# Xharlie/BtcDet

Measured on AMD Instinct MI355X. Metric: scenes/s fwd+bwd KITTI-Car bs=2/GPU (BtcDet hot path), higher is better.
Workload: dtype f32

## Files before the change

### btcdet_amd/_lib.py

```python
import ctypes
import os

import numpy as np
import torch

_HERE = os.path.dirname(os.path.abspath(__file__))
LIB_PATH = os.path.join(_HERE, "libbtcdet_hip.so")
_lib = None

c_i32p = ctypes.POINTER(ctypes.c_int32)
c_f32p = ctypes.POINTER(ctypes.c_float)
vp = ctypes.c_void_p
ci = ctypes.c_int
sz = ctypes.c_size_t

MODE_SUBM, MODE_CONV, MODE_TRANSPOSE = 0, 1, 2


class BtcHipError(RuntimeError):
    pass


class BtcOccConfig(ctypes.Structure):
    _fields_ = [("batch", ctypes.c_int32), ("grid", ctypes.c_int32 * 3), ("sphere_grid", ctypes.c_int32 * 3),
                ("dist_kern", ctypes.c_int32 * 3), ("concede_x", ctypes.c_int32), ("empt_sur_thresh", ctypes.c_int32),
                ("max_boxes", ctypes.c_int32), ("use_box_weight", ctypes.c_int32),
                ("occ_range", ctypes.c_float * 6), ("occ_voxel", ctypes.c_float * 3),
                ("sphere_range", ctypes.c_float * 6), ("sphere_voxel", ctypes.c_float * 3),
                ("det_zmin", ctypes.c_float), ("det_zmax", ctypes.c_float),
                ("w_fore_cls", ctypes.c_float), ("w_mirr_cls", ctypes.c_float), ("w_bm_cls", ctypes.c_float),
                ("w_neg_cls", ctypes.c_float), ("w_fore_res", ctypes.c_float), ("w_mirr_res", ctypes.c_float),
                ("w_bm_res", ctypes.c_float), ("box_weight", ctypes.c_float), ("backproject_lut", ctypes.c_void_p),
                ("reverse_vis", ctypes.c_int32), ("vis_half", ctypes.c_int32)]


OCC_BUFFER_FIELDS = ["vcc_mask", "voxelwise_mask", "bm_voxelwise_mask", "occ_voxelwise_mask", "fore_voxelwise_mask",
                     "pos_mask", "general_cls_loss_mask", "occ_fore_cls_mask", "occ_mirr_cls_mask", "occ_bm_cls_mask",
                     "general_reg_loss_mask", "forebox_label", "general_cls_loss_mask_float",
                     "general_reg_loss_mask_float", "res_mtrx", "pos_all_num"]


class BtcOccBuffers(ctypes.Structure):
    _fields_ = [(k, ctypes.c_void_p) for k in OCC_BUFFER_FIELDS]


class BtcChainLayer(ctypes.Structure):
    _fields_ = [("kind", ctypes.c_int32), ("ref", ctypes.c_int32), ("mode", ctypes.c_int32), ("in_shape", ctypes.c_int32 * 3),
                ("out_shape", ctypes.c_int32 * 3), ("k", ctypes.c_int32 * 3), ("s", ctypes.c_int32 * 3), ("p", ctypes.c_int32 * 3),
                ("d", ctypes.c_int32 * 3)]


class BtcPovConfig(ctypes.Structure):
    _fields_ = [("batch", ctypes.c_int32), ("max_k", ctypes.c_int32), ("occ_grid", ctypes.c_int32 * 3), ("det_grid", ctypes.c_int32 * 3),
                ("occ_origin", ctypes.c_float * 3), ("occ_voxel", ctypes.c_float * 3), ("det_origin", ctypes.c_float * 3),
                ("det_voxel", ctypes.c_float * 3), ("occ_thresh", ctypes.c_float), ("inten", ctypes.c_float), ("code_dim", ctypes.c_int32)]


_SIGS = {
    "btc_last_error": (ctypes.c_char_p, []),
    "btc_version": (ci, []),
    "btc_tune_set": (ci, [ci, ci]),
    "btc_tune_value": (ci, [ci]),
    "btc_mean_vfe": (ci, [vp, vp, ci, ci, ci, ci, vp, vp]),
    "btc_occ_vfe": (ci, [vp, vp, ci, ci, ci, ci, ci, vp, vp, vp]),
    "btc_boxes_pairwise_bev": (ci, [vp, ci, vp, ci, ci, vp, vp]),
    "btc_nms_ws_bytes": (sz, [ci]),
    "btc_nms": (ci, [vp, ci, ctypes.c_float, ci, vp, vp, vp, sz, vp]),
    "btc_nms_topk_ws_bytes": (sz, [ci, ci, ci]),
    "btc_trilinear_corners": (ci, [vp, ctypes.c_longlong, ctypes.c_longlong, c_f32p, c_f32p, c_f32p, c_i32p, ci, vp, vp, vp, vp, vp, vp]),
    "btc_trilinear_gather": (ci, [vp, ci, ctypes.c_longlong, vp, vp, vp, vp]),
    "btc_trilinear_scatter": (ci, [vp, ci, vp, vp, vp, ci, vp, vp]),
    "btc_nms_topk": (ci, [vp, ci, ci, ctypes.c_float, ci, ci, vp, vp, vp, sz, vp]),
    "btc_voxelize_ws_bytes": (sz, [ci, ci, ci]),
    "btc_voxelize": (ci, [vp, ci, ci, ci, ci, ci, vp, ci, c_f32p, c_f32p, c_i32p, ci, ci, vp, vp, vp, vp, vp, sz, vp]),
    "btc_cart_to_occ_coords": (ci, [vp, vp, ci, ci, ci, vp]),
    "btc_voxel_shift_col": (ci, [vp, vp, ci, ci, ci, ci, vp, ctypes.c_float, vp]),
    "btc_range_mask_ws_bytes": (sz, [ci]),
    "btc_range_mask_compact": (ci, [vp, vp, ci, ci, ci, vp, ci, c_f32p, vp, vp, vp, vp, vp, sz, vp]),
    "btc_gather_rows": (ci, [vp, vp, ci, ci, ci, vp, vp, vp]),
    "btc_out_shape": (ci, [c_i32p, c_i32p, c_i32p, c_i32p, c_i32p, c_i32p, ci, c_i32p]),
    "btc_rulebook_subm_ws_bytes": (sz, [ci]),
    "btc_rulebook_subm": (ci, [vp, ci, ci, c_i32p, c_i32p, c_i32p, vp, vp, vp, sz, vp]),
    "btc_rulebook_conv_ws_bytes": (sz, [ci, c_i32p]),
    "btc_rulebook_conv_count": (ci, [vp, ci, ci, c_i32p, c_i32p, c_i32p, c_i32p, c_i32p, c_i32p, ci, vp, vp, sz, vp]),
    "btc_rulebook_conv_fill": (ci, [vp, ci, ci, c_i32p, c_i32p, c_i32p, c_i32p, c_i32p, c_i32p, ci, ci, vp, vp, vp, vp, sz, vp]),
    "btc_pairs_from_nbr_ws_bytes": (sz, [ci, ci]),
    "btc_pairs_from_nbr": (ci, [vp, ci, ci, ci, vp, vp, vp, sz, vp]),
    "btc_chain_ws_bytes": (sz, [vp, ci, ci, ci]),
    "btc_chain_caps": (ci, [vp, ci, ci, ci, vp]),
    "btc_chain_levels": (ci, [vp, ci, ci, vp, ci, vp, vp, vp, vp, sz, vp]),
    "btc_chain_maps": (ci, [vp, ci, ci, vp, ci, vp, vp, vp, vp, vp, vp, vp, sz, vp]),
    "btc_conv_fwd": (ci, [vp, vp, vp, vp, ci, ci, ci, ci, vp, vp]),
    "btc_conv_dgrad": (ci, [vp, vp, vp, ci, ci, ci, ci, vp, vp]),
    "btc_conv_wgrad_ws_bytes": (sz, [ci, ci, ci, ci, ci]),
    "btc_conv_wgrad": (ci, [vp, vp, vp, ci, vp, ci, ci, ci, ci, vp, vp, sz, vp]),
    "btc_conv_fwd_bf16": (ci, [vp, vp, vp, vp, ci, ci, ci, ci, vp, vp]),
    "btc_conv_dgrad_bf16": (ci, [vp, vp, vp, ci, ci, ci, ci, vp, vp]),
    "btc_conv_wgrad_bf16": (ci, [vp, vp, vp, ci, vp, ci, ci, ci, ci, vp, vp, sz, vp]),
    "btc_conv_bf16w_supported": (ci, [ci, ci, ci]),
    "btc_weights_to_bf16": (ci, [vp, ci, ci, ci, vp, vp, vp]),
    "btc_conv_split_supported": (ci, [ci, ci, ci]),
    "btc_set_scratch": (ci, [vp, vp, sz]),
    "btc_conv_split_wanted": (ci, [ci, ci, ci, ci]),
    "btc_weights_split3": (ci, [vp, ci, ci, ci, vp, vp, vp]),
    "btc_weights_split3_multi": (ci, [vp, vp, vp, c_i32p, c_i32p, c_i32p, ci, vp]),
    "btc_weights_to_bf16_multi": (ci, [vp, vp, vp, c_i32p, c_i32p, c_i32p, ci, vp]),
    "btc_conv_fwd_bf16w": (ci, [vp, vp, vp, vp, ci, ci, ci, ci, vp, vp]),
    "btc_conv_dgrad_bf16w": (ci, [vp, vp, vp, ci, ci, ci, ci, vp, vp]),
    "btc_row_orders": (ci, [vp, c_i32p, c_i32p, ci, vp, vp]),
    "btc_row_orders_keyed": (ci, [vp, vp, c_i32p, c_i32p, ci, vp, vp]),
    "btc_conv_apply_ordered": (ci, [ci, ci, vp, vp, vp, vp, vp, ci, ci, ci, ci, vp, vp]),
    "btc_conv_apply_src": (ci, [ci, ci, vp, ctypes.c_longlong, vp, vp, vp, vp, ci, ci, ci, ci, vp, vp]),
    "btc_conv_wgrad_ordered": (ci, [ci, vp, vp, vp, ci, vp, ci, vp, vp, ci, ci, ci, vp, vp, sz, vp]),
    "btc_conv_wgrad_slabs": (ci, [ci, vp, vp, vp, ci, vp, ci, vp, vp, ci, ci, ci, vp, vp, sz, vp, vp]),
    "btc_wgrad_reduce_multi": (ci, [vp, vp, vp, vp, ci, vp]),
    "btc_adam_group_ws_bytes": (sz, [ci]),
    "btc_adam_max_segments": (ci, []),
    "btc_grads_pack": (ci, [vp, ci, vp, vp, vp, vp, c_i32p, vp, vp]),
    "btc_adam_group_step": (ci, [vp, ci, vp, vp, vp, vp, c_i32p, ci, vp, vp, vp, ctypes.c_longlong, ctypes.c_float, ctypes.c_float, ctypes.c_float,
                                 ctypes.c_float, ctypes.c_float, ctypes.c_float, vp, sz, vp]),
    "btc_maxpool_fwd": (ci, [vp, vp, ci, ci, ci, vp, vp]),
    "btc_maxpool_bwd": (ci, [vp, vp, vp, vp, ci, ci, ci, vp, vp]),
    "btc_dense_fwd": (ci, [vp, vp, ci, ci, c_i32p, vp, vp]),
    "btc_dense_bwd": (ci, [vp, vp, ci, ci, c_i32p, vp, vp]),
    "btc_revoxelize_ws_bytes": (sz, [ci, ci, c_i32p]),
    "btc_revoxelize_count": (ci, [vp, ci, ci, c_i32p, vp, vp, vp, sz, vp]),
    "btc_revoxelize_fill": (ci, [vp, vp, ci, ci, ci, c_i32p, ci, ci, vp, vp, vp, vp, sz, vp]),
    "btc_pass_occ_vox_ws_bytes": (sz, [ctypes.POINTER(BtcPovConfig), ci, ci]),
    "btc_pass_occ_vox_count": (ci, [ctypes.POINTER(BtcPovConfig), vp, vp, vp, vp, vp, vp, ci, ci, ci, vp, vp, sz, vp]),
    "btc_pass_occ_vox_fill": (ci, [ctypes.POINTER(BtcPovConfig), vp, ci, ci, ci, ci, ci, ci, vp, vp, vp, vp, vp, vp, sz, vp]),
    "btc_pass_occ_vox_fill_i32": (ci, [ctypes.POINTER(BtcPovConfig), vp, ci, ci, ci, ci, ci, ci, vp, vp, vp, vp, vp, vp, vp, vp, sz, vp]),
    "btc_occ_loss_ws_bytes": (sz, []),
    "btc_occ_loss_fwd": (ci, [vp, vp, vp, vp, vp, vp, vp, vp, ci, ctypes.c_longlong, ctypes.c_float, ctypes.c_float, ctypes.c_float, vp, vp, vp,
                              sz, vp]),
    "btc_occ_loss_bwd": (ci, [vp, vp, vp, vp, vp, vp, vp, vp, ci, ctypes.c_longlong, ctypes.c_float, vp, vp, vp, vp, vp]),
    "btc_occ_loss_fwd_total": (ci, [vp, vp, vp, vp, vp, vp, vp, vp, ci, ctypes.c_longlong, ctypes.c_float, ctypes.c_float, ctypes.c_float, vp, vp,
                                    vp, sz, vp]),
    "btc_occ_loss_bwd_total": (ci, [vp, vp, vp, vp, vp, vp, vp, vp, ci, ctypes.c_longlong, ctypes.c_float, vp, vp, vp, vp, vp]),
    "btc_dense_split_fwd": (ci, [vp, vp, ci, ci, ci, vp, vp, vp, vp]),
    "btc_occ_prob": (ci, [vp, vp, ci, ctypes.c_longlong, vp, vp]),
    "btc_dense_split_bwd": (ci, [vp, vp, vp, ci, ci, ci, vp, vp, vp]),
    "btc_cat_pad_fwd": (ci, [vp, ci, vp, ci, ctypes.c_longlong, ci, ci, vp, vp]),
    "btc_cat_pad_bwd": (ci, [vp, ci, ctypes.c_longlong, ci, vp, ci, vp, ci, vp]),
    "btc_sumsq2_ws_bytes": (sz, []),
    "btc_sumsq2_fwd": (ci, [vp, ctypes.c_longlong, ci, ctypes.c_double, vp, ctypes.c_longlong, ci, ctypes.c_double, vp, vp, sz, vp]),
    "btc_sumsq2_bwd": (ci, [vp, ctypes.c_longlong, ci, ctypes.c_float, vp, vp, ctypes.c_longlong, ci, ctypes.c_float, vp, vp, vp]),
    "btc_bn_ws_bytes": (sz, [ci]),
    "btc_bn_relu_fwd": (ci, [vp, ci, ci, vp, vp, vp, vp, vp, ctypes.c_float, ctypes.c_float, ci, ci, vp, vp, vp, vp, sz, vp]),
    "btc_spin": (ci, [ci, vp]),
    "btc_bn_relu_bwd": (ci, [vp, vp, vp, ci, ci, vp, vp, vp, ci, ci, vp, vp, vp, vp, sz, vp]),
    "btc_bn_relu_fwd_bf16": (ci, [vp, ci, ci, vp, vp, vp, vp, vp, ctypes.c_float, ctypes.c_float, ci, ci, vp, vp, vp, vp, sz, vp]),
    "btc_bn_relu_bwd_bf16": (ci, [vp, vp, vp, ci, ci, vp, vp, vp, ci, ci, vp, vp, vp, vp, sz, vp]),
    "btc_ball_query": (ci, [vp, vp, vp, vp, ci, ci, ctypes.c_float, ctypes.c_float, ci, vp, vp]),
    "btc_group_points": (ci, [vp, vp, vp, vp, ci, ci, ci, ci, vp, vp]),
    "btc_group_points_grad": (ci, [vp, vp, vp, vp, ci, ci, ci, ci, ci, vp, vp]),
    "btc_furthest_point_sampling": (ci, [vp, ci, ci, ci, vp, vp, vp]),
    "btc_three_nn": (ci, [vp, vp, vp, vp, ci, ci, vp, vp, vp]),
    "btc_three_interpolate": (ci, [vp, vp, vp, ci, ci, vp, vp]),
    "btc_three_interpolate_grad": (ci, [vp, vp, vp, ci, ci, ci, vp, vp]),
    "btc_bn_fuse_ws_bytes": (sz, []),
    "btc_conv_bn_relu_fwd": (ci, [ci, vp, vp, vp, vp, vp, ci, ci, ci, ci, vp, vp, vp, vp, vp, vp, ctypes.c_float, ctypes.c_float, ci, vp, vp, vp, vp, sz, vp, vp]),
    "btc_conv_bn_relu_fwd_src": (ci, [ci, vp, ctypes.c_longlong, vp, vp, vp, vp, ci, ci, ci, ci, vp, vp, vp, vp, vp, vp, ctypes.c_float, ctypes.c_float, ci, vp, vp, vp, vp, sz, vp, vp]),
    "btc_col_sum": (ci, [vp, ci, ci, vp, vp, sz, vp]),
    "btc_col_sum_bf16": (ci, [vp, ci, ci, vp, vp, sz, vp]),
    "btc_occ_targets_ws_bytes": (sz, [ctypes.POINTER(BtcOccConfig)]),
    "btc_occ_backproject_lut": (ci, [ctypes.POINTER(BtcOccConfig), vp, vp]),
    "btc_occ_targets": (ci, [ctypes.POINTER(BtcOccConfig), vp, vp, vp, ci, ci, ci, vp, vp, vp, vp, ci, vp, vp,
                             ctypes.POINTER(BtcOccBuffers), vp, sz, vp]),
}

EXPORTED_SYMBOLS = tuple(_SIGS.keys())

_INFER_SIGS = {
    "btc_conv_bn_eval_fwd": (ci, [ci, vp, ctypes.c_longlong, vp, vp, vp, vp, ci, ci, ci, ci, vp, vp, vp, vp, ctypes.c_float, ci, vp, vp]),
    "btc_det_select_nms_ws_bytes": (sz, [ci, ci]),
    "btc_det_select_nms": (ci, [vp, vp, ci, ci, ci, ci, ci, ctypes.c_float, ctypes.c_float, ci, ci, ci, vp, vp, vp, vp, sz, vp]),
    "btc_det_finish": (ci, [vp, vp, ci, ci, ci, ci, ci, ci, vp, vp, vp, vp, ci, vp, ci, ci, vp, ci, ci, c_f32p, ci, vp, vp, vp, vp, vp, vp]),
    "btc_occ_metrics_ws_bytes": (sz, [ci, ci]),
    "btc_occ_metrics": (ci, [vp, vp, vp, vp, ctypes.c_longlong, vp, vp, vp, ctypes.c_longlong, vp, vp, ci, ci, ci, vp, vp, sz, vp]),
    "btc_kitti_overlaps": (ci, [vp, vp, vp, vp, vp, c_i32p, ci, vp, vp, vp]),
    "btc_kitti_match_tp": (ci, [vp, vp, vp, vp, vp, vp, vp, c_i32p, ci, ci, ci, ci, ci, ci, vp, vp, vp]),
    "btc_kitti_match_stats_ws_bytes": (sz, [ci, ci, ci, ci, ci]),
    "btc_kitti_match_stats": (ci, [vp, vp, vp, vp, vp, vp, vp, vp, vp, vp, vp, c_i32p, ci, ci, ci, ci, ci, ci, ci, vp, vp, vp, sz, vp]),
}

INFER_EXPORTED_SYMBOLS = tuple(_INFER_SIGS.keys())

_AUGMENT_SIGS = {
    "btc_augment_ws_bytes": (sz, [ci, ci, ci]),
    "btc_augment_batch": (ci, [vp, ci, ci, vp, ci, vp, vp, vp, ctypes.c_longlong, vp, vp, vp, vp, ci, ctypes.c_longlong, vp, vp,
                               ctypes.c_longlong, vp, vp, vp, vp, sz, vp]),
    "btc_world_transform": (ci, [vp, ci, ci, vp, ci, vp, vp, vp, vp]),
}

AUGMENT_EXPORTED_SYMBOLS = tuple(_AUGMENT_SIGS.keys())

_BESTMATCH_SIGS = {
    "btc_place_templates": (ci, [vp, ctypes.c_longlong, vp, vp, vp, vp, vp, ci, ci, vp, vp, ctypes.c_longlong, ci, vp, vp]),
}

BESTMATCH_EXPORTED_SYMBOLS = tuple(_BESTMATCH_SIGS.keys())

_FRAMES_SIGS = {
    "btc_fov_crop_ws_bytes": (sz, [ci, ci]),
    "btc_fov_crop": (ci, [vp, ci, ci, vp, ci, vp, ci, vp, vp, vp, vp, sz, vp]),
}

FRAMES_EXPORTED_SYMBOLS = tuple(_FRAMES_SIGS.keys())

_GTDB_SIGS = {
    "btc_cut_objects_ws_bytes": (sz, [ci, ci, ci, ci]),
    "btc_cut_objects": (ci, [vp, ci, ci, vp, ci, vp, vp, vp, ci, ci, ci, vp, vp, vp, vp, sz, vp]),
}

GTDB_EXPORTED_SYMBOLS = tuple(_GTDB_SIGS.keys())

cf = ctypes.c_float
_TEMPLATES_SIGS = {
    "btc_nn_sqdist": (ci, [vp, ci, vp, ci, vp, vp, ci, ci, vp, vp]),
    "btc_match_candidates": (ci, [vp, ci, vp, vp, ci, vp, vp, ci, ci, cf, cf, cf, ci, ci, vp, vp, vp]),
    "btc_select_templates_ws_bytes": (sz, [ci, ci, ci]),
    "btc_select_templates": (ci, [vp, ci, vp, ci, vp, vp, vp, vp, vp, vp, ci, ci, ci, ci, ci, cf, cf, cf, ci, ci, vp, vp, vp, vp, vp, sz, vp]),
}

TEMPLATES_EXPORTED_SYMBOLS = tuple(_TEMPLATES_SIGS.keys())

_INFOS_SIGS = {
    "btc_count_in_boxes_ws_bytes": (sz, [ci, ci]),
    "btc_count_in_boxes": (ci, [vp, ci, ci, vp, ci, vp, vp, vp, ci, vp, vp, vp, sz, vp]),
    "btc_coverage_cells_ws_bytes": (sz, [ci, ci]),
    "btc_coverage_cells": (ci, [vp, ci, vp, ci, ci, vp, vp, ci, ci, vp, vp, vp, sz, vp]),
}

INFOS_EXPORTED_SYMBOLS = tuple(_INFOS_SIGS.keys())

_HEADS_SIGS = {
    "btc_anchor_targets_ws_bytes": (sz, [ci, ci]),
    "btc_anchor_targets": (ci, [vp, ci, ci, vp, ci, vp, vp, vp, ci, vp, ci, ci, vp, vp, vp, vp, sz, vp]),
    "btc_decode_anchor_boxes": (ci, [vp, vp, vp, ci, ci, ci, cf, cf, vp, vp]),
}

HEADS_EXPORTED_SYMBOLS = tuple(_HEADS_SIGS.keys())

_ANCHOR_LOSS_SIGS = {
    "btc_anchor_loss_ws_bytes": (sz, [ci, ci]),
    "btc_anchor_loss_fwd": (ci, [vp, vp, vp, vp, vp, vp, ci, ci, ci, ci, cf, cf, cf, cf, vp, vp, vp, sz, vp]),
    "btc_anchor_loss_bwd": (ci, [vp, vp, vp, vp, vp, vp, ci, ci, ci, ci, cf, cf, cf, cf, vp, vp, vp, vp, vp, vp]),
}

ANCHOR_LOSS_EXPORTED_SYMBOLS = tuple(_ANCHOR_LOSS_SIGS.keys())


class BtcRoiTargetsConfig(ctypes.Structure):
    _fields_ = [("R", ctypes.c_int32), ("fg_quota", ctypes.c_int32), ("by_class", ctypes.c_int32), ("score_type", ctypes.c_int32),
                ("reg_fg", ctypes.c_float), ("cls_fg", ctypes.c_float), ("cls_bg", ctypes.c_float), ("cls_bg_lo", ctypes.c_float),
                ("fg_thresh", ctypes.c_float), ("cls_span", ctypes.c_float), ("hard_bg_ratio", ctypes.c_double)]


_ROI_TARGETS_SIGS = {
    "btc_roi_targets_ws_bytes": (sz, [ci, ci]),
    "btc_roi_targets": (ci, [vp, vp, vp, vp, vp, vp, ci, ci, ci, ctypes.POINTER(BtcRoiTargetsConfig), vp, vp, vp, vp, vp, vp, vp, vp, vp, vp, vp, vp, sz, vp]),
}

ROI_TARGETS_EXPORTED_SYMBOLS = tuple(_ROI_TARGETS_SIGS.keys())


def lib():
    global _lib
    if _lib is None:
        if not os.path.exists(LIB_PATH):
            raise BtcHipError(
                f"{LIB_PATH} not found: build it with `python -c 'import __graft_entry__ as g; g.build()'` "
                f"or `make -C btcdet_amd/csrc` (there is no CPU fallback for the hot path)")
        L = ctypes.CDLL(LIB_PATH)
        for name, (res, args) in (list(_SIGS.items()) + list(_INFER_SIGS.items()) + list(_AUGMENT_SIGS.items()) + list(_BESTMATCH_SIGS.items()) +
                                  list(_FRAMES_SIGS.items()) + list(_GTDB_SIGS.items()) + list(_TEMPLATES_SIGS.items()) + list(_INFOS_SIGS.items()) + list(_HEADS_SIGS.items()) +
                                  list(_ANCHOR_LOSS_SIGS.items()) + list(_ROI_TARGETS_SIGS.items())):
            fn = getattr(L, name)
            fn.restype = res
            fn.argtypes = args
        for kv in filter(None, os.environ.get("BTC_TUNE", "").split(",")):
            k, v = kv.split("=")
            if L.btc_tune_set(int(k), int(v)) != 0:
                raise BtcHipError("BTC_TUNE: bad entry %r" % kv)
        _lib = L
    return _lib


_fast = False


def fast():
    global _fast
    if _fast is False:
        _fast = None
        if os.environ.get("BTC_FASTPATH", "1") != "0":
            try:
                lib()
                from . import _btcfast
                if _btcfast.abi_version() == lib().btc_version():
                    _fast = _btcfast
            except ImportError:
                _fast = None
    return _fast


def check(rc, what):
    if rc != 0:
        msg = lib().btc_last_error().decode("utf-8", "replace")
        raise BtcHipError(f"{what} failed (code {rc}): {msg}")


_raw_stream = torch._C._cuda_getCurrentRawStream
_cur_device = torch._C._cuda_getDevice


def stream_ptr():
    return _raw_stream(_cur_device())


def ptr(t):
    if t is None:
        return None
    if not (t.is_cuda and t.is_contiguous()):
        raise BtcHipError("expected a contiguous tensor on the GPU (HIP) device")
    return t.data_ptr()


_I3_CACHE = {}


def i3(v):
    if isinstance(v, (int, np.integer)):
        key = (int(v),) * 3
    else:
        key = tuple(int(x) for x in np.asarray(v).reshape(-1))
        if len(key) != 3:
            raise BtcHipError(f"expected 3 values, got {v!r}")
    a = _I3_CACHE.get(key)
    if a is None:
        a = np.ascontiguousarray(np.array(key, dtype=np.int32))
        a.setflags(write=False)
        a_ptr = a.ctypes.data_as(c_i32p)
        _I3_CACHE[key] = a
        _I3P_CACHE[id(a)] = (a, a_ptr)
    return a


_I3P_CACHE = {}


def i3p(a):
    hit = _I3P_CACHE.get(id(a))
    if hit is not None and hit[0] is a:
        return hit[1]
    return a.ctypes.data_as(c_i32p)


def f32p(a):
    return a.ctypes.data_as(c_f32p)


def workspace(nbytes, device):
    return torch.empty(max(int(nbytes), 256), dtype=torch.uint8, device=device)
```

### btcdet_amd/backbones_3d.py

```python
import os
from functools import partial

import torch
import torch.nn as nn

from . import spconv


def post_act_block(in_channels, out_channels, kernel_size, indice_key=None, stride=1, padding=0, conv_type='subm',
                   norm_fn=None, defaultvalue=1.0, activation=nn.ReLU):
    if conv_type == 'subm':
        conv = spconv.SubMConv3d(in_channels, out_channels, kernel_size, bias=False, indice_key=indice_key)
    elif conv_type == 'subm2d':
        conv = spconv.SubMConv2d(in_channels, out_channels, kernel_size, bias=False, indice_key=indice_key)
    elif conv_type == 'spconv':
        conv = spconv.SparseConv3d(in_channels, out_channels, kernel_size, stride=stride, padding=padding, bias=False,
                                   indice_key=indice_key)
    elif conv_type == 'fixspconv':
        conv = fixSparseConv3d(in_channels, out_channels, kernel_size, stride=stride, padding=padding, bias=False,
                               indice_key=indice_key, defaultvalue=defaultvalue)
        conv.requires_grad_(False)
    elif conv_type == 'spdeconv':
        conv = spconv.SparseConvTranspose3d(in_channels, out_channels, kernel_size, stride=stride, padding=padding,
                                            bias=False, indice_key=indice_key)
    elif conv_type == 'inverseconv':
        conv = spconv.SparseInverseConv3d(in_channels, out_channels, kernel_size, indice_key=indice_key, bias=False)
    elif conv_type == 'submbias':
        conv = spconv.SubMConv3d(in_channels, out_channels, kernel_size, bias=True, indice_key=indice_key)
    elif conv_type == 'maxpool':
        conv = spconv.SparseMaxPool3d(kernel_size, stride=stride, padding=padding)
    else:
        raise NotImplementedError(conv_type)
    if norm_fn is not None:
        return spconv.SparseSequential(conv, norm_fn(out_channels), activation())
    return spconv.SparseSequential(conv)


def _feature_dtype(model_cfg):
    v = str(model_cfg.get("FEATURE_DTYPE", "fp32")).lower()
    if v in ("bf16", "bfloat16"):
        return torch.bfloat16
    if v in ("fp32", "float32"):
        return None
    raise ValueError("FEATURE_DTYPE must be fp32 or bf16, got %r" % v)


class fixSparseConv3d(spconv.SparseConv3d):

    def __init__(self, in_channels, out_channels, kernel_size, stride=1, padding=0, bias=False, indice_key=None,
                 defaultvalue=1.0):
        super(fixSparseConv3d, self).__init__(in_channels, out_channels, kernel_size, stride=stride, padding=padding,
                                              bias=bias, indice_key=indice_key)
        self.weight.data.fill_(defaultvalue)


def _to_feature_dtype(x, dtype):
    if dtype is not None and x.features is not None and x.features.dtype != dtype and x.features.shape[1] % 16 == 0:
        x.features = x.features.to(dtype)
    return x


def _seq(specs, norm_fn):
    return spconv.SparseSequential(*[post_act_block(ci, co, k, norm_fn=norm_fn, **kw) for ci, co, k, kw in specs])


class VoxelBackBoneDeconv(nn.Module):

    def __init__(self, model_cfg, input_channels, grid_size, **kwargs):
        super().__init__()
        self.model_cfg = model_cfg
        self.y_shift = model_cfg.get("SHIFT", 0)
        self.feature_dtype = _feature_dtype(model_cfg)
        norm_fn = partial(nn.BatchNorm1d, eps=1e-3, momentum=0.01)
        self.sparse_shape = grid_size[::-1]
        self.sparse_shape[1] += self.y_shift * 2
        c = [16, 32, 64]
        sp = dict(padding=1, conv_type='spconv')
        self.conv1 = spconv.SparseSequential(post_act_block(input_channels, c[0], 3, norm_fn=norm_fn, indice_key='spconv1', **sp))
        self.conv2 = _seq([(c[0], c[1], 3, dict(stride=2, indice_key='spconv2', **sp)),
                           (c[1], c[1], 3, dict(padding=1, indice_key='subm2'))], norm_fn)
        self.conv3 = _seq([(c[1], c[2], 3, dict(stride=2, indice_key='spconv3', **sp)),
                           (c[2], c[2], 3, dict(padding=1, indice_key='subm3'))], norm_fn)
        self.deconv4 = _seq([(c[2], c[1], 3, dict(stride=2, padding=1, indice_key='spconv4', conv_type='spdeconv')),
                             (c[1], c[1], 3, dict(padding=1, indice_key='subm4'))], norm_fn)
        self.deconv5 = _seq([(c[1], c[1], 3, dict(stride=2, padding=1, indice_key='spconv5', conv_type='spdeconv')),
                             (c[1], c[1], 3, dict(padding=1, indice_key='subm5'))], norm_fn)
        self.num_point_features = c[1]

    def forward(self, batch_dict):
        voxel_features, voxel_coords = batch_dict['voxel_features'], batch_dict['voxel_coords'].int()
        if self.feature_dtype is not None and voxel_features.shape[1] % 16 == 0:
            voxel_features = voxel_features.to(self.feature_dtype)
        if self.y_shift > 0:
            voxel_features, voxel_coords = self.add_shift(voxel_features, voxel_coords)
        x = spconv.SparseConvTensor(features=voxel_features, indices=voxel_coords, spatial_shape=self.sparse_shape,
                                    batch_size=batch_dict['batch_size'])
        ready = batch_dict.pop('occ_geometry', None)
        if ready is not None and ready[0] is voxel_coords:
            x.indice_dict = ready[1]
        x = self._forward_stages(x)
        if self.y_shift > 0:
            x = self.remove_shift(x)
        batch_dict.update({'encoded_spconv_tensor': x, 'encoded_spconv_tensor_stride': 1})
        return batch_dict

    def _forward_stages(self, x):
        for stage in (self.conv1, self.conv2, self.conv3, self.deconv4, self.deconv5):
            x = stage(x)
            x = _to_feature_dtype(x, self.feature_dtype)
        return x

    def prefetch_geometry(self, batch_dict, head=None):
        if self.y_shift > 0:
            return batch_dict
        voxel_coords = batch_dict['voxel_coords'].int()
        if not voxel_coords.is_cuda:
            return batch_dict
        from .spconv import ops as sp_ops
        stages = (self.conv1, self.conv2, self.conv3, self.deconv4, self.deconv5)
        bs = batch_dict['batch_size']
        merged_head = head is not None and hasattr(head, "_merge_ok") and head._merge_ok()
        if sp_ops.fast() is not None and (head is None or merged_head or hasattr(head, "conv_cls")):
            from .spconv.geometry import cached_plan
            def plan_stages():
                out = list(stages)
                if head is not None:
                    out.append(head.conv_cls)
                    if getattr(head, "reg", False):
                        out.append(head.conv_res)
                return out
            plan = cached_plan(self, (int(bs), id(head)), plan_stages, self.sparse_shape, bs)
            indice_dict = {}
            plan.run(voxel_coords, indice_dict)
            batch_dict['occ_geometry'] = (voxel_coords, indice_dict)
            return batch_dict
        x = spconv.SparseConvTensor(features=None, indices=voxel_coords, spatial_shape=self.sparse_shape, batch_size=bs)
        for stage in stages:
            x = stage.forward_geometry(x)
        if head is not None and hasattr(head, "forward_geometry"):
            head.forward_geometry(x)
        batch_dict['occ_geometry'] = (voxel_coords, x.indice_dict)
        return batch_dict

    def add_shift(self, voxel_features, voxel_coords):
        y_max = self.sparse_shape[1] - 2 * self.y_shift
        left = voxel_coords[..., 2] < self.y_shift
        right = voxel_coords[..., 2] >= (y_max - self.y_shift)
        lc, rc = voxel_coords[left, :].clone(), voxel_coords[right, :].clone()
        rc[..., 2] -= y_max
        lc[..., 2] += y_max
        feats = torch.cat([voxel_features[right, :], voxel_features, voxel_features[left, :]], dim=0)
        coords = torch.cat([rc, voxel_coords, lc], dim=0)
        coords[..., 2] += self.y_shift
        return feats, coords

    def remove_shift(self, x):
        y_max = self.sparse_shape[1] - 2 * self.y_shift
        x.indices[..., 2] -= self.y_shift
        keep = (x.indices[..., 2] >= 0) & (x.indices[..., 2] < y_max)
        x.features, x.indices = x.features[keep, :], x.indices[keep, :]
        x.spatial_shape[1] -= self.y_shift * 2
        return x


DET_GEOMETRY_WALK = True
FAST_STAGES = True


class VoxelBackBone8xOcc(nn.Module):

    def __init__(self, model_cfg, input_channels, grid_size, **kwargs):
        super().__init__()
        self.model_cfg = model_cfg
        norm_fn = partial(nn.BatchNorm1d, eps=1e-3, momentum=0.01)
        self.sparse_shape = grid_size[::-1] + [1, 0, 0]
        self.occ_conv_type = self.model_cfg.OCC_CONV_TYPE
        self.occ_conv_exec = self.model_cfg.OCC_CONV_EXECUTE
        self.out_feat_type = getattr(self.model_cfg, "OUT_FEAT_TYPE", ["None", "None", "None", "None", "combine"])
        self.out_att = getattr(self.model_cfg, "OCC_ATT", [False, False, False, False])
        c = [16, 32, 64, 64, 128]
        self.occ_code_num = input_channels - kwargs["original_num_rawpoint_features"]
        add = [self.occ_code_num if t else 0 for t in self.occ_conv_exec] + [0] * (4 - len(self.occ_conv_exec))

        for i in range(1, len(self.occ_conv_exec)):
            self._build_occ_net(self.occ_conv_type[i], i)
        for i in range(len(self.occ_conv_exec)):
            if self.out_att[i]:
                ch = c[i] + add[i]
                setattr(self, 'att_conv%d' % (i + 1), spconv.SparseSequential(post_act_block(
                    ch, ch, 3, norm_fn=norm_fn, stride=1, padding=1, indice_key='subm%d' % (i + 1), activation=nn.LeakyReLU)))

        self.conv1 = spconv.SparseSequential(
            spconv.SubMConv3d(input_channels, c[0], 3, padding=1, bias=False, indice_key='subm1'), norm_fn(c[0]), nn.ReLU())
        self.conv1_combine = _seq([(c[0] + add[0], c[0], 3, dict(padding=1, indice_key='subm1'))], norm_fn)
        down = [None, dict(stride=2, padding=1, indice_key='spconv2', conv_type='spconv'),
                dict(stride=2, padding=1, indice_key='spconv3', conv_type='spconv'),
                dict(stride=2, padding=(0, 1, 1), indice_key='spconv4', conv_type='spconv')]
        for lvl in (1, 2, 3):
            setattr(self, 'conv%d' % (lvl + 1), _seq([(c[lvl - 1], c[lvl], 3, down[lvl])], norm_fn))
            key = 'subm%d' % (lvl + 1)
            setattr(self, 'conv%d_combine' % (lvl + 1),
                    _seq([(c[lvl] + add[lvl], c[lvl], 3, dict(padding=1, indice_key=key)),
                          (c[lvl], c[lvl], 3, dict(padding=1, indice_key=key))], norm_fn))
        last_pad = self.model_cfg.get('last_pad', 0)
        self.feature_dtype = _feature_dtype(model_cfg)
        self.conv_out = spconv.SparseSequential(
            spconv.SparseConv3d(c[3], c[4], (3, 1, 1), stride=(2, 1, 1), padding=last_pad, bias=False,
                                indice_key='spconv_down2'), norm_fn(c[4]), nn.ReLU())
        self.num_point_features = 128

        for i in range(4):
            if self.out_feat_type[i] == "2D":
                ch = c[i] * [41, 21, 11, 5][i]
                setattr(self, 'squeeze_z_conv%d' % (i + 1), spconv.SparseSequential(post_act_block(
                    ch, ch // 2, 3, norm_fn=norm_fn, padding=1, indice_key='submsqueez%d' % (i + 1), conv_type='subm2d')))
        self._build_combine_net(norm_fn, c, self.out_feat_type[4])
        self.walk_async = True

    def _walk_geometry(self, coords, bs, indice_dict, allow_async=True):
        from .spconv import ops as sp_ops
        if not (DET_GEOMETRY_WALK and coords.is_cuda and sp_ops.fast() is not None and sp_ops.CAPTURE is None):
            return False
        from .spconv.geometry import cached_plan
        plan = cached_plan(self, int(bs), self._plan_stages, self.sparse_shape, bs)
        if allow_async and self.walk_async and sp_ops.PROFILE is None and plan.entries[0][0] == 0:
            conv0 = plan.convs[0]
            rb0 = sp_ops.build_rulebook_g(coords, bs, conv0._geometry(self.sparse_shape))
            if conv0.indice_key is not None:
                indice_dict[conv0.indice_key] = rb0
            indice_dict.setdefault("__geometry_cache__", {})[conv0._gkey(coords, self.sparse_shape)] = (rb0, coords)
            return (plan, plan.start(coords, side_stream=True), {0: rb0}, coords)
        return ("done", plan, plan.run(coords, indice_dict))

    def _plan_stages(self):
        stages = [self.conv1, self.conv1_combine, self.conv2, self.conv2_combine, self.conv3, self.conv3_combine, self.conv4, self.conv4_combine,
                  self.conv_out]
        if getattr(self, "squeezeBev", None) is not None:
            stages.append(self.squeezeBev)
        if getattr(self, "down3", None) is not None:
            stages += [self.down2, self.down3, self.down_combine]
        return stages

    @staticmethod
    def _finish_walk(walk, indice_dict):
        if isinstance(walk, tuple) and walk[0] == "done":
            return walk[1], walk[2]
        if isinstance(walk, tuple):
            plan, handle, have, coords = walk
            return plan, plan.finish(handle, coords, indice_dict, have)
        return None

    def _stage(self, stage, x, ready):
        sl = ready[0].stage_slices.get(id(stage)) if ready is not None else None
        if sl is not None:
            chain = stage._chain_plan(x, ready[1][sl[0]:sl[1]])
            if chain is not None:
                return stage._run_chain(x, *chain)
        return stage(x)

    def _stages(self, stages, x, ready):
        for stage in stages:
            x = self._stage(stage, x, ready)
        return x

    def _build_occ_net(self, kind, i):
        n = self.occ_code_num
        key = 'spconv%d' % (i + 1)
        pad = 1 if i < 3 else (1, 1, 1)
        kw = {'maxpool': dict(k=3, conv_type='maxpool'), 'weight': dict(k=3, conv_type='spconv'),
              'fix': dict(k=3, conv_type='fixspconv', defaultvalue=1.0 / 27),
              'avgpool': dict(k=2, conv_type='fixspconv', defaultvalue=1)}[kind]
        k = kw.pop('k')
        setattr(self, 'occ_conv%d' % (i + 1), spconv.SparseSequential(
            post_act_block(n, n, k, norm_fn=None, stride=2, padding=pad, indice_key=key, **kw)))

    def _build_combine_net(self, norm_fn, c, comb_type):
        sp = dict(stride=2, conv_type='spconv')
        self.down2 = _seq([(c[1], c[1], 3, dict(padding=1, indice_key='spconv3', **sp)),
                           (c[1], c[2], 3, dict(padding=(0, 1, 1), indice_key='spconv4', **sp))], norm_fn)
        self.down3 = _seq([(c[2], c[2], 3, dict(padding=(0, 1, 1), indice_key='spconv4', **sp))], norm_fn)
        cat = c[2] * 2 + c[3]
        if comb_type == "big_combine":
            self.down_combine = _seq([(cat, c[3] * 2, 3, dict(padding=1, indice_key='subm4')),
                                      (c[3] * 2, c[3] * 2, 3, dict(padding=1, indice_key='subm4'))], norm_fn)
        elif comb_type == "combine":
            self.down_combine = _seq([(cat, c[3] * 2, 3, dict(padding=1, indice_key='subm4')),
                                      (c[3] * 2, c[3] * 2, 3, dict(stride=[1, 2, 2], padding=(1, 1, 1), indice_key='spconv5',
                                                                   conv_type='spconv')),
                                      (c[3] * 2, c[3] * 2, 3, dict(padding=1, indice_key='subm5'))], norm_fn)
        elif comb_type == "big_bev_combine":
            self.squeezeBev = _seq([(c[4], c[3], (2, 1, 1), dict(stride=(2, 1, 1), padding=0, indice_key='subm_down2',
                                                                  conv_type='spconv'))], norm_fn)
            self.down_combine = _seq([(cat + c[3], c[3] * 2, 3, dict(padding=1, indice_key='subm4')),
                                      (c[3] * 2, c[3] * 2, 3, dict(padding=1, indice_key='subm4'))], norm_fn)

    @staticmethod
    def sparse_cat(input_lst, pad=False):
        xrep, xocc = input_lst
        if pad:
            from .spconv import ops as sp_ops
            xrep.features = sp_ops.cat_features(xrep.features, xocc.features)
        else:
            xrep.features = torch.cat((xrep.features, xocc.features.to(xrep.features.dtype)), dim=1)
        return xrep

    @staticmethod
    def apply_att(x, att_conv):
        a = att_conv(x)
        x.features = x.features * a.features + x.features
        return x

    def suqeeze(self, feat, i, kind):
        if kind == "None":
            return None
        if kind == "3D":
            return feat
        conv = getattr(self, "squeeze_z_conv{}".format(i), None)
        dense = feat.dense()
        B, C, Z, Y, X = list(dense.shape)
        inds = torch.unique(torch.cat([feat.indices[..., 0:1], feat.indices[..., 2:]], dim=-1), dim=0).long()
        pix = dense.reshape(B, C * Z, Y, X)[inds[..., 0], :, inds[..., 1], inds[..., 2]]
        return conv(spconv.SparseConvTensor(features=pix, indices=inds.int(), spatial_shape=[Y, X], batch_size=B)).dense()

    @staticmethod
    def compress_height(t):
        d = t.dense()
        N, C, D, H, W = d.shape
        return d.view(N, C * D, H, W)

    def res_combine(self, x2, x3, x4, bev, out_feat_type="combine", ready=None):
        if getattr(self, "down3", None) is None:
            return None
        x2, x3 = self._stage(self.down2, x2, ready), self._stage(self.down3, x3, ready)
        if out_feat_type == "big_bev_combine":
            bev2d = self.compress_height(self._stage(self.squeezeBev, bev, ready))
            x4.features = torch.cat((x2.features, x3.features, x4.features,
                                     _BevGather.apply(bev2d, x4.indices, tuple(x4.spatial_shape), x4.batch_size).to(x4.features.dtype)), dim=1)
        else:
            x4.features = torch.cat((x2.features, x3.features, x4.features), dim=1)
        return self._stage(self.down_combine, x4, ready)

    @staticmethod
    def _coords_i32(batch_dict):
        from .vfe import i32_twin
        coords = batch_dict['voxel_coords']
        tw = i32_twin(batch_dict, coords)
        return tw if tw is not None else coords.int()

    def prefetch_geometry(self, batch_dict):
        coords = self._coords_i32(batch_dict)
        if not coords.is_cuda or coords.shape[0] == 0:
            return batch_dict
        indice_dict = {}
        walk = self._walk_geometry(coords, batch_dict['batch_size'], indice_dict, allow_async=False)
        if isinstance(walk, tuple) and walk[0] == "done":
            batch_dict['det_geometry'] = (coords, indice_dict, walk)
        return batch_dict

    def forward(self, batch_dict):
        coords = self._coords_i32(batch_dict)
        feats = batch_dict['voxel_features']
        if self.feature_dtype is not None and feats.shape[1] % 16 == 0:
            feats = feats.to(self.feature_dtype)
        bs = batch_dict['batch_size']
        x = spconv.SparseConvTensor(features=feats, indices=coords, spatial_shape=self.sparse_shape, batch_size=bs)
        pre = batch_dict.pop('det_geometry', None)
        if pre is not None and pre[0] is coords:
            x.indice_dict = pre[1]
            walk = pre[2]
        else:
            walk = self._walk_geometry(coords, bs, x.indice_dict)
        n_occ = len(self.occ_conv_exec)
        ready = None
        if FAST_STAGES and isinstance(walk, tuple) and walk[0] == "done":
            ready = self._finish_walk(walk, x.indice_dict)
        merge_first = ready is not None and not (n_occ > 0 and self.occ_conv_exec[0])
        x1 = _to_feature_dtype(self._stage(self.conv1, x, ready), self.feature_dtype)
        if merge_first:
            x1 = self._stage(self.conv1_combine, x1, ready)
        occ = None
        if n_occ > 0:
            occ = spconv.SparseConvTensor(features=batch_dict["occ_voxel_features"], indices=coords,
                                          spatial_shape=self.sparse_shape, batch_size=bs)
            occ.indice_dict["__geometry_cache__"] = x.indice_dict.setdefault("__geometry_cache__", {})
            if self.occ_conv_exec[0]:
                x1 = self.sparse_cat([x1, occ], pad=not self.out_att[0])
                if self.out_att[0]:
                    x1 = self.apply_att(x1, self.att_conv1)
        if not merge_first:
            x1 = self._stage(self.conv1_combine, x1, ready)
        if ready is None:
            ready = self._finish_walk(walk, x.indice_dict)
            if not FAST_STAGES:
                ready = None
        levels = [x1]
        cur = x1
        for lvl in (1, 2, 3):
            if not (n_occ > lvl):
                cur = self._stages([getattr(self, 'conv%d' % (lvl + 1)), getattr(self, 'conv%d_combine' % (lvl + 1))], cur, ready)
                levels.append(cur)
                continue
            cur = self._stage(getattr(self, 'conv%d' % (lvl + 1)), cur, ready)
            if n_occ > lvl:
                occ = getattr(self, 'occ_conv%d' % (lvl + 1))(occ)
                if self.occ_conv_exec[lvl]:
                    cur = self.sparse_cat([cur, occ], pad=not self.out_att[lvl])
                    if self.out_att[lvl]:
                        cur = self.apply_att(cur, getattr(self, 'att_conv%d' % (lvl + 1)))
            cur = self._stage(getattr(self, 'conv%d_combine' % (lvl + 1)), cur, ready)
            levels.append(cur)
        x1, x2, x3, x4 = levels
        out = self._stage(self.conv_out, x4, ready)
        batch_dict.update({'encoded_spconv_tensor': out, 'encoded_spconv_tensor_stride': 8})
        batch_dict['__level_rows__'] = {'det_L0': int(x1.features.shape[0]), 'det_L1': int(x2.features.shape[0]),
                                        'det_L2': int(x3.features.shape[0]), 'det_L3': int(x4.features.shape[0]),
                                        'det_out': int(out.features.shape[0])}
        batch_dict.update({'multi_scale_3d_features': {
            'x_conv1': self.suqeeze(x1, 1, self.out_feat_type[0]),
            'x_conv2': self.suqeeze(x2, 2, self.out_feat_type[1]),
            'x_conv3': self.suqeeze(x3, 3, self.out_feat_type[2]),
            'x_conv4': self.suqeeze(x4, 4, self.out_feat_type[3]),
            'x_combine': self.res_combine(x2, x3, x4, out, out_feat_type=self.out_feat_type[4], ready=ready),
        }})
        return batch_dict


class _BevGather(torch.autograd.Function):

    @staticmethod
    def forward(ctx, bev2d, indices, spatial_shape, batch_size):
        inds = indices.long()
        ctx.save_for_backward(indices)
        ctx.meta = (spatial_shape, batch_size, bev2d.dtype)
        return bev2d[inds[:, 0], :, inds[:, 2], inds[:, 3]]

    @staticmethod
    def backward(ctx, grad):
        (indices,) = ctx.saved_tensors
        spatial_shape, batch_size, dtype = ctx.meta
        vol = spconv.SparseConvTensor(grad.contiguous(), indices, list(spatial_shape), batch_size).dense()
        return vol.sum(2).to(dtype), None, None, None


class SparseBasicBlock(spconv.SparseModule):
    expansion = 1

    def __init__(self, inplanes, planes, stride=1, norm_fn=None, downsample=None, indice_key=None):
        super().__init__()
        assert norm_fn is not None
        self.conv1 = spconv.SubMConv3d(inplanes, planes, kernel_size=3, stride=stride, padding=1, bias=True, indice_key=indice_key)
        self.bn1 = norm_fn(planes)
        self.relu = nn.ReLU()
        self.conv2 = spconv.SubMConv3d(planes, planes, kernel_size=3, stride=stride, padding=1, bias=True, indice_key=indice_key)
        self.bn2 = norm_fn(planes)
        self.downsample = downsample
        self.stride = stride

    def forward(self, x):
        identity = x.features if self.downsample is None else self.downsample(x).features
        out = self.conv1(x)
        out.features = _bn_act(self.bn1, out.features, True)
        out = self.conv2(out)
        out.features = torch.relu(_bn_act(self.bn2, out.features, False) + identity)
        return out


def _bn_act(bn, feats, relu):
    from .spconv import fused_bn
    if feats.is_cuda and feats.dim() == 2 and fused_bn.is_sync(bn):
        return fused_bn.sync_batch_norm_relu(bn, feats, relu)
    if feats.is_cuda and feats.dim() == 2 and feats.shape[0] > 0 and fused_bn.fusable(bn):
        return fused_bn.batch_norm_relu(bn, feats, relu)
    y = bn(feats)
    return torch.relu(y) if relu else y


def _lateral_combine(x_lateral, x_bottom, conv_expnd, comb_conv):
    x_expnd = conv_expnd(x_lateral)
    M = x_bottom.features.shape[0]
    ind_all = torch.cat([x_bottom.indices, x_expnd.indices], dim=0)
    _, rinds = torch.unique(ind_all, dim=0, return_inverse=True)
    pad = torch.zeros((M, x_expnd.features.shape[1]), dtype=x_bottom.features.dtype, device=x_bottom.features.device)
    pad[rinds[M:], :] = x_expnd.features.to(pad.dtype)
    x_bottom.features = torch.cat([x_bottom.features, pad], dim=-1)
    return comb_conv(x_bottom)


class _ResDecoderBase(nn.Module):

    def forward(self, batch_dict):
        feats, coords = batch_dict['voxel_features'], batch_dict['voxel_coords'].int()
        x = spconv.SparseConvTensor(features=feats, indices=coords, spatial_shape=self.sparse_shape, batch_size=batch_dict['batch_size'])
        x1 = self.conv1(x)
        x2 = self.conv2(x1)
        x3 = self.conv3(x2)
        x2d = _lateral_combine(x2, self.deconv2(x3), self.conv22, self.comb_conv2)
        x1d = _lateral_combine(x1, self.deconv1(x2d), self.conv11, self.comb_conv1)
        batch_dict.update({'encoded_spconv_tensor': x1d, 'encoded_spconv_tensor_stride': 1})
        return batch_dict


class VoxelBackBoneDeconvRes(_ResDecoderBase):

    def __init__(self, model_cfg, input_channels, grid_size, **kwargs):
        super().__init__()
        self.model_cfg = model_cfg
        norm_fn = partial(nn.BatchNorm1d, eps=1e-3, momentum=0.01)
        self.sparse_shape = grid_size[::-1]
        c = [16, 32, 64]
        sp, dc = dict(conv_type='spconv'), dict(conv_type='spdeconv')
        self.conv1 = _seq([(input_channels, c[0], 3, dict(padding=1, indice_key='spconv1', **sp))], norm_fn)
        self.conv2 = _seq([(c[0], c[1], 3, dict(stride=2, padding=1, indice_key='spconv2', **sp)),
                           (c[1], c[1], 3, dict(padding=1, indice_key='subm2'))], norm_fn)
        self.conv3 = _seq([(c[1], c[2], 3, dict(stride=2, padding=1, indice_key='spconv3', **sp)),
                           (c[2], c[2], 3, dict(padding=1, indice_key='subm3'))], norm_fn)
        self.conv22 = _seq([(c[1], c[1], 3, dict(stride=1, padding=1, indice_key='spconv22', **sp))], norm_fn)
        self.deconv2 = _seq([(c[2], c[1], 3, dict(stride=2, padding=1, indice_key='spconvd2', **dc))], norm_fn)
        self.comb_conv2 = _seq([(c[1] + c[1], c[1], 3, dict(padding=1, indice_key='submd2'))], norm_fn)
        self.conv11 = _seq([(c[0], c[0], 3, dict(stride=1, padding=1, indice_key='spconv11', **sp))], norm_fn)
        self.deconv1 = _seq([(c[1], c[1], 3, dict(stride=2, padding=1, indice_key='spconvd1', **dc))], norm_fn)
        self.comb_conv1 = _seq([(c[1] + c[0], c[1], 3, dict(padding=1, indice_key='submd1'))], norm_fn)
        self.num_point_features = c[1]


class VoxelBackBoneInverseRes(_ResDecoderBase):

    def __init__(self, model_cfg, input_channels, grid_size, **kwargs):
        super().__init__()
        self.model_cfg = model_cfg
        norm_fn = partial(nn.BatchNorm1d, eps=1e-3, momentum=0.01)
        self.sparse_shape = grid_size[::-1]
        c = [16, 32, 64]
        sp, inv = dict(conv_type='spconv'), dict(conv_type='inverseconv')
        self.conv1 = _seq([(input_channels, c[0], 3, dict(padding=1, indice_key='subm1'))], norm_fn)
        self.conv2 = _seq([(c[0], c[1], 3, dict(stride=2, padding=1, indice_key='spconv2', **sp)),
                           (c[1], c[1], 3, dict(padding=1, indice_key='subm2'))], norm_fn)
        self.conv3 = _seq([(c[1], c[2], 3, dict(stride=2, padding=1, indice_key='spconv3', **sp)),
                           (c[2], c[2], 3, dict(padding=1, indice_key='subm3'))], norm_fn)
        self.conv22 = _seq([(c[1], c[1], 3, dict(stride=1, padding=1, indice_key='subm2'))], norm_fn)
        self.deconv2 = _seq([(c[2], c[1], 3, dict(stride=2, padding=1, indice_key='spconv3', **inv))], norm_fn)
        self.comb_conv2 = _seq([(c[1] + c[1], c[1], 3, dict(padding=1, indice_key='subm2'))], norm_fn)
        self.conv11 = _seq([(c[0], c[0], 3, dict(stride=1, padding=1, indice_key='subm1'))], norm_fn)
        self.deconv1 = _seq([(c[1], c[1], 3, dict(stride=2, padding=1, indice_key='spconv2', **inv))], norm_fn)
        self.comb_conv1 = _seq([(c[1] + c[0], c[1], 3, dict(padding=1, indice_key='subm1'))], norm_fn)
        self.num_point_features = c[1]


class VoxelResBackBone8x(nn.Module):

    def __init__(self, model_cfg, input_channels, grid_size, **kwargs):
        super().__init__()
        self.model_cfg = model_cfg
        norm_fn = partial(nn.BatchNorm1d, eps=1e-3, momentum=0.01)
        self.sparse_shape = grid_size[::-1] + [1, 0, 0]
        self.conv_input = spconv.SparseSequential(spconv.SubMConv3d(input_channels, 16, 3, padding=1, bias=False, indice_key='subm1'),
                                                  norm_fn(16), nn.ReLU())
        res = lambda ch, key: SparseBasicBlock(ch, ch, norm_fn=norm_fn, indice_key=key)
        down = lambda ci, co, pad, key: post_act_block(ci, co, 3, norm_fn=norm_fn, stride=2, padding=pad, indice_key=key, conv_type='spconv')
        self.conv1 = spconv.SparseSequential(res(16, 'res1'), res(16, 'res1'))
        self.conv2 = spconv.SparseSequential(down(16, 32, 1, 'spconv2'), res(32, 'res2'), res(32, 'res2'))
        self.conv3 = spconv.SparseSequential(down(32, 64, 1, 'spconv3'), res(64, 'res3'), res(64, 'res3'))
        self.conv4 = spconv.SparseSequential(down(64, 128, (0, 1, 1), 'spconv4'), res(128, 'res4'), res(128, 'res4'))
        last_pad = self.model_cfg.get('last_pad', 0)
        self.conv_out = spconv.SparseSequential(spconv.SparseConv3d(128, 128, (3, 1, 1), stride=(2, 1, 1), padding=last_pad, bias=False,
                                                                    indice_key='spconv_down2'), norm_fn(128), nn.ReLU())
        self.num_point_features = 128

    def forward(self, batch_dict):
        feats, coords = batch_dict['voxel_features'], batch_dict['voxel_coords'].int()
        x = spconv.SparseConvTensor(features=feats, indices=coords, spatial_shape=self.sparse_shape, batch_size=batch_dict['batch_size'])
        x = self.conv_input(x)
        x1 = self.conv1(x)
        x2 = self.conv2(x1)
        x3 = self.conv3(x2)
        x4 = self.conv4(x3)
        out = self.conv_out(x4)
        batch_dict.update({'encoded_spconv_tensor': out, 'encoded_spconv_tensor_stride': 8,
                           'multi_scale_3d_features': {'x_conv1': x1, 'x_conv2': x2, 'x_conv3': x3, 'x_conv4': x4}})
        return batch_dict


__all__ = {'VoxelBackBoneDeconv': VoxelBackBoneDeconv, 'VoxelBackBone8xOcc': VoxelBackBone8xOcc,
           'VoxelBackBoneDeconvRes': VoxelBackBoneDeconvRes, 'VoxelBackBoneInverseRes': VoxelBackBoneInverseRes,
           'VoxelResBackBone8x': VoxelResBackBone8x}
```

### btcdet_amd/csrc/binding.cpp

```cpp
#include <torch/extension.h>
#include <c10/hip/HIPCachingAllocator.h>
#include <c10/hip/HIPStream.h>
#include <c10/hip/HIPGuard.h>
#include <hip/hip_runtime_api.h>
#include <torch/csrc/autograd/engine.h>

#include <atomic>
#include <mutex>
#include <stdexcept>
#include <string>
#include <unordered_map>
#include <cstdio>
#include <cstdlib>
#include <memory>
#include <tuple>
#include <vector>

#include "../../include/btcdet_hip.h"
#include "../../include/btcdet_hip_infer.h"

namespace {

using at::Tensor;
using OptTensor = c10::optional<at::Tensor>;

inline void chk(int rc, const char* what) {
  if (rc != 0) throw std::runtime_error(std::string(what) + " failed (code " + std::to_string(rc) + "): " + btc_last_error());
}

inline const float* fptr(const OptTensor& t) { return (t.has_value() && t->defined()) ? (const float*)t->data_ptr() : nullptr; }
inline void* vptr(const OptTensor& t) { return (t.has_value() && t->defined()) ? t->data_ptr() : nullptr; }
inline void* st(int64_t stream) { return reinterpret_cast<void*>(stream); }
inline const int32_t* ip(int64_t p) { return reinterpret_cast<const int32_t*>(p); }


inline void need(bool ok, const char* msg) {
  if (!ok) throw std::runtime_error(msg);
}
inline void need(bool ok, const char* who, const char* msg) {
  if (!ok) throw std::runtime_error(std::string(who) + msg);
}

struct WqEntry {
  c10::weak_intrusive_ptr<c10::TensorImpl> weak;
  uint32_t version;
  Tensor q;
  WqEntry(c10::weak_intrusive_ptr<c10::TensorImpl> w, uint32_t v, Tensor t) : weak(std::move(w)), version(v), q(std::move(t)) {}
};
std::mutex g_wq_mu;
std::unordered_map<const void*, WqEntry> g_wq;
std::unordered_map<const void*, WqEntry> g_ws;

void convert_weights(const Tensor& w, int64_t K, int64_t cin, int64_t cout, int planes, Tensor& q, int64_t stream) {
  char* row1 = (char*)q.data_ptr() + 2 * planes * w.numel();
  if (planes == 1)
    chk(btc_weights_to_bf16((const float*)w.data_ptr(), (int)K, (int)cin, (int)cout, q.data_ptr(), row1, st(stream)), "btc_weights_to_bf16");
  else
    chk(btc_weights_split3((const float*)w.data_ptr(), (int)K, (int)cin, (int)cout, q.data_ptr(), row1, st(stream)), "btc_weights_split3");
}

Tensor weights_q(const Tensor& w, int64_t K, int64_t cin, int64_t cout, int64_t stream, int planes) {
  const void* key = w.unsafeGetTensorImpl();
  const uint32_t version = (uint32_t)w._version();
  if (!w.is_leaf()) {
    Tensor q = at::empty({2, planes * w.numel()}, w.options().dtype(at::kBFloat16));
    convert_weights(w, K, cin, cout, planes, q, stream);
    return q;
  }
  std::lock_guard<std::mutex> lock(g_wq_mu);
  auto& tab = planes == 1 ? g_wq : g_ws;
  auto it = tab.find(key);
  if (it != tab.end() && !it->second.weak.expired() && it->second.version == version && it->second.q.get_device() == w.get_device())
    return it->second.q;
  Tensor q = (it != tab.end() && !it->second.weak.expired() && it->second.q.numel() == 2 * planes * w.numel() && it->second.q.get_device() == w.get_device())
                 ? it->second.q : at::empty({2, planes * w.numel()}, w.options().dtype(at::kBFloat16));
  convert_weights(w, K, cin, cout, planes, q, stream);
  if (it != tab.end()) tab.erase(it);
  tab.emplace(key, WqEntry(c10::weak_intrusive_ptr<c10::TensorImpl>(w.getIntrusivePtr()), version, q));
  for (auto e = tab.begin(); e != tab.end();) e = e->second.weak.expired() ? tab.erase(e) : std::next(e);
  return q;
}

void refresh_weights(const std::vector<Tensor>& weights, int64_t stream, int planes) {
  const size_t n = weights.size();
  if (n == 0) return;
  std::vector<const float*> W(n);
  std::vector<void*> ws(n), wts(n);
  std::vector<int32_t> K(n), Cin(n), Cout(n);
  std::lock_guard<std::mutex> lock(g_wq_mu);
  auto& tab = planes == 1 ? g_wq : g_ws;
  for (size_t i = 0; i < n; ++i) {
    const Tensor& w = weights[i];
    need(w.is_leaf() && w.is_contiguous() && w.scalar_type() == at::kFloat && w.dim() >= 3, "refresh_weights: contiguous fp32 leaf weights [.., Cin, Cout] expected");
    const int64_t cin = w.size(-2), cout = w.size(-1);
    const void* key = w.unsafeGetTensorImpl();
    auto it = tab.find(key);
    Tensor q = (it != tab.end() && !it->second.weak.expired() && it->second.q.numel() == 2 * planes * w.numel() && it->second.q.get_device() == w.get_device())
                   ? it->second.q : at::empty({2, planes * w.numel()}, w.options().dtype(at::kBFloat16));
    if (it != tab.end()) tab.erase(it);
    tab.emplace(key, WqEntry(c10::weak_intrusive_ptr<c10::TensorImpl>(w.getIntrusivePtr()), (uint32_t)w._version(), q));
    W[i] = (const float*)w.data_ptr();
    ws[i] = q.data_ptr();
    wts[i] = (char*)q.data_ptr() + 2 * planes * w.numel();
    K[i] = (int32_t)(w.numel() / (cin * cout)); Cin[i] = (int32_t)cin; Cout[i] = (int32_t)cout;
  }
  if (planes == 1)
    chk(btc_weights_to_bf16_multi(W.data(), ws.data(), wts.data(), K.data(), Cin.data(), Cout.data(), (int)n, st(stream)), "btc_weights_to_bf16_multi");
  else
    chk(btc_weights_split3_multi(W.data(), ws.data(), wts.data(), K.data(), Cin.data(), Cout.data(), (int)n, st(stream)), "btc_weights_split3_multi");
}

void split_weights(const std::vector<Tensor>& weights, int64_t stream) { refresh_weights(weights, stream, 3); }
void bf16_weights(const std::vector<Tensor>& weights, int64_t stream) { refresh_weights(weights, stream, 1); }

void ensure_scratch(const Tensor& like, int64_t stream) {
  static std::mutex mu;
  static std::unordered_map<uint64_t, Tensor> tab;
  const uint64_t key = ((uint64_t)(uint8_t)like.get_device() << 56) ^ (uint64_t)stream;
  std::lock_guard<std::mutex> lock(mu);
  if (tab.find(key) != tab.end()) return;
  Tensor t = at::empty({(int64_t)48 << 20}, like.options().dtype(at::kByte));
  chk(btc_set_scratch(st(stream), t.data_ptr(), (size_t)t.numel()), "btc_set_scratch");
  tab.emplace(key, t);
}

struct Operands {
  int operands;
  const void* w;
  Tensor hold;
};

Operands operands_of(const Tensor& src, const Tensor& w, int64_t K, int64_t cred, int64_t cres, int64_t n_rows, int pass, int64_t stream) {
  const bool fwd = pass == BTC_PASS_FWD, bf = src.scalar_type() == at::kBFloat16;
  int planes = 0;
  if (bf) {
    if (btc_conv_bf16w_supported((int)K, (int)cred, (int)cres) && btc_tune_value(BTC_TUNE_BF16_OPERANDS) != 1) planes = 1;
  } else if (src.scalar_type() == at::kFloat && btc_conv_split_wanted((int)K, (int)cred, (int)cres, (int)n_rows) &&
             src.numel() * 4 < (int64_t)0xFFFFFF00LL) {
    ensure_scratch(src, stream);
    planes = 3;
  }
  if (!planes) return {bf ? BTC_OPERANDS_BF16_ACT : BTC_OPERANDS_F32, w.data_ptr(), Tensor()};
  Tensor q = weights_q(w, K, fwd ? cred : cres, fwd ? cres : cred, stream, planes);
  return {planes == 1 ? BTC_OPERANDS_BF16 : BTC_OPERANDS_F32_SPLIT, (const char*)q.data_ptr() + (fwd ? 2 * planes * w.numel() : 0), q};
}

const int32_t* order_ptr(const OptTensor& o, int64_t n_rows, const char* who) {
  if (!o.has_value() || !o->defined()) return nullptr;
  need(o->scalar_type() == at::kInt && o->is_contiguous() && o->numel() == n_rows, who, ": the row order does not match the map");
  return (const int32_t*)o->data_ptr();
}

struct FwdSite {
  int64_t cin, cout, K, n_res;
  const int32_t* order;
  Tensor out;
};

FwdSite fwd_site(const char* who, const Tensor& features, const Tensor& w, const Tensor& map_fwd, const OptTensor& order_fwd, bool stats_ok = true) {
  FwdSite f;
  f.cin = w.size(-2), f.cout = w.size(-1), f.K = map_fwd.size(1), f.n_res = map_fwd.size(0);
  need(features.is_contiguous() && w.is_contiguous() && map_fwd.is_contiguous(), who, ": contiguous tensors expected");
  need(w.numel() == f.K * f.cin * f.cout && features.size(1) == f.cin, who, ": weight does not match the rulebook / features");
  need(stats_ok, who, ": running statistics of the result channels expected");
  f.order = order_ptr(order_fwd, f.n_res, who);
  f.out = at::empty({f.n_res, f.cout}, features.options());
  return f;
}

Tensor conv_fwd(const Tensor& features, const Tensor& w, const OptTensor& bias, const Tensor& map_fwd, const OptTensor& order_fwd, int64_t stream) {
  FwdSite f = fwd_site("conv_fwd", features, w, map_fwd, order_fwd);
  const Operands op = operands_of(features, w, f.K, f.cin, f.cout, f.n_res, BTC_PASS_FWD, stream);
  chk(btc_conv_apply_src(BTC_PASS_FWD, op.operands, features.data_ptr(), (long long)features.size(0), op.w, fptr(bias), (const int32_t*)map_fwd.data_ptr(),
                         f.order, (int)f.n_res, (int)f.K, (int)f.cin, (int)f.cout, f.out.data_ptr(), st(stream)), "btc_conv_apply_src (fwd)");
  return f.out;
}

std::tuple<Tensor, Tensor> bn_fwd(const Tensor& x, const OptTensor& gamma, const OptTensor& beta, const OptTensor& rm, const OptTensor& rv,
                                  const OptTensor& nbt, bool use_batch, double momentum, double eps, bool relu, const Tensor& ws, int64_t ws_bytes,
                                  int64_t stream) {
  const int64_t N = x.size(0), C = x.size(1);
  Tensor y = at::empty_like(x);
  Tensor stats = at::empty({2, C}, x.options().dtype(at::kFloat));
  float* mean = (float*)stats.data_ptr();
  float* rstd = mean + C;
  long long* nb = (nbt.has_value() && nbt->defined()) ? (long long*)nbt->data_ptr() : nullptr;
  if (x.scalar_type() == at::kBFloat16)
    chk(btc_bn_relu_fwd_bf16(x.data_ptr(), (int)N, (int)C, fptr(gamma), fptr(beta), (float*)vptr(rm), (float*)vptr(rv), nb, (float)momentum,
                             (float)eps, (int)use_batch, (int)relu, y.data_ptr(), mean, rstd, ws.data_ptr(), (size_t)ws_bytes, st(stream)),
        "btc_bn_relu_fwd_bf16");
  else
    chk(btc_bn_relu_fwd((const float*)x.data_ptr(), (int)N, (int)C, fptr(gamma), fptr(beta), (float*)vptr(rm), (float*)vptr(rv), nb,
                        (float)momentum, (float)eps, (int)use_batch, (int)relu, (float*)y.data_ptr(), mean, rstd, ws.data_ptr(), (size_t)ws_bytes,
                        st(stream)), "btc_bn_relu_fwd");
  return std::make_tuple(y, stats);
}

Tensor fuse_ws_of(const Tensor& like, int64_t stream) {
  static std::mutex mu;
  static std::unordered_map<uint64_t, Tensor> tab;
  const uint64_t key = ((uint64_t)(uint8_t)like.get_device() << 56) ^ (uint64_t)stream;
  std::lock_guard<std::mutex> lock(mu);
  auto it = tab.find(key);
  if (it != tab.end()) return it->second;
  Tensor t = at::zeros({(int64_t)btc_bn_fuse_ws_bytes()}, like.options().dtype(at::kByte));
  tab.emplace(key, t);
  return t;
}

std::tuple<Tensor, Tensor, Tensor> conv_bn_fwd(const Tensor& features, const Tensor& w, const OptTensor& bias, const Tensor& map_fwd,
                                               const OptTensor& order_fwd, const OptTensor& gamma, const OptTensor& beta, const OptTensor& rm, const OptTensor& rv,
                                               const OptTensor& nbt, bool use_batch, double momentum, double eps, bool relu, const Tensor& ws,
                                               int64_t ws_bytes, int64_t stream) {
  if (use_batch && map_fwd.size(0) >= 1) {
    FwdSite f = fwd_site("conv_bn_fwd", features, w, map_fwd, order_fwd);
    Tensor y = at::empty_like(f.out);
    Tensor stats = at::empty({2, f.cout}, features.options().dtype(at::kFloat));
    Tensor fw = fuse_ws_of(features, stream);
    float* mean = (float*)stats.data_ptr();
    long long* nb = (nbt.has_value() && nbt->defined()) ? (long long*)nbt->data_ptr() : nullptr;
    const Operands op = operands_of(features, w, f.K, f.cin, f.cout, f.n_res, BTC_PASS_FWD, stream);
    chk(btc_conv_bn_relu_fwd_src(op.operands, features.data_ptr(), (long long)features.size(0), op.w, fptr(bias), (const int32_t*)map_fwd.data_ptr(), f.order,
                                 (int)f.n_res, (int)f.K, (int)f.cin, (int)f.cout, f.out.data_ptr(), fptr(gamma), fptr(beta), (float*)vptr(rm), (float*)vptr(rv), nb,
                                 (float)momentum, (float)eps, (int)relu, y.data_ptr(), mean, mean + f.cout, ws.data_ptr(), (size_t)ws_bytes, fw.data_ptr(), st(stream)),
        "btc_conv_bn_relu_fwd_src");
    return std::make_tuple(f.out, y, stats);
  }
  Tensor x = conv_fwd(features, w, bias, map_fwd, order_fwd, stream);
  auto ys = bn_fwd(x, gamma, beta, rm, rv, nbt, use_batch, momentum, eps, relu, ws, ws_bytes, stream);
  return std::make_tuple(x, std::get<0>(ys), std::get<1>(ys));
}

std::atomic<int64_t> g_eval_fold_calls{0};

Tensor conv_bn_eval_fold(const Tensor& features, const Tensor& w, const OptTensor& bias, const Tensor& map_fwd, const OptTensor& order_fwd,
                         const OptTensor& gamma, const OptTensor& beta, const Tensor& rm, const Tensor& rv, double eps, bool relu, int64_t stream) {
  FwdSite f = fwd_site("conv_bn_eval_fold", features, w, map_fwd, order_fwd,
                       rm.defined() && rv.defined() && rm.numel() == w.size(-1) && rv.numel() == w.size(-1));
  const Operands op = operands_of(features, w, f.K, f.cin, f.cout, f.n_res, BTC_PASS_FWD, stream);
  chk(btc_conv_bn_eval_fwd(op.operands, features.data_ptr(), (long long)features.size(0), op.w, fptr(bias), (const int32_t*)map_fwd.data_ptr(), f.order,
                           (int)f.n_res, (int)f.K, (int)f.cin, (int)f.cout, fptr(gamma), fptr(beta), (const float*)rm.data_ptr(), (const float*)rv.data_ptr(),
                           (float)eps, (int)relu, f.out.data_ptr(), st(stream)), "btc_conv_bn_eval_fwd");
  ++g_eval_fold_calls;
  return f.out;
}

int64_t eval_fold_calls() { return g_eval_fold_calls.load(); }

bool eval_fold_wanted(const Tensor& features, const Tensor& weight, const OptTensor& bias, const Tensor& map_fwd, const OptTensor& gamma,
                      const OptTensor& beta, const OptTensor& rm, const OptTensor& rv, bool use_batch) {
  if (use_batch || map_fwd.size(0) < 1 || !(rm.has_value() && rm->defined() && rv.has_value() && rv->defined())) return false;
  if (btc_tune_value(BTC_TUNE_EVAL_FOLD) == 1) return false;
  if (!at::GradMode::is_enabled()) return true;
  auto rg = [](const OptTensor& t) { return t.has_value() && t->defined() && t->requires_grad(); };
  return !(features.requires_grad() || weight.requires_grad() || rg(bias) || rg(gamma) || rg(beta));
}

std::tuple<Tensor, Tensor> bn_bwd(const Tensor& x, const Tensor& y, const Tensor& dy, const OptTensor& gamma, const Tensor& stats, bool use_batch,
                                  bool relu, const Tensor& ws, int64_t ws_bytes, int64_t stream) {
  const int64_t N = x.size(0), C = x.size(1);
  need(dy.is_contiguous() && dy.scalar_type() == x.scalar_type(), "bn_bwd: dy must be contiguous and of the activation type");
  Tensor dx = at::empty_like(x);
  Tensor dparam = at::empty({2, C}, x.options().dtype(at::kFloat));
  const float* mean = (const float*)stats.data_ptr();
  float* dgamma = (float*)dparam.data_ptr();
  if (x.scalar_type() == at::kBFloat16)
    chk(btc_bn_relu_bwd_bf16(x.data_ptr(), y.data_ptr(), dy.data_ptr(), (int)N, (int)C, fptr(gamma), mean, mean + C, (int)use_batch, (int)relu,
                             dx.data_ptr(), dgamma, dgamma + C, ws.data_ptr(), (size_t)ws_bytes, st(stream)), "btc_bn_relu_bwd_bf16");
  else
    chk(btc_bn_relu_bwd((const float*)x.data_ptr(), (const float*)y.data_ptr(), (const float*)dy.data_ptr(), (int)N, (int)C, fptr(gamma), mean,
                        mean + C, (int)use_batch, (int)relu, (float*)dx.data_ptr(), dgamma, dgamma + C, ws.data_ptr(), (size_t)ws_bytes, st(stream)),
        "btc_bn_relu_bwd");
  return std::make_tuple(dx, dparam);
}

struct SlabJob {
  Tensor ws;
  c10::weak_intrusive_ptr<c10::StorageImpl> dw_storage;
  float* dw;
  long long count;
  int S;
};

struct SideStream {
  hipStream_t side = nullptr;
  hipEvent_t fork = nullptr, join = nullptr;
  c10::hip::HIPStream* c10side = nullptr;
  std::mutex slab_mu;
  std::vector<SlabJob> slabs;
  std::atomic<bool> pending{false};
  std::atomic<int> queued_task{-1};
};

std::atomic<bool> g_defer_join{false};
const bool g_batch_reduce = true;

unsigned sync_event_flags() {
  return hipEventDisableTiming | hipEventDisableSystemFence;
}

SideStream& side_of(int device) {
  static SideStream tab[64];
  static std::mutex mu;
  SideStream& s = tab[device & 63];
  std::lock_guard<std::mutex> lock(mu);
  if (!s.side) {
    static std::vector<c10::hip::HIPStream> keep;
    keep.reserve(64);
    keep.push_back(c10::hip::getStreamFromPool(false, (c10::DeviceIndex)device));
    s.c10side = &keep.back();
    s.side = keep.back().stream();
    const unsigned flags = sync_event_flags();
    if (hipEventCreateWithFlags(&s.fork, flags) != hipSuccess || hipEventCreateWithFlags(&s.join, flags) != hipSuccess)
      throw std::runtime_error("hipEventCreateWithFlags failed");
  }
  return s;
}

void reduce_slabs(SideStream& s) {
  std::vector<SlabJob> jobs;
  {
    std::lock_guard<std::mutex> lock(s.slab_mu);
    jobs.swap(s.slabs);
  }
  if (jobs.empty()) return;
  std::vector<const float*> parts;
  std::vector<float*> dws;
  std::vector<int> S;
  std::vector<long long> counts;
  std::vector<c10::intrusive_ptr<c10::StorageImpl>> alive;
  for (size_t i = 0; i < jobs.size(); ++i) {
    auto st = jobs[i].dw_storage.lock();
    if (!st) continue;
    alive.push_back(std::move(st));
    parts.push_back((const float*)jobs[i].ws.data_ptr());
    dws.push_back(jobs[i].dw);
    S.push_back(jobs[i].S);
    counts.push_back(jobs[i].count);
  }
  if (parts.empty()) return;
  chk(btc_wgrad_reduce_multi(parts.data(), dws.data(), S.data(), counts.data(), (int)parts.size(), (void*)s.side), "btc_wgrad_reduce_multi");
}

void join_side(SideStream& s, hipStream_t main) {
  if (!s.pending.load()) return;
  reduce_slabs(s);
  if (hipEventRecord(s.join, s.side) != hipSuccess || hipStreamWaitEvent(main, s.join, 0) != hipSuccess)
    throw std::runtime_error("side-stream join failed");
  s.pending = false;
}

void join_wgrad() {
  const int dev = (int)c10::hip::current_device();
  join_side(side_of(dev), c10::hip::getCurrentHIPStream().stream());
}

void set_defer_wgrad_join(bool on) { g_defer_join = on; }

void set_side_stream(int64_t raw_stream, int64_t device_index) {
  SideStream& s = side_of((int)device_index);
  if (s.pending.load()) throw std::runtime_error("set_side_stream: weight gradients are in flight on the current side stream");
  static std::mutex mu;
  std::lock_guard<std::mutex> lock(mu);
  static std::vector<c10::hip::HIPStream> keep;
  keep.reserve(256);
  keep.push_back(c10::hip::getStreamFromExternal(reinterpret_cast<hipStream_t>(raw_stream), (c10::DeviceIndex)device_index));
  s.c10side = &keep.back();
  s.side = keep.back().stream();
}

std::tuple<OptTensor, OptTensor> conv_bwd(const Tensor& features, const Tensor& w, const Tensor& map_fwd, const Tensor& map_bwd,
                                          const OptTensor& order_bwd, const Tensor& grad_out, bool need_din, bool need_dw, bool overlap,
                                          bool allow_defer, int64_t stream) {
  const int64_t cin = w.size(-2), cout = w.size(-1), K = map_fwd.size(1), n_res = map_fwd.size(0), n_src = map_bwd.size(0);
  need(grad_out.is_contiguous() && grad_out.scalar_type() == features.scalar_type(), "conv_bwd: grad must be contiguous and of the activation type");
  const bool bf = features.scalar_type() == at::kBFloat16;
  const int32_t* order = order_ptr(order_bwd, n_src, "conv_bwd");
  const bool mirror = map_fwd.numel() > 0 && map_bwd.data_ptr() == map_fwd.data_ptr();
  const int pass_dgrad = mirror ? BTC_PASS_DGRAD_MIRROR : BTC_PASS_DGRAD;
  const int32_t* wg_map_bwd = (const int32_t*)map_bwd.data_ptr();
  OptTensor din, dw;
  Tensor ws;
  hipStream_t main = (hipStream_t)st(stream);
  const bool defer = g_defer_join && need_dw && allow_defer && (!w.is_leaf() || !w.grad().defined());
  SideStream* ss = ((overlap && need_din && need_dw) || defer) ? &side_of(features.get_device()) : nullptr;
  void* wstream = st(stream);
  if (ss) {
    if (hipEventRecord(ss->fork, main) != hipSuccess || hipStreamWaitEvent(ss->side, ss->fork, 0) != hipSuccess)
      throw std::runtime_error("side-stream fork failed");
    wstream = (void*)ss->side;
  }
  const bool wgrad_first = bf;
  Tensor q_hold;
  auto run_dgrad = [&]() {
  if (need_din) {
    Tensor d = at::empty({n_src, cin}, features.options());
    const Operands op = operands_of(grad_out, w, K, cout, cin, n_src, pass_dgrad, stream);
    q_hold = op.hold;
    chk(btc_conv_apply_src(pass_dgrad, op.operands, grad_out.data_ptr(), (long long)grad_out.size(0), op.w, nullptr, (const int32_t*)map_bwd.data_ptr(), order,
                           (int)n_src, (int)K, (int)cin, (int)cout, d.data_ptr(), st(stream)), "btc_conv_apply_src (dgrad)");
    din = d;
  }
  };
  auto run_wgrad = [&]() {
  if (need_dw) {
    Tensor g = at::empty(w.sizes(), w.options());
    const size_t ws_bytes = btc_conv_wgrad_ws_bytes((int)n_res, (int)K, (int)cin, (int)cout, (int)n_src);
    ws = at::empty({(int64_t)(ws_bytes > 256 ? ws_bytes : 256)}, features.options().dtype(at::kByte));
    if (defer && g_batch_reduce) {
      int n_slabs = 0;
      chk(btc_conv_wgrad_slabs((int)bf, features.data_ptr(), grad_out.data_ptr(), (const int32_t*)map_fwd.data_ptr(), (int)n_res, wg_map_bwd, (int)n_src,
                               nullptr, nullptr, (int)K, (int)cin, (int)cout, (float*)g.data_ptr(), ws.data_ptr(), ws_bytes, &n_slabs, wstream),
          "btc_conv_wgrad_slabs");
      if (n_slabs > 0) {
        std::lock_guard<std::mutex> lock(ss->slab_mu);
        ss->slabs.push_back(SlabJob{ws, g.storage().getWeakStorageImpl(), (float*)g.data_ptr(), (long long)g.numel(), n_slabs});
      }
    } else if (bf)
      chk(btc_conv_wgrad_bf16(features.data_ptr(), grad_out.data_ptr(), (const int32_t*)map_fwd.data_ptr(), (int)n_res,
                              wg_map_bwd, (int)n_src, (int)K, (int)cin, (int)cout, (float*)g.data_ptr(), ws.data_ptr(),
                              ws_bytes, wstream), "btc_conv_wgrad_bf16");
    else
      chk(btc_conv_wgrad((const float*)features.data_ptr(), (const float*)grad_out.data_ptr(), (const int32_t*)map_fwd.data_ptr(), (int)n_res,
                         wg_map_bwd, (int)n_src, (int)K, (int)cin, (int)cout, (float*)g.data_ptr(), ws.data_ptr(),
                         ws_bytes, wstream), "btc_conv_wgrad");
    dw = g;
  }
  };
  if (wgrad_first) { run_wgrad(); run_dgrad(); } else { run_dgrad(); run_wgrad(); }
  if (ss && !defer) {
    ss->pending = true;
    join_side(*ss, main);
  } else if (ss) {
    ss->pending = true;
    c10::hip::HIPCachingAllocator::recordStream(grad_out.storage().data_ptr(), *ss->c10side);
    c10::hip::HIPCachingAllocator::recordStream(ws.storage().data_ptr(), *ss->c10side);
    c10::hip::HIPCachingAllocator::recordStream(features.storage().data_ptr(), *ss->c10side);
    c10::hip::HIPCachingAllocator::recordStream(dw->storage().data_ptr(), *ss->c10side);
    c10::hip::HIPCachingAllocator::recordStream(map_fwd.storage().data_ptr(), *ss->c10side);
    c10::hip::HIPCachingAllocator::recordStream(map_bwd.storage().data_ptr(), *ss->c10side);
    const int task = torch::autograd::get_current_graph_task_id();
    if (task < 0) {
      join_side(*ss, main);
    } else if (ss->queued_task.load() != task) {
      SideStream* sp = ss;
      try {
        torch::autograd::Engine::get_default_engine().queue_callback([sp]() {
          sp->queued_task = -1;
          join_side(*sp, c10::hip::getCurrentHIPStream().stream());
        });
        ss->queued_task = task;
      } catch (const std::exception&) {
        join_side(*ss, main);
      }
    }
  }
  return std::make_tuple(din, dw);
}

std::vector<Tensor> row_orders_keyed(const std::vector<Tensor>& maps, const std::vector<Tensor>& keys, int64_t stream);
std::vector<Tensor> row_orders(const std::vector<Tensor>& maps, int64_t stream) { return row_orders_keyed(maps, {}, stream); }

std::vector<Tensor> row_orders_keyed(const std::vector<Tensor>& maps, const std::vector<Tensor>& keys, int64_t stream) {
  std::vector<Tensor> out(maps.size());
  need(keys.empty() || keys.size() == maps.size(), "row_orders: one key tensor (or an undefined one) per map");
  for (size_t base = 0; base < maps.size(); base += BTC_ROW_ORDER_MAX_MAPS) {
    const size_t m = std::min(maps.size() - base, (size_t)BTC_ROW_ORDER_MAX_MAPS);
    std::vector<const int32_t*> ptrs(m), kptrs(m, nullptr);
    std::vector<int32_t> ns(m), ks(m);
    int64_t total = 0;
    for (size_t j = 0; j < m; ++j) {
      const Tensor& t = maps[base + j];
      need(t.dim() == 2 && t.scalar_type() == at::kInt && t.is_contiguous(), "row_orders: (n, K) int32 contiguous maps expected");
      ptrs[j] = (const int32_t*)t.data_ptr();
      ns[j] = (int32_t)t.size(0);
      ks[j] = (int32_t)t.size(1);
      total += t.size(0);
      if (!keys.empty() && keys[base + j].defined()) {
        const Tensor& k = keys[base + j];
        need(k.scalar_type() == at::kInt && k.is_contiguous() && k.numel() == t.size(0), "row_orders: keys must be (n) int32 contiguous");
        kptrs[j] = (const int32_t*)k.data_ptr();
      }
    }
    Tensor order = at::empty({total > 0 ? total : 1}, maps[base].options());
    chk(btc_row_orders_keyed(ptrs.data(), kptrs.data(), ns.data(), ks.data(), (int)m, (int32_t*)order.data_ptr(), st(stream)), "btc_row_orders_keyed");
    int64_t off = 0;
    for (size_t j = 0; j < m; ++j) {
      out[base + j] = order.narrow(0, off, ns[j]);
      off += ns[j];
    }
  }
  return out;
}

Tensor rulebook_subm(const Tensor& indices, int64_t batch, int64_t p_in, int64_t p_k, int64_t p_d, int64_t K, int64_t stream) {
  const int64_t n = indices.size(0);
  Tensor nbr = at::empty({n, K}, indices.options());
  const size_t ws_bytes = btc_rulebook_subm_ws_bytes((int)n);
  Tensor ws = at::empty({(int64_t)(ws_bytes > 256 ? ws_bytes : 256)}, indices.options().dtype(at::kByte));
  chk(btc_rulebook_subm((const int32_t*)indices.data_ptr(), (int)n, (int)batch, ip(p_in), ip(p_k), ip(p_d), (int32_t*)nbr.data_ptr(), nullptr,
                        ws.data_ptr(), ws_bytes, st(stream)), "btc_rulebook_subm");
  return nbr;
}

std::tuple<Tensor, Tensor, Tensor, Tensor, Tensor> rulebook_conv(const Tensor& indices, int64_t batch, int64_t p_in, int64_t p_out, int64_t p_k, int64_t p_s,
                                                 int64_t p_p, int64_t p_d, int64_t mode, int64_t K, int64_t ws_bytes, int64_t stream) {
  const int64_t n = indices.size(0);
  Tensor ws = at::empty({ws_bytes > 256 ? ws_bytes : 256}, indices.options().dtype(at::kByte));
  Tensor d_n = at::empty({1}, indices.options());
  chk(btc_rulebook_conv_count((const int32_t*)indices.data_ptr(), (int)n, (int)batch, ip(p_in), ip(p_out), ip(p_k), ip(p_s), ip(p_p), ip(p_d),
                              (int)mode, (int32_t*)d_n.data_ptr(), ws.data_ptr(), (size_t)ws_bytes, st(stream)), "btc_rulebook_conv_count");
  const int64_t n_out = d_n.item<int32_t>();
  Tensor out_indices = at::empty({n_out, 4}, indices.options());
  Tensor nbr_out = at::empty({n_out, K}, indices.options());
  Tensor nbr_in = at::empty({n, K}, indices.options());
  chk(btc_rulebook_conv_fill((const int32_t*)indices.data_ptr(), (int)n, (int)batch, ip(p_in), ip(p_out), ip(p_k), ip(p_s), ip(p_p), ip(p_d),
                             (int)mode, (int)n_out, (int32_t*)out_indices.data_ptr(), (int32_t*)nbr_out.data_ptr(), (int32_t*)nbr_in.data_ptr(),
                             ws.data_ptr(), (size_t)ws_bytes, st(stream)), "btc_rulebook_conv_fill");
  auto ord = row_orders({nbr_out, nbr_in}, stream);
  return std::make_tuple(out_indices, nbr_out, nbr_in, ord[0], ord[1]);
}

inline int64_t current_stream() { return reinterpret_cast<int64_t>(c10::hip::getCurrentHIPStream().stream()); }

struct ConvBNReLUNode : public torch::autograd::Function<ConvBNReLUNode> {
  static Tensor forward(torch::autograd::AutogradContext* ctx, const Tensor& features, const Tensor& weight, const OptTensor& bias,
                        const Tensor& map_fwd, const Tensor& map_bwd, const OptTensor& order_fwd, const OptTensor& order_bwd,
                        const OptTensor& gamma, const OptTensor& beta, const OptTensor& rm, const OptTensor& rv, const OptTensor& nbt,
                        bool use_batch, double momentum, double eps, bool relu, const Tensor& ws, int64_t ws_bytes, bool overlap,
                        bool allow_defer) {
    const int64_t stream = current_stream();
    auto r = conv_bn_fwd(features, weight, bias, map_fwd, order_fwd, gamma, beta, rm, rv, nbt, use_batch, momentum, eps, relu, ws, ws_bytes, stream);
    const Tensor g = (gamma.has_value() && gamma->defined()) ? *gamma : Tensor();
    const Tensor ob = (order_bwd.has_value() && order_bwd->defined()) ? *order_bwd : Tensor();
    ctx->save_for_backward({features, weight, map_fwd, map_bwd, std::get<0>(r), std::get<1>(r), g, std::get<2>(r), ws, ob});
    ctx->saved_data["use_batch"] = use_batch;
    ctx->saved_data["relu"] = relu;
    ctx->saved_data["ws_bytes"] = ws_bytes;
    ctx->saved_data["overlap"] = overlap;
    ctx->saved_data["allow_defer"] = allow_defer;
    ctx->saved_data["has_bias"] = bias.has_value() && bias->defined();
    return std::get<1>(r);
  }

  static torch::autograd::variable_list backward(torch::autograd::AutogradContext* ctx, torch::autograd::variable_list grads) {
    const auto saved = ctx->get_saved_variables();
    const Tensor &features = saved[0], &w = saved[1], &map_fwd = saved[2], &map_bwd = saved[3], &x = saved[4], &y = saved[5], &gamma = saved[6],
                 &stats = saved[7], &ws = saved[8];
    const bool use_batch = ctx->saved_data["use_batch"].toBool(), relu = ctx->saved_data["relu"].toBool();
    const int64_t ws_bytes = ctx->saved_data["ws_bytes"].toInt(), stream = current_stream();
    Tensor dy = grads[0];
    if (dy.scalar_type() != x.scalar_type()) dy = dy.to(x.scalar_type());
    dy = dy.contiguous();
    OptTensor og;
    if (gamma.defined()) og = gamma;
    auto b = bn_bwd(x, y, dy, og, stats, use_batch, relu, ws, ws_bytes, stream);
    const Tensor& dx = std::get<0>(b);
    const Tensor& dparam = std::get<1>(b);
    OptTensor order_bwd;
    if (saved[9].defined()) order_bwd = saved[9];
    auto cb = conv_bwd(features, w, map_fwd, map_bwd, order_bwd, dx, ctx->needs_input_grad(0), ctx->needs_input_grad(1),
                       ctx->saved_data["overlap"].toBool(), ctx->saved_data["allow_defer"].toBool(), stream);
    Tensor din = std::get<0>(cb).has_value() ? *std::get<0>(cb) : Tensor();
    Tensor dw = std::get<1>(cb).has_value() ? *std::get<1>(cb) : Tensor();
    Tensor db;
    if (ctx->saved_data["has_bias"].toBool() && ctx->needs_input_grad(2)) {
      db = at::empty({dx.size(1)}, dx.options().dtype(at::kFloat));
      if (dx.scalar_type() == at::kBFloat16)
        chk(btc_col_sum_bf16(dx.data_ptr(), (int)dx.size(0), (int)dx.size(1), (float*)db.data_ptr(), ws.data_ptr(), (size_t)ws_bytes, st(stream)),
            "btc_col_sum_bf16");
      else
        chk(btc_col_sum((const float*)dx.data_ptr(), (int)dx.size(0), (int)dx.size(1), (float*)db.data_ptr(), ws.data_ptr(), (size_t)ws_bytes,
                        st(stream)), "btc_col_sum");
    }
    Tensor dgamma, dbeta;
    if (gamma.defined()) {
      dgamma = dparam[0];
      dbeta = dparam[1];
    }
    return {din, dw, db, Tensor(), Tensor(), Tensor(), Tensor(), dgamma, dbeta, Tensor(), Tensor(), Tensor(), Tensor(), Tensor(), Tensor(), Tensor(), Tensor(), Tensor(),
            Tensor(), Tensor()};
  }
};

Tensor conv_bn_relu(const Tensor& features, const Tensor& weight, const OptTensor& bias, const Tensor& map_fwd, const Tensor& map_bwd,
                    const OptTensor& order_fwd, const OptTensor& order_bwd, const OptTensor& gamma, const OptTensor& beta, const OptTensor& rm, const OptTensor& rv, const OptTensor& nbt, bool use_batch,
                    double momentum, double eps, bool relu, const Tensor& ws, int64_t ws_bytes, bool overlap, bool allow_defer) {
  if (eval_fold_wanted(features, weight, bias, map_fwd, gamma, beta, rm, rv, use_batch))
    return conv_bn_eval_fold(features, weight, bias, map_fwd, order_fwd, gamma, beta, *rm, *rv, eps, relu, current_stream());
  return ConvBNReLUNode::apply(features, weight, bias, map_fwd, map_bwd, order_fwd, order_bwd, gamma, beta, rm, rv, nbt, use_batch, momentum, eps, relu, ws, ws_bytes,
                               overlap, allow_defer);
}

struct WalkSide {
  hipStream_t side = nullptr;
  c10::hip::HIPStream* c10side = nullptr;
  hipEvent_t fork[8] = {}, done[8] = {};
  int32_t* host_counts = nullptr;
  std::atomic<unsigned> next{0};
};

WalkSide& walk_of(int device) {
  static WalkSide tab[64];
  static std::mutex mu;
  WalkSide& w = tab[device & 63];
  std::lock_guard<std::mutex> lock(mu);
  if (!w.side) {
    static std::vector<c10::hip::HIPStream> keep;
    keep.reserve(64);
    keep.push_back(c10::hip::getStreamFromPool(false, (c10::DeviceIndex)device));
    bool ok = hipHostMalloc((void**)&w.host_counts, 8 * BTC_CHAIN_MAX_LAYERS * sizeof(int32_t), hipHostMallocDefault) == hipSuccess;
    for (int i = 0; ok && i < 8; ++i)
      ok = hipEventCreateWithFlags(&w.fork[i], sync_event_flags()) == hipSuccess &&
           hipEventCreateWithFlags(&w.done[i], hipEventDisableTiming) == hipSuccess;
    if (!ok) throw std::runtime_error("geometry walk: event / pinned-memory setup failed");
    w.c10side = &keep.back();
    w.side = keep.back().stream();
  }
  return w;
}

struct PendingWalk {
  Tensor indices, ws, d_counts, h_counts;
  std::vector<Tensor> out_idx;
  std::vector<BtcChainLayer> layers;
  std::vector<int64_t> kind, K, ref;
  size_t wsb = 0;
  int n0 = 0;
  int64_t batch = 0;
  bool side = false;
  hipEvent_t done = nullptr;
  const int32_t* counts = nullptr;
};

std::shared_ptr<PendingWalk> geometry_walk_start(const Tensor& indices, int64_t batch, const std::vector<int64_t>& kind,
                                                 const std::vector<int64_t>& a_in, const std::vector<int64_t>& a_out,
                                                 const std::vector<int64_t>& a_k, const std::vector<int64_t>& a_s,
                                                 const std::vector<int64_t>& a_p, const std::vector<int64_t>& a_d,
                                                 const std::vector<int64_t>& mode, const std::vector<int64_t>& K,
                                                 const std::vector<int64_t>& ws_bytes, const std::vector<int64_t>& ref, int64_t side_mode) {
  need(side_mode == 0 || side_mode == 1, "geometry_walk_start: side_mode must be 0 or 1");
  const bool side = side_mode == 1;
  const size_t n = kind.size();
  need(a_in.size() == n && a_out.size() == n && a_k.size() == n && a_s.size() == n && a_p.size() == n && a_d.size() == n && mode.size() == n &&
           K.size() == n && ws_bytes.size() == n && ref.size() == n, "geometry_walk: per-layer argument lists differ in length");
  need(n >= 1 && n <= BTC_CHAIN_MAX_LAYERS, "geometry_walk: too many layers for one chain");
  auto p = std::make_shared<PendingWalk>();
  p->indices = indices; p->batch = batch; p->kind = kind; p->K = K; p->ref = ref; p->side = side;
  p->n0 = (int)indices.size(0);
  p->layers.resize(n);
  for (size_t i = 0; i < n; ++i) {
    BtcChainLayer& l = p->layers[i];
    l.kind = (int32_t)kind[i];
    l.ref = (int32_t)ref[i];
    l.mode = (int32_t)mode[i];
    for (int j = 0; j < 3; ++j) {
      const bool built = kind[i] < 2;
      l.in_shape[j] = built ? ip(a_in[i])[j] : 1;
      l.out_shape[j] = built ? (kind[i] == 1 ? ip(a_out[i])[j] : ip(a_in[i])[j]) : 1;
      l.k[j] = built ? ip(a_k[i])[j] : 1;
      l.s[j] = (built && kind[i] == 1) ? ip(a_s[i])[j] : 1;
      l.p[j] = (built && kind[i] == 1) ? ip(a_p[i])[j] : 0;
      l.d[j] = built ? ip(a_d[i])[j] : 1;
    }
  }
  std::vector<int64_t> cap(n, 0);
  chk(btc_chain_caps(p->layers.data(), (int)n, (int)batch, p->n0, cap.data()), "btc_chain_caps");
  p->wsb = btc_chain_ws_bytes(p->layers.data(), (int)n, (int)batch, p->n0);
  need(p->wsb > 0, "geometry_walk: btc_chain_ws_bytes failed");
  p->ws = at::empty({(int64_t)p->wsb}, indices.options().dtype(at::kByte));
  p->d_counts = at::empty({(int64_t)n}, indices.options());
  p->out_idx.resize(n);
  std::vector<int32_t*> p_out_idx(n, nullptr);
  for (size_t i = 0; i < n; ++i)
    if (kind[i] == 1) {
      p->out_idx[i] = at::empty({cap[i], 4}, indices.options());
      p_out_idx[i] = (int32_t*)p->out_idx[i].data_ptr();
    }
  hipStream_t main = (hipStream_t)st(current_stream());
  hipStream_t run = main;
  WalkSide* w = nullptr;
  int slot = 0;
  if (side) {
    w = &walk_of(indices.get_device());
    slot = (int)(w->next.fetch_add(1) & 7u);
  }
  if (side) {
    run = w->side;
    if (hipEventRecord(w->fork[slot], main) != hipSuccess || hipStreamWaitEvent(run, w->fork[slot], 0) != hipSuccess)
      throw std::runtime_error("geometry walk: fork failed");
    for (const Tensor* t : {&p->ws, &p->d_counts, &p->indices}) c10::hip::HIPCachingAllocator::recordStream(t->storage().data_ptr(), *w->c10side);
    for (const Tensor& t : p->out_idx)
      if (t.defined()) c10::hip::HIPCachingAllocator::recordStream(t.storage().data_ptr(), *w->c10side);
  }
  chk(btc_chain_levels((const int32_t*)indices.data_ptr(), p->n0, (int)batch, p->layers.data(), (int)n, p_out_idx.data(), cap.data(),
                       (int32_t*)p->d_counts.data_ptr(), p->ws.data_ptr(), p->wsb, (void*)run), "btc_chain_levels");
  if (side) {
    int32_t* host = w->host_counts + slot * BTC_CHAIN_MAX_LAYERS;
    if (hipMemcpyAsync(host, p->d_counts.data_ptr(), n * sizeof(int32_t), hipMemcpyDeviceToHost, run) != hipSuccess ||
        hipEventRecord(w->done[slot], run) != hipSuccess)
      throw std::runtime_error("geometry walk: read-back enqueue failed");
    p->done = w->done[slot];
    p->counts = host;
  } else {
    p->h_counts = p->d_counts.to(at::kCPU);
    p->counts = (const int32_t*)p->h_counts.data_ptr();
  }
  return p;
}

std::vector<std::vector<Tensor>> geometry_walk_finish(const std::shared_ptr<PendingWalk>& p, const std::vector<int64_t>& skip_maps) {
  const size_t n = p->kind.size();
  const std::vector<int64_t>&kind = p->kind, &K = p->K, &ref = p->ref;
  const Tensor& indices = p->indices;
  const int64_t stream = current_stream();
  if (p->side) {
    if (hipEventSynchronize(p->done) != hipSuccess || hipStreamWaitEvent((hipStream_t)st(stream), p->done, 0) != hipSuccess)
      throw std::runtime_error("geometry walk: join failed");
    const c10::hip::HIPStream cur = c10::hip::getCurrentHIPStream();
    for (const Tensor* t : {&p->ws, &p->d_counts, &p->indices}) c10::hip::HIPCachingAllocator::recordStream(t->storage().data_ptr(), cur);
    for (const Tensor& t : p->out_idx)
      if (t.defined()) c10::hip::HIPCachingAllocator::recordStream(t.storage().data_ptr(), cur);
  }
  int32_t hc_copy[BTC_CHAIN_MAX_LAYERS];
  for (size_t i = 0; i < n; ++i) hc_copy[i] = p->counts[i];
  const int32_t* hc = hc_copy;
  std::vector<char> skip(n, 0);
  for (int64_t i : skip_maps) {
    need(i >= 0 && (size_t)i < n && kind[i] == 0, "geometry_walk: only built submanifold layers can skip their maps");
    skip[i] = 1;
  }
  std::vector<Tensor> level_in(n), level_out(n);
  std::vector<int32_t*> p_out_idx(n, nullptr), p_nbr_out(n, nullptr), p_nbr_in(n, nullptr);
  Tensor cur = indices;
  int64_t strided_elems = 0, other_elems = 0;
  for (size_t i = 0; i < n; ++i) {
    if (kind[i] == 0) {
      level_in[i] = level_out[i] = cur;
      if (!skip[i]) other_elems += cur.size(0) * K[i];
    } else if (kind[i] == 1) {
      level_in[i] = cur;
      p_out_idx[i] = (int32_t*)p->out_idx[i].data_ptr();
      cur = p->out_idx[i].narrow(0, 0, hc[i]);
      level_out[i] = cur;
      strided_elems += (int64_t)hc[i] * K[i];
      other_elems += level_in[i].size(0) * K[i];
    } else {
      need(ref[i] >= 0 && (size_t)ref[i] < i, "geometry_walk: bad layer reference");
      cur = kind[i] == 2 ? level_in[ref[i]] : level_out[ref[i]];
      level_in[i] = kind[i] == 2 ? level_out[ref[i]] : level_in[ref[i]];
      level_out[i] = cur;
    }
  }
  Tensor buf_s = at::empty({strided_elems > 0 ? strided_elems : 1}, indices.options());
  Tensor buf_o = at::empty({other_elems > 0 ? other_elems : 1}, indices.options());
  int64_t off_s = 0, off_o = 0;
  std::vector<std::vector<Tensor>> out(n);
  constexpr int order_mode = 1;
  auto wants_order = [&](size_t i) {
    return !skip[i] && K[i] <= 64 && ((kind[i] == 1 && order_mode >= 1) || (kind[i] == 0 && order_mode >= 2));
  };
  int64_t key_elems = 0;
  for (size_t i = 0; i < n; ++i)
    if (kind[i] == 1 && wants_order(i)) key_elems += level_in[i].size(0) + level_out[i].size(0);
  Tensor buf_k = at::empty({key_elems > 0 ? key_elems : 1}, indices.options());
  int64_t off_k = 0;
  std::vector<int32_t*> p_first_out(n, nullptr), p_first_in(n, nullptr);
  std::vector<Tensor> key_out(n), key_in(n);
  for (size_t i = 0; i < n; ++i) {
    if (kind[i] > 1 || skip[i]) continue;
    const int64_t rows_in = level_in[i].size(0), rows_out = level_out[i].size(0);
    Tensor nbr_out, nbr_in;
    if (kind[i] == 1) {
      nbr_out = buf_s.narrow(0, off_s, rows_out * K[i]).view({rows_out, K[i]});
      off_s += rows_out * K[i];
    } else {
      nbr_out = buf_o.narrow(0, off_o, rows_out * K[i]).view({rows_out, K[i]});
      off_o += rows_out * K[i];
    }
    p_nbr_out[i] = (int32_t*)nbr_out.data_ptr();
    if (kind[i] == 1) {
      nbr_in = buf_o.narrow(0, off_o, rows_in * K[i]).view({rows_in, K[i]});
      off_o += rows_in * K[i];
      p_nbr_in[i] = (int32_t*)nbr_in.data_ptr();
      if (wants_order(i)) {
        key_in[i] = buf_k.narrow(0, off_k, rows_in);
        off_k += rows_in;
        p_first_in[i] = (int32_t*)key_in[i].data_ptr();
        key_out[i] = buf_k.narrow(0, off_k, rows_out);
        off_k += rows_out;
        p_first_out[i] = (int32_t*)key_out[i].data_ptr();
      }
    } else {
      nbr_in = nbr_out;
    }
    out[i] = {level_in[i], level_out[i], nbr_out, nbr_in};
  }
  chk(btc_chain_maps((const int32_t*)indices.data_ptr(), p->n0, (int)p->batch, p->layers.data(), (int)n, hc, p_out_idx.data(), p_nbr_out.data(),
                     p_nbr_in.data(), p_first_out.data(), p_first_in.data(), p->ws.data_ptr(), p->wsb, st(stream)), "btc_chain_maps");
  std::vector<Tensor> to_order, to_order_keys;
  for (size_t i = 0; i < n; ++i)
    if (wants_order(i)) {
      to_order.push_back(out[i][2]);
      to_order_keys.push_back(key_out[i]);
      to_order.push_back(out[i][3]);
      to_order_keys.push_back(key_in[i]);
    }
  if (!to_order.empty()) {
    auto ord = row_orders_keyed(to_order, to_order_keys, stream);
    size_t q = 0;
    for (size_t i = 0; i < n; ++i)
      if (wants_order(i)) {
        out[i].push_back(ord[q++]);
        out[i].push_back(ord[q++]);
      }
  }
  return out;
}

std::vector<std::vector<Tensor>> geometry_walk(const Tensor& indices, int64_t batch, const std::vector<int64_t>& kind,
                                               const std::vector<int64_t>& a_in, const std::vector<int64_t>& a_out,
                                               const std::vector<int64_t>& a_k, const std::vector<int64_t>& a_s,
                                               const std::vector<int64_t>& a_p, const std::vector<int64_t>& a_d,
                                               const std::vector<int64_t>& mode, const std::vector<int64_t>& K,
                                               const std::vector<int64_t>& ws_bytes, const std::vector<int64_t>& ref) {
  return geometry_walk_finish(geometry_walk_start(indices, batch, kind, a_in, a_out, a_k, a_s, a_p, a_d, mode, K, ws_bytes, ref, 0), {});
}

Tensor conv_bn_relu_chain(const Tensor& features, const std::vector<Tensor>& weights, const std::vector<OptTensor>& biases,
                          const std::vector<Tensor>& map_fwd, const std::vector<Tensor>& map_bwd, const std::vector<OptTensor>& order_fwd,
                          const std::vector<OptTensor>& order_bwd, const std::vector<OptTensor>& gammas,
                          const std::vector<OptTensor>& betas, const std::vector<OptTensor>& rms, const std::vector<OptTensor>& rvs,
                          const std::vector<OptTensor>& nbts, const std::vector<bool>& use_batch, const std::vector<double>& momenta,
                          const std::vector<double>& epss, const std::vector<bool>& relus, const Tensor& ws, const std::vector<int64_t>& ws_bytes,
                          const std::vector<bool>& overlaps, const std::vector<bool>& allow_defers) {
  const size_t L = weights.size();
  need(L >= 1 && biases.size() == L && map_fwd.size() == L && map_bwd.size() == L && order_fwd.size() == L && order_bwd.size() == L && gammas.size() == L && betas.size() == L && rms.size() == L &&
           rvs.size() == L && nbts.size() == L && use_batch.size() == L && momenta.size() == L && epss.size() == L && relus.size() == L &&
           ws_bytes.size() == L && overlaps.size() == L && allow_defers.size() == L,
       "conv_bn_relu_chain: per-layer argument lists differ in length");
  Tensor x = features;
  for (size_t i = 0; i < L; ++i) {
    if (eval_fold_wanted(x, weights[i], biases[i], map_fwd[i], gammas[i], betas[i], rms[i], rvs[i], use_batch[i])) {
      x = conv_bn_eval_fold(x, weights[i], biases[i], map_fwd[i], order_fwd[i], gammas[i], betas[i], *rms[i], *rvs[i], epss[i], relus[i], current_stream());
      continue;
    }
    x = ConvBNReLUNode::apply(x, weights[i], biases[i], map_fwd[i], map_bwd[i], order_fwd[i], order_bwd[i], gammas[i], betas[i], rms[i], rvs[i], nbts[i], use_batch[i],
                              momenta[i], epss[i], relus[i], ws, ws_bytes[i], overlaps[i], allow_defers[i]);
  }
  return x;
}

void adam_group_step(const std::vector<Tensor>& params, const std::vector<Tensor>& grads, const Tensor& chunk_seg, const Tensor& chunk_off,
                     const Tensor& chunk_len, const Tensor& chunk_flat, const std::vector<int64_t>& seg_chunk0, const Tensor& flat_p,
                     const Tensor& flat_m, const Tensor& flat_v, int64_t step, double lr, double beta1, double beta2, double eps, double weight_decay,
                     double clip, const Tensor& ws, int64_t stream) {
  const size_t n = params.size();
  need(grads.size() == n && seg_chunk0.size() == n + 1, "adam_group_step: list lengths differ");
  std::vector<const float*> ptrs(n);
  std::vector<int32_t> sc(n + 1);
  for (size_t i = 0; i < n; ++i) {
    const Tensor& g = grads[i];
    need(g.defined() && g.is_contiguous() && g.scalar_type() == at::kFloat && g.numel() == params[i].numel() && g.get_device() == flat_p.get_device(),
         "adam_group_step: every gradient must be a contiguous fp32 tensor of its parameter's size on the parameters' device");
    ptrs[i] = (const float*)g.data_ptr();
    sc[i] = (int32_t)seg_chunk0[i];
  }
  sc[n] = (int32_t)seg_chunk0[n];
  chk(btc_adam_group_step(ptrs.data(), (int)n, (const int32_t*)chunk_seg.data_ptr(), (const int32_t*)chunk_off.data_ptr(),
                          (const int32_t*)chunk_len.data_ptr(), (const int64_t*)chunk_flat.data_ptr(), sc.data(), (int)chunk_seg.numel(),
                          (float*)flat_p.data_ptr(), (float*)flat_m.data_ptr(), (float*)flat_v.data_ptr(), (long long)step, (float)lr, (float)beta1,
                          (float)beta2, (float)eps, (float)weight_decay, (float)clip, ws.data_ptr(), (size_t)ws.numel(), st(stream)),
      "btc_adam_group_step");
  for (size_t i = 0; i < n; ++i) params[i].unsafeGetTensorImpl()->bump_version();
}

struct ParamList {
  std::vector<Tensor> p;
};

std::shared_ptr<ParamList> make_param_list(const std::vector<Tensor>& params) {
  auto pl = std::make_shared<ParamList>();
  pl->p = params;
  return pl;
}

bool adam_group_step_pl(const std::shared_ptr<ParamList>& pl, const Tensor& chunk_seg, const Tensor& chunk_off, const Tensor& chunk_len,
                        const Tensor& chunk_flat, const std::vector<int64_t>& seg_chunk0, const Tensor& flat_p, const Tensor& flat_m,
                        const Tensor& flat_v, int64_t step, double lr, double beta1, double beta2, double eps, double weight_decay, double clip,
                        const Tensor& ws, int64_t stream) {
  const size_t n = pl->p.size();
  std::vector<Tensor> grads(n);
  for (size_t i = 0; i < n; ++i) {
    const Tensor& g = pl->p[i].grad();
    if (!(g.defined() && g.is_contiguous() && g.scalar_type() == at::kFloat && g.numel() == pl->p[i].numel() && g.get_device() == flat_p.get_device()))
      return false;
    grads[i] = g;
  }
  adam_group_step(pl->p, grads, chunk_seg, chunk_off, chunk_len, chunk_flat, seg_chunk0, flat_p, flat_m, flat_v, step, lr, beta1, beta2, eps,
                  weight_decay, clip, ws, stream);
  return true;
}

void clear_grads_pl(const std::shared_ptr<ParamList>& pl) {
  for (Tensor& t : pl->p) t.mutable_grad().reset();
}

void pack_grads(const std::vector<Tensor>& grads, const Tensor& chunk_seg, const Tensor& chunk_off, const Tensor& chunk_len, const Tensor& chunk_flat,
                const std::vector<int64_t>& seg_chunk0, const std::vector<int64_t>& sizes, const Tensor& flat, int64_t stream) {
  const size_t n = grads.size();
  need(seg_chunk0.size() == n + 1 && sizes.size() == n, "pack_grads: list lengths differ");
  std::vector<const float*> ptrs(n);
  std::vector<int32_t> sc(n + 1);
  for (size_t i = 0; i < n; ++i) {
    const Tensor& g = grads[i];
    need(g.defined() && g.is_contiguous() && g.scalar_type() == at::kFloat && g.numel() == sizes[i] && g.get_device() == flat.get_device(),
         "pack_grads: every gradient must be a contiguous fp32 tensor of its parameter's size on the bucket's device");
    ptrs[i] = (const float*)g.data_ptr();
    sc[i] = (int32_t)seg_chunk0[i];
  }
  sc[n] = (int32_t)seg_chunk0[n];
  chk(btc_grads_pack(ptrs.data(), (int)n, (const int32_t*)chunk_seg.data_ptr(), (const int32_t*)chunk_off.data_ptr(), (const int32_t*)chunk_len.data_ptr(),
                     (const int64_t*)chunk_flat.data_ptr(), sc.data(), (float*)flat.data_ptr(), st(stream)), "btc_grads_pack");
}

}

PYBIND11_MODULE(TORCH_EXTENSION_NAME, m) {
  m.doc() = "compiled PyTorch binding of libbtcdet_hip.so's hot entry points";
  m.def("split_weights", &split_weights, py::call_guard<py::gil_scoped_release>());
  m.def("bf16_weights", &bf16_weights, py::call_guard<py::gil_scoped_release>());
  m.def("conv_fwd", &conv_fwd, py::call_guard<py::gil_scoped_release>());
  m.def("bn_fwd", &bn_fwd, py::call_guard<py::gil_scoped_release>());
  m.def("conv_bn_fwd", &conv_bn_fwd, py::call_guard<py::gil_scoped_release>());
  m.def("conv_bn_eval_fold", &conv_bn_eval_fold, py::call_guard<py::gil_scoped_release>());
  m.def("eval_fold_calls", &eval_fold_calls);
  m.def("bn_bwd", &bn_bwd, py::call_guard<py::gil_scoped_release>());
  m.def("conv_bwd", &conv_bwd, py::call_guard<py::gil_scoped_release>());
  m.def("conv_bn_relu", &conv_bn_relu, py::call_guard<py::gil_scoped_release>());
  m.def("row_orders", &row_orders, py::call_guard<py::gil_scoped_release>());
  m.def("geometry_walk", &geometry_walk, py::call_guard<py::gil_scoped_release>());
  py::class_<PendingWalk, std::shared_ptr<PendingWalk>>(m, "PendingWalk");
  m.def("geometry_walk_start", &geometry_walk_start, py::call_guard<py::gil_scoped_release>());
  m.def("geometry_walk_finish", &geometry_walk_finish, py::call_guard<py::gil_scoped_release>());
  m.def("conv_bn_relu_chain", &conv_bn_relu_chain, py::call_guard<py::gil_scoped_release>());
  m.def("pack_grads", &pack_grads, py::call_guard<py::gil_scoped_release>());
  m.def("adam_group_step", &adam_group_step, py::call_guard<py::gil_scoped_release>());
  py::class_<ParamList, std::shared_ptr<ParamList>>(m, "ParamList");
  m.def("make_param_list", &make_param_list);
  m.def("adam_group_step_pl", &adam_group_step_pl, py::call_guard<py::gil_scoped_release>());
  m.def("clear_grads_pl", &clear_grads_pl);
  m.def("join_wgrad", &join_wgrad, py::call_guard<py::gil_scoped_release>());
  m.def("set_defer_wgrad_join", &set_defer_wgrad_join);
  m.def("set_side_stream", &set_side_stream);
  m.def("rulebook_subm", &rulebook_subm, py::call_guard<py::gil_scoped_release>());
  m.def("rulebook_conv", &rulebook_conv, py::call_guard<py::gil_scoped_release>());
  m.def("abi_version", []() { return btc_version(); });
}
```

### btcdet_amd/csrc/bn.hip

```cpp
#include "btc_common.h"
#include "bn_fuse.h"
#include "../../include/btcdet_hip_infer.h"

#include <type_traits>

namespace {

constexpr int BN_T = 256;

struct BnShape {
  int N, C, cpow, rpi;
};

__device__ __forceinline__ void st_partial(double* p, double v) { btc_st_agent(p, v); }

template <bool BF, int W>
__device__ __forceinline__ void bn_ld(const float* base, long long i, float (&e)[W]) {
  if constexpr (W == 4) {
    const float4 v = btc_ld4<BF>(base, i);
    e[0] = v.x; e[1] = v.y; e[2] = v.z; e[3] = v.w;
  } else {
    e[0] = btc_ld1<BF>(base, i);
  }
}

template <int W, int Q, int P, class Fill, class Emit>
__device__ __forceinline__ void bn_pass(const BnShape& S, double (&s)[Q][P], Fill fill, Emit emit) {
  const int tid = threadIdx.x;
  for (int c0 = 0; c0 < S.C; c0 += S.cpow) {
    const int cw = c0 + (tid % S.cpow), rr = tid / S.cpow;
    double acc[Q][W];
#pragma unroll
    for (int q = 0; q < Q; ++q)
#pragma unroll
      for (int j = 0; j < W; ++j) acc[q][j] = 0.0;
    if (cw < S.C) fill(cw, rr, acc);
#pragma unroll
    for (int j = 0; j < W; ++j)
#pragma unroll
      for (int q = 0; q < Q; ++q) s[q][tid * W + j] = acc[q][j];
    __syncthreads();
    if (rr == 0 && cw < S.C) {
      for (int l = 1; l < S.rpi; ++l)
#pragma unroll
        for (int j = 0; j < W; ++j)
#pragma unroll
          for (int q = 0; q < Q; ++q) acc[q][j] += s[q][(tid + l * S.cpow) * W + j];
      emit(cw, acc);
    }
    __syncthreads();
  }
}

template <int W, int Q, int D, class Rows, class Done>
__device__ __forceinline__ bool bn_reduce(const BnShape& S, const BnShape& SW, double* __restrict__ partial, int32_t* __restrict__ counter,
                                          Rows rows, Done done) {
  __shared__ double s[Q][BN_T * W];
  const int G = (int)gridDim.x;
  auto at = [&](int g, int q, int c) { return &partial[((size_t)g * Q + q) * S.C + c]; };
  bn_pass<W>(SW, s,
             [&](int cw, int rr, double (&acc)[Q][W]) { rows(cw, (long long)blockIdx.x * SW.rpi + rr, (long long)G * SW.rpi, acc); },
             [&](int cw, double (&acc)[Q][W]) {
#pragma unroll
               for (int j = 0; j < W; ++j)
#pragma unroll
                 for (int q = 0; q < Q; ++q) st_partial(at(blockIdx.x, q, cw * W + j), acc[q][j]);
             });
  if (!btc_last_arriver(counter, G)) return false;
  bn_pass<1>(S, s,
             [&](int c, int rr, double (&acc)[Q][1]) {
               int g = rr;
               for (; g + (D - 1) * S.rpi < G; g += D * S.rpi) {
                 double v[Q][D];
#pragma unroll
                 for (int u = 0; u < D; ++u)
#pragma unroll
                   for (int q = 0; q < Q; ++q) v[q][u] = btc_ld_agent(at(g + u * S.rpi, q, c));
#pragma unroll
                 for (int q = 0; q < Q; ++q) {
#pragma unroll
                   for (int h = 1; h < D; h *= 2)
#pragma unroll
                     for (int u = 0; u < D; u += 2 * h) v[q][u] += v[q][u + h];
                   acc[q][0] += v[q][0];
                 }
               }
               for (; g < G; g += S.rpi)
#pragma unroll
                 for (int q = 0; q < Q; ++q) acc[q][0] += btc_ld_agent(at(g, q, c));
             },
             [&](int c, double (&acc)[Q][1]) {
               double t[Q];
#pragma unroll
               for (int q = 0; q < Q; ++q) t[q] = acc[q][0];
               done(c, t);
             });
  if (threadIdx.x == 0) __hip_atomic_store(counter, 0, __ATOMIC_RELAXED, __HIP_MEMORY_SCOPE_AGENT);
  return true;
}

template <bool BF, bool VEC>
__global__ __launch_bounds__(BN_T) void bn_stats(const float* __restrict__ x, BnShape S, BnShape SW, double* __restrict__ partial,
                                                 int32_t* __restrict__ counter, float momentum, float eps, float* __restrict__ running_mean,
                                                 float* __restrict__ running_var, long long* __restrict__ num_batches,
                                                 float* __restrict__ mean_out, float* __restrict__ rstd_out) {
  constexpr int W = VEC ? 4 : 1;
  const bool last = bn_reduce<W, 2, 8>(
      S, SW, partial, counter,
      [&](int cw, long long r, long long stride, double (&acc)[2][W]) {
        const long long step = stride * S.C;
        long long i = r * S.C + cw * W;
        for (; r + 3 * stride < S.N; r += 4 * stride, i += 4 * step) {
          float e0[W], e1[W], e2[W], e3[W];
          bn_ld<BF>(x, i, e0);
          bn_ld<BF>(x, i + step, e1);
          bn_ld<BF>(x, i + 2 * step, e2);
          bn_ld<BF>(x, i + 3 * step, e3);
          __builtin_amdgcn_sched_barrier(0);
#pragma unroll
          for (int j = 0; j < W; ++j) {
            acc[0][j] += (double)e0[j] + (double)e1[j] + (double)e2[j] + (double)e3[j];
            acc[1][j] += (double)e0[j] * e0[j] + (double)e1[j] * e1[j] + (double)e2[j] * e2[j] + (double)e3[j] * e3[j];
          }
        }
        for (; r < S.N; r += stride, i += step) {
          float e[W];
          bn_ld<BF>(x, i, e);
#pragma unroll
          for (int j = 0; j < W; ++j) { acc[0][j] += e[j]; acc[1][j] += (double)e[j] * e[j]; }
        }
      },
      [&](int c, const double (&t)[2]) {
        double mean = t[0] / S.N;
        double var = t[1] / S.N - mean * mean;
        if (var < 0.0) var = 0.0;
        mean_out[c] = (float)mean;
        rstd_out[c] = (float)(1.0 / sqrt(var + (double)eps));
        if (running_mean) {
          double unb = S.N > 1 ? var * ((double)S.N / (double)(S.N - 1)) : var;
          running_mean[c] = (float)((1.0 - momentum) * running_mean[c] + momentum * mean);
          running_var[c] = (float)((1.0 - momentum) * running_var[c] + momentum * unb);
        }
      });
  if (last && threadIdx.x == 0 && num_batches) *num_batches += 1;
}

__global__ __launch_bounds__(BN_T) void bn_eval_stats(const float* __restrict__ running_mean, const float* __restrict__ running_var,
                                                      int C, float eps, float* __restrict__ mean_out, float* __restrict__ rstd_out) {
  int c = blockIdx.x * blockDim.x + threadIdx.x;
  if (c >= C) return;
  mean_out[c] = running_mean[c];
  rstd_out[c] = bn_rstd_eval(running_var[c], eps);
}

template <bool VEC, bool BF>
__global__ __launch_bounds__(BN_T) void bn_apply(const float* __restrict__ x, const float* __restrict__ mean, const float* __restrict__ rstd,
                                                 const float* __restrict__ gamma, const float* __restrict__ beta, long long total, int C,
                                                 int relu, float* __restrict__ y) {
  long long i = ((long long)blockIdx.x * blockDim.x + threadIdx.x) * (VEC ? 4 : 1);
  if (i >= total) return;
  if (VEC) {
    int c = (int)(i % C);
    float4 v = btc_ld4<BF>(x, i);
    float o[4] = {v.x, v.y, v.z, v.w};
#pragma unroll
    for (int j = 0; j < 4; ++j) {
      float g = gamma ? gamma[c + j] : 1.f, b = beta ? beta[c + j] : 0.f;
      o[j] = bn_affine(o[j], mean[c + j], rstd[c + j], g, b, relu);
    }
    btc_st4<BF>(y, i, o[0], o[1], o[2], o[3]);
  } else {
    int c = (int)(i % C);
    float g = gamma ? gamma[c] : 1.f, b = beta ? beta[c] : 0.f;
    btc_st1<BF>(y, i, bn_affine(btc_ld1<BF>(x, i), mean[c], rstd[c], g, b, relu));
  }
}

template <bool BF, bool VEC>
__global__ __launch_bounds__(BN_T) void bn_bwd_stats(const float* __restrict__ x, const float* __restrict__ y, const float* __restrict__ dy,
                                                     const float* __restrict__ mean, const float* __restrict__ rstd, BnShape S, BnShape SW, int relu,
                                                     double* __restrict__ partial, int32_t* __restrict__ counter,
                                                     float* __restrict__ dgamma, float* __restrict__ dbeta) {
  constexpr int W = VEC ? 4 : 1, U = VEC ? 2 : 4;
  bn_reduce<W, 2, 8>(
      S, SW, partial, counter,
      [&](int cw, long long r, long long stride, double (&acc)[2][W]) {
        float m[W], rs[W];
#pragma unroll
        for (int j = 0; j < W; ++j) { m[j] = mean[cw * W + j]; rs[j] = rstd[cw * W + j]; }
        const long long step = stride * S.C;
        long long i = r * S.C + cw * W;
        for (; r + (U - 1) * stride < S.N; r += U * stride, i += U * step) {
          float gv[U][W], yv[U][W], xv[U][W];
#pragma unroll
          for (int u = 0; u < U; ++u) {
            bn_ld<BF>(dy, i + u * step, gv[u]);
            bn_ld<BF>(y, i + u * step, yv[u]);
            bn_ld<BF>(x, i + u * step, xv[u]);
          }
#pragma unroll
          for (int u = 0; u < U; ++u)
#pragma unroll
            for (int j = 0; j < W; ++j) {
              const float g = (relu && !(yv[u][j] > 0.f)) ? 0.f : gv[u][j];
              acc[0][j] += (double)g;
              acc[1][j] += (double)g * ((xv[u][j] - m[j]) * rs[j]);
            }
        }
        for (; r < S.N; r += stride, i += step) {
          float gv[W], yv[W], xv[W];
          bn_ld<BF>(dy, i, gv);
          bn_ld<BF>(y, i, yv);
          bn_ld<BF>(x, i, xv);
#pragma unroll
          for (int j = 0; j < W; ++j) {
            const float g = (relu && !(yv[j] > 0.f)) ? 0.f : gv[j];
            acc[0][j] += (double)g;
            acc[1][j] += (double)g * ((xv[j] - m[j]) * rs[j]);
          }
        }
      },
      [&](int c, const double (&t)[2]) {
        dbeta[c] = (float)t[0];
        dgamma[c] = (float)t[1];
      });
}

template <bool VEC, bool BF>
__global__ __launch_bounds__(BN_T) void bn_bwd_apply(const float* __restrict__ x, const float* __restrict__ y, const float* __restrict__ dy,
                                                     const float* __restrict__ mean, const float* __restrict__ rstd,
                                                     const float* __restrict__ gamma, const float* __restrict__ dgamma,
                                                     const float* __restrict__ dbeta, long long total, int C, int N, int relu, int training,
                                                     float* __restrict__ dx) {
  long long i = ((long long)blockIdx.x * blockDim.x + threadIdx.x) * (VEC ? 4 : 1);
  if (i >= total) return;
  const float invn = 1.0f / (float)N;
  constexpr int W = VEC ? 4 : 1;
  float xv[W], yv[W], gv[W];
  if (VEC) {
    float4 a = btc_ld4<BF>(x, i), b = btc_ld4<BF>(y, i), c4 = btc_ld4<BF>(dy, i);
    xv[0] = a.x; xv[W > 1 ? 1 : 0] = a.y; xv[W > 2 ? 2 : 0] = a.z; xv[W > 3 ? 3 : 0] = a.w;
    yv[0] = b.x; yv[W > 1 ? 1 : 0] = b.y; yv[W > 2 ? 2 : 0] = b.z; yv[W > 3 ? 3 : 0] = b.w;
    gv[0] = c4.x; gv[W > 1 ? 1 : 0] = c4.y; gv[W > 2 ? 2 : 0] = c4.z; gv[W > 3 ? 3 : 0] = c4.w;
  } else {
    xv[0] = btc_ld1<BF>(x, i); yv[0] = btc_ld1<BF>(y, i); gv[0] = btc_ld1<BF>(dy, i);
  }
  const int c = (int)(i % C);
  float o[W];
#pragma unroll
  for (int j = 0; j < W; ++j) {
    float g = gv[j];
    if (relu && !(yv[j] > 0.f)) g = 0.f;
    const float gm = gamma ? gamma[c + j] : 1.f, rs = rstd[c + j];
    if (training) {
      float xh = (xv[j] - mean[c + j]) * rs;
      o[j] = gm * rs * (g - dbeta[c + j] * invn - xh * dgamma[c + j] * invn);
    } else {
      o[j] = gm * rs * g;
    }
  }
  if (VEC) btc_st4<BF>(dx, i, o[0], o[W > 1 ? 1 : 0], o[W > 2 ? 2 : 0], o[W > 3 ? 3 : 0]);
  else btc_st1<BF>(dx, i, o[0]);
}

template <bool BF>
__global__ __launch_bounds__(BN_T) void col_sum(const float* __restrict__ x, BnShape S, double* __restrict__ partial,
                                                int32_t* __restrict__ counter, float* __restrict__ out) {
  bn_reduce<1, 1, 1>(
      S, S, partial, counter,
      [&](int c, long long r, long long stride, double (&acc)[1][1]) {
        for (; r + 3 * stride < S.N; r += 4 * stride) {
          float v0 = btc_ld1<BF>(x, r * S.C + c), v1 = btc_ld1<BF>(x, (r + stride) * S.C + c), v2 = btc_ld1<BF>(x, (r + 2 * stride) * S.C + c),
                v3 = btc_ld1<BF>(x, (r + 3 * stride) * S.C + c);
          acc[0][0] += ((double)v0 + (double)v1) + ((double)v2 + (double)v3);
        }
        for (; r < S.N; r += stride) acc[0][0] += (double)btc_ld1<BF>(x, r * S.C + c);
      },
      [&](int c, const double (&t)[1]) { out[c] = (float)t[0]; });
}

BnShape bn_shape(int N, int C) {
  BnShape S;
  S.N = N;
  S.C = C;
  int cp = 1;
  while (cp < C && cp < BN_T) cp <<= 1;
  S.cpow = cp;
  S.rpi = BN_T / cp;
  return S;
}

int bn_grid_bwd(int N, const BnShape& S) {
  int g = btc_cdiv(N, S.rpi * 16);
  if (g > 512) g = 512;
  if (g < 1) g = 1;
  return g;
}

int bn_grid(int N, const BnShape& S) {
  int g = btc_cdiv(N, S.rpi * 64);
  if (g > 256) g = 256;
  if (g < 1) g = 1;
  return g;
}

int bn_grid_bytes(long long bytes, int tune_key, int kb_default) {
  const int t = btc_tune_get(tune_key);
  const long long per = 1024LL * (t > 0 ? t : kb_default);
  long long g = (bytes + per - 1) / per;
  return (int)(g > 256 ? 256 : (g < 1 ? 1 : g));
}

struct BnWs {
  int32_t* counter;
  double* partial;
  explicit BnWs(void* ws) : counter((int32_t*)ws), partial((double*)((char*)ws + 256)) {}
};

template <class F>
int bn_by_width(int N, int C, F&& f) {
  if ((C & 3) == 0) return f(std::integral_constant<int, 4>(), bn_shape(N, C >> 2));
  return f(std::integral_constant<int, 1>(), bn_shape(N, C));
}

}

extern "C" size_t btc_bn_ws_bytes(int C) { return 256 + btc_align((size_t)512 * 2 * C * sizeof(double)); }

template <bool BF>
static int bn_fwd_impl(const float* x, int N, int C, const float* gamma, const float* beta, float* running_mean,
                               float* running_var, long long* num_batches_tracked, float momentum, float eps, int training, int relu,
                               float* y, float* save_mean, float* save_rstd, void* ws_, size_t ws_bytes, void* stream_, bool have_stats = false) {
  hipStream_t stream = (hipStream_t)stream_;
  BTC_CHECK_ARG(N >= 1 && C >= 1, "btc_bn_relu_fwd: empty input");
  BTC_CHECK_ARG(ws_bytes >= btc_bn_ws_bytes(C), "btc_bn_relu_fwd: workspace too small");
  BTC_CHECK_ARG(training || (running_mean && running_var), "btc_bn_relu_fwd: eval mode needs running statistics");
  const BnWs ws(ws_);
  const BnShape S = bn_shape(N, C);
  const long long total = (long long)N * C;
  return bn_by_width(N, C, [&](auto w, const BnShape& SW) {
    constexpr int W = decltype(w)::value;
    if (!have_stats && training) {
      const int g = W == 4 ? bn_grid_bytes(total * (BF ? 2 : 4), BTC_TUNE_BN_FWD_KB, 64) : bn_grid(N, S);
      bn_stats<BF, W == 4><<<g, BN_T, 0, stream>>>(x, S, SW, ws.partial, ws.counter, momentum, eps, running_mean, running_var,
                                                    num_batches_tracked, save_mean, save_rstd);
    } else if (!have_stats) {
      bn_eval_stats<<<btc_cdiv(C, BN_T), BN_T, 0, stream>>>(running_mean, running_var, C, eps, save_mean, save_rstd);
    }
    BTC_LAUNCH_CHECK();
    bn_apply<W == 4, BF><<<btc_cdiv(total / W, BN_T), BN_T, 0, stream>>>(x, save_mean, save_rstd, gamma, beta, total, C, relu, y);
    BTC_LAUNCH_CHECK();
    return BTC_OK;
  });
}

template <bool BF>
static int bn_bwd_impl(const float* x, const float* y, const float* dy, int N, int C, const float* gamma, const float* save_mean,
                               const float* save_rstd, int training, int relu, float* dx, float* dgamma, float* dbeta, void* ws_,
                               size_t ws_bytes, void* stream_) {
  hipStream_t stream = (hipStream_t)stream_;
  BTC_CHECK_ARG(N >= 1 && C >= 1, "btc_bn_relu_bwd: empty input");
  BTC_CHECK_ARG(ws_bytes >= btc_bn_ws_bytes(C), "btc_bn_relu_bwd: workspace too small");
  const BnWs ws(ws_);
  const BnShape S = bn_shape(N, C);
  const long long total = (long long)N * C;
  return bn_by_width(N, C, [&](auto w, const BnShape& SW) {
    constexpr int W = decltype(w)::value;
    const int g = W == 4 ? bn_grid_bytes(total * (BF ? 6 : 12), BTC_TUNE_BN_BWD_KB, 128) : bn_grid_bwd(N, S);
    bn_bwd_stats<BF, W == 4><<<g, BN_T, 0, stream>>>(x, y, dy, save_mean, save_rstd, S, SW, relu, ws.partial, ws.counter, dgamma, dbeta);
    BTC_LAUNCH_CHECK();
    bn_bwd_apply<W == 4, BF><<<btc_cdiv(total / W, BN_T), BN_T, 0, stream>>>(x, y, dy, save_mean, save_rstd, gamma, dgamma, dbeta, total, C, N,
                                                                             relu, training, dx);
    BTC_LAUNCH_CHECK();
    return BTC_OK;
  });
}

template <bool BF>
static int col_sum_impl(const float* x, int N, int C, float* out, void* ws_, size_t ws_bytes, void* stream_) {
  hipStream_t stream = (hipStream_t)stream_;
  BTC_CHECK_ARG(N >= 1 && C >= 1, "btc_col_sum: empty input");
  BTC_CHECK_ARG(ws_bytes >= btc_bn_ws_bytes(C), "btc_col_sum: workspace too small");
  const BnWs ws(ws_);
  const BnShape S = bn_shape(N, C);
  col_sum<BF><<<bn_grid_bwd(N, S), BN_T, 0, stream>>>(x, S, ws.partial, ws.counter, out);
  BTC_LAUNCH_CHECK();
  return BTC_OK;
}

extern "C" int btc_col_sum(const float* x, int N, int C, float* out, void* ws, size_t ws_bytes, void* stream) {
  return col_sum_impl<false>(x, N, C, out, ws, ws_bytes, stream);
}

extern "C" int btc_col_sum_bf16(const void* x, int N, int C, float* out, void* ws, size_t ws_bytes, void* stream) {
  return col_sum_impl<true>((const float*)x, N, C, out, ws, ws_bytes, stream);
}

extern "C" int btc_bn_relu_fwd(const float* x, int N, int C, const float* gamma, const float* beta, float* running_mean,
                               float* running_var, long long* num_batches_tracked, float momentum, float eps, int training, int relu,
                               float* y, float* save_mean, float* save_rstd, void* ws, size_t ws_bytes, void* stream) {
  return bn_fwd_impl<false>(x, N, C, gamma, beta, running_mean, running_var, num_batches_tracked, momentum, eps, training, relu, y, save_mean,
                            save_rstd, ws, ws_bytes, stream);
}

extern "C" int btc_bn_relu_bwd(const float* x, const float* y, const float* dy, int N, int C, const float* gamma, const float* save_mean,
                               const float* save_rstd, int training, int relu, float* dx, float* dgamma, float* dbeta, void* ws,
                               size_t ws_bytes, void* stream) {
  return bn_bwd_impl<false>(x, y, dy, N, C, gamma, save_mean, save_rstd, training, relu, dx, dgamma, dbeta, ws, ws_bytes, stream);
}

extern "C" int btc_bn_relu_fwd_bf16(const void* x, int N, int C, const float* gamma, const float* beta, float* running_mean,
                                    float* running_var, long long* num_batches_tracked, float momentum, float eps, int training, int relu,
                                    void* y, float* save_mean, float* save_rstd, void* ws, size_t ws_bytes, void* stream) {
  return bn_fwd_impl<true>((const float*)x, N, C, gamma, beta, running_mean, running_var, num_batches_tracked, momentum, eps, training, relu,
                           (float*)y, save_mean, save_rstd, ws, ws_bytes, stream);
}

extern "C" int btc_bn_relu_bwd_bf16(const void* x, const void* y, const void* dy, int N, int C, const float* gamma, const float* save_mean,
                                    const float* save_rstd, int training, int relu, void* dx, float* dgamma, float* dbeta, void* ws,
                                    size_t ws_bytes, void* stream) {
  return bn_bwd_impl<true>((const float*)x, (const float*)y, (const float*)dy, N, C, gamma, save_mean, save_rstd, training, relu, (float*)dx,
                           dgamma, dbeta, ws, ws_bytes, stream);
}

extern "C" size_t btc_bn_fuse_ws_bytes(void) { return btc_bn_fuse_bytes(); }

extern "C" int btc_conv_bn_relu_fwd(int operands, const void* src, const void* W, const float* bias, const int32_t* nbr, const int32_t* order,
                                    int n_rows, int K, int Cin, int Cout, void* x, const float* gamma, const float* beta, float* running_mean,
                                    float* running_var, long long* num_batches_tracked, float momentum, float eps, int relu, void* y,
                                    float* save_mean, float* save_rstd, void* ws, size_t ws_bytes, void* fuse_ws, void* stream) {
  return btc_conv_bn_relu_fwd_src(operands, src, -1LL, W, bias, nbr, order, n_rows, K, Cin, Cout, x, gamma, beta, running_mean, running_var,
                                  num_batches_tracked, momentum, eps, relu, y, save_mean, save_rstd, ws, ws_bytes, fuse_ws, stream);
}

extern "C" int btc_conv_bn_relu_fwd_src(int operands, const void* src, long long src_rows, const void* W, const float* bias, const int32_t* nbr,
                                        const int32_t* order, int n_rows, int K, int Cin, int Cout, void* x, const float* gamma, const float* beta,
                                        float* running_mean, float* running_var, long long* num_batches_tracked, float momentum, float eps, int relu,
                                        void* y, float* save_mean, float* save_rstd, void* ws, size_t ws_bytes, void* fuse_ws, void* stream) {
  BTC_CHECK_ARG(n_rows >= 1, "btc_conv_bn_relu_fwd: empty input");
  BTC_CHECK_ARG(operands >= BTC_OPERANDS_F32 && operands <= BTC_OPERANDS_F32_SPLIT, "btc_conv_bn_relu_fwd: operands=%d", operands);
  const bool bf = operands == BTC_OPERANDS_BF16_ACT || operands == BTC_OPERANDS_BF16;
  const bool fused = fuse_ws && Cout <= BN_FUSE_CMAX && btc_tune_get(BTC_TUNE_BN_FUSE) != 1;
  BnFuse bn = btc_bn_fuse_none();
  if (fused) {
    bn.counter = (int32_t*)fuse_ws;
    bn.slots = (double*)((char*)fuse_ws + 256);
    bn.mean_out = save_mean; bn.rstd_out = save_rstd;
    bn.running_mean = running_mean; bn.running_var = running_var; bn.num_batches = num_batches_tracked;
    bn.momentum = momentum; bn.eps = eps; bn.N = n_rows; bn.C = Cout; bn.nslots = btc_bn_fuse_nslots(n_rows);
  }
  const int rc = btc_apply("btc_conv_bn_relu_fwd_src", BTC_PASS_FWD, operands, src, src_rows, W, bias, nbr, order, n_rows, K, Cin, Cout, x,
                           (hipStream_t)stream, fused ? &bn : nullptr);
  if (rc) return rc;
  if (bf)
    return bn_fwd_impl<true>((const float*)x, n_rows, Cout, gamma, beta, running_mean, running_var, num_batches_tracked, momentum, eps, 1, relu,
                             (float*)y, save_mean, save_rstd, ws, ws_bytes, stream, fused);
  return bn_fwd_impl<false>((const float*)x, n_rows, Cout, gamma, beta, running_mean, running_var, num_batches_tracked, momentum, eps, 1, relu,
                            (float*)y, save_mean, save_rstd, ws, ws_bytes, stream, fused);
}

extern "C" int btc_conv_bn_eval_fwd(int operands, const void* src, long long src_rows, const void* W, const float* bias, const int32_t* nbr,
                                    const int32_t* order, int n_rows, int K, int Cin, int Cout, const float* gamma, const float* beta,
                                    const float* running_mean, const float* running_var, float eps, int relu, void* y, void* stream) {
  BTC_CHECK_ARG(n_rows >= 1, "btc_conv_bn_eval_fwd: empty input");
  BTC_CHECK_ARG(operands >= BTC_OPERANDS_F32 && operands <= BTC_OPERANDS_F32_SPLIT, "btc_conv_bn_eval_fwd: operands=%d", operands);
  BTC_CHECK_ARG(running_mean && running_var, "btc_conv_bn_eval_fwd: eval mode needs running statistics");
  BTC_CHECK_ARG(src && W && nbr && y, "btc_conv_bn_eval_fwd: null operand");
  BnFuse bn = btc_bn_fuse_none();
  bn.ev_mean = running_mean; bn.ev_var = running_var; bn.ev_gamma = gamma; bn.ev_beta = beta; bn.ev_relu = relu ? 1 : 0;
  bn.eps = eps; bn.N = n_rows; bn.C = Cout;
  return btc_apply("btc_conv_bn_eval_fwd", BTC_PASS_FWD, operands, src, src_rows, W, bias, nbr, order, n_rows, K, Cin, Cout, y, (hipStream_t)stream, &bn);
}
```

### btcdet_amd/spconv/modules.py

```python
from collections import OrderedDict

from torch import nn

from .tensor import SparseConvTensor


import torch as _torch

nn_float32 = _torch.float32
FUSE_CONV_BN = True
CHAIN_LAYERS = True
FUSE_BN_RELU = True


class SparseModule(nn.Module):
    pass


def is_spconv_module(module):
    return isinstance(module, SparseModule)


def is_sparse_conv(module):
    from .conv import SparseConvolution
    return isinstance(module, SparseConvolution)


class SparseSequential(SparseModule):
    def __init__(self, *args, **kwargs):
        super(SparseSequential, self).__init__()
        if len(args) == 1 and isinstance(args[0], OrderedDict):
            for key, module in args[0].items():
                self.add_module(key, module)
        else:
            for idx, module in enumerate(args):
                self.add_module(str(idx), module)
        for name, module in kwargs.items():
            if name in self._modules:
                raise ValueError("name exists.")
            self.add_module(name, module)
        self._sparity_dict = {}

    def __getitem__(self, idx):
        if not (-len(self) <= idx < len(self)):
            raise IndexError('index {} is out of range'.format(idx))
        if idx < 0:
            idx += len(self)
        it = iter(self._modules.values())
        for _ in range(idx):
            next(it)
        return next(it)

    def __len__(self):
        return len(self._modules)

    @property
    def sparity_dict(self):
        return self._sparity_dict

    def add(self, module, name=None):
        if name is None:
            name = str(len(self._modules))
            if name in self._modules:
                raise KeyError("name exists")
        self.add_module(name, module)

    def forward_geometry(self, input):
        for module in self._modules.values():
            if is_spconv_module(module):
                input = module.forward_geometry(input)
        return input

    def _flat_modules(self):
        out = []
        for m in self._modules.values():
            if type(m) is SparseSequential:
                out.extend(m._flat_modules())
            else:
                out.append(m)
        return out

    def _triples(self):
        triples = self.__dict__.get("_chain_triples", False)
        if triples is False:
            from . import ops
            from .conv import SparseConvolution
            mods = self._flat_modules()
            triples, i = [], 0
            while i < len(mods):
                conv = mods[i]
                bn = mods[i + 1] if i + 1 < len(mods) else None
                if not (isinstance(conv, SparseConvolution) and not conv.conv1x1 and conv.ndim == 3 and isinstance(bn, nn.BatchNorm1d)) \
                        or ops.pads_in_channels(conv.in_channels):
                    triples = None
                    break
                relu = i + 2 < len(mods) and type(mods[i + 2]) is nn.ReLU
                triples.append((conv, bn, relu))
                i += 2 + int(relu)
            self.__dict__["_chain_triples"] = triples
        return triples

    def _chain_plan(self, input, rulebooks=None):
        from . import fused_bn, ops
        f = input.features
        if not (FUSE_CONV_BN and FUSE_BN_RELU and CHAIN_LAYERS and ops.PROFILE is None and ops.CAPTURE is None and ops.NATIVE_AUTOGRAD
                and f is not None and f.is_cuda and f.shape[0] > 0 and f.dtype in (nn_float32, _torch.bfloat16) and ops.fast() is not None):
            return None
        triples = self._triples()
        if not triples or (rulebooks is not None and len(rulebooks) != len(triples)):
            return None
        plan = []
        indices, shape = input.indices, input.spatial_shape
        geom = input.indice_dict.get("__geometry_cache__", None) if rulebooks is None else None
        for i, (conv, bn, relu) in enumerate(triples):
            if not fused_bn.fusable(bn):
                return None
            if f.dtype == _torch.bfloat16 and (conv.in_channels % 16 or conv.out_channels % 16):
                return None
            if rulebooks is not None:
                rb = rulebooks[i]
            else:
                rb = input.indice_dict.get(conv.indice_key, None) if conv.indice_key is not None else None
                if rb is None and not conv.inverse and geom is not None:
                    hit = geom.get(conv._gkey(indices, shape), None)
                    rb = hit[0] if hit is not None else None
            if rb is None or (rb.n_in if conv.inverse else rb.n_out) == 0:
                return None
            if conv.inverse:
                indices, shape = rb.in_indices, rb.in_shape[3 - conv.ndim:]
            else:
                indices, shape = rb.out_indices, rb.out_shape
            plan.append((conv, bn, relu, rb, conv.inverse))
        return plan, indices, shape

    def _run_chain(self, input, plan, indices, shape):
        from . import fused_bn, ops
        F = ops.fast()
        key = tuple((bn.training, bn.track_running_stats, id(conv.weight), id(conv.bias), id(bn.weight), id(bn.bias), id(bn.running_mean),
                     id(bn.running_var), id(bn.num_batches_tracked), conv.weight.device) for conv, bn, _, _, _ in plan)
        st = self.__dict__.get("_chain_static")
        if st is None or st[0] != key:
            w, b, ga, be, rms, rvs, nbts, ub, mom, eps, relus, need, dfr = ([] for _ in range(13))
            for conv, bn, relu, rb, inverse in plan:
                training = bn.training or not bn.track_running_stats
                rm = bn.running_mean if bn.track_running_stats else None
                w.append(ops._f32c(conv.weight)); b.append(conv.bias)
                ga.append(bn.weight); be.append(bn.bias); rms.append(rm); rvs.append(bn.running_var if bn.track_running_stats else None)
                nbts.append(bn.num_batches_tracked if (bn.training and bn.track_running_stats) else None)
                ub.append(bool(training or rm is None)); mom.append(float(bn.momentum)); eps.append(float(bn.eps)); relus.append(bool(relu))
                need.append(int(fused_bn._ws(input.features.device, conv.weight.shape[-1])[1])); dfr.append(bool(conv.weight.is_leaf))
            st = self.__dict__["_chain_static"] = (key, (w, b, ga, be, rms, rvs, nbts, ub, mom, eps, relus, need, dfr))
        w, b, ga, be, rms, rvs, nbts, ub, mom, eps, relus, need, dfr = st[1]
        mf, mb, of, ob, ov = [], [], [], [], []
        for conv, bn, relu, rb, inverse in plan:
            if inverse:
                mf.append(rb.nbr_in); mb.append(rb.nbr_out); of.append(rb.order_in); ob.append(rb.order_out)
            else:
                mf.append(rb.nbr_out); mb.append(rb.map_bwd); of.append(rb.order_out); ob.append(rb.order_in)
            ov.append(bool(ops._overlap_ok(mf[-1].shape[0])))
        ws = fused_bn._ws(input.features.device, max(wt.shape[-1] for wt in w))[0]
        out = F.conv_bn_relu_chain(ops._actc(input.features), w, b, mf, mb, of, ob, ga, be, rms, rvs, nbts, ub, mom, eps, relus, ws, need, ov, dfr)
        out_tensor = SparseConvTensor(out, indices, shape, input.batch_size)
        out_tensor.indice_dict = input.indice_dict
        out_tensor.grid = input.grid
        return out_tensor

    def forward(self, input):
        from . import fused_bn
        from .conv import SparseConvolution
        if isinstance(input, SparseConvTensor):
            plan = self._chain_plan(input)
            if plan is not None:
                return self._run_chain(input, *plan)
        mods = list(self._modules.values())
        i = 0
        while i < len(mods):
            module = mods[i]
            i += 1
            if is_spconv_module(module):
                assert isinstance(input, SparseConvTensor)
                nxt = mods[i] if i < len(mods) else None
                f = input.features
                if FUSE_CONV_BN and FUSE_BN_RELU and nxt is not None and isinstance(module, SparseConvolution) and fused_bn.fusable(nxt) and f.is_cuda \
                        and f.dtype in (nn_float32, _torch.bfloat16) and f.shape[0] != 0:
                    relu = i + 1 < len(mods) and type(mods[i + 1]) is nn.ReLU
                    input = module(input, fuse_bn=(nxt, relu))
                    i += 1 + int(relu)
                else:
                    input = module(input)
            else:
                if isinstance(input, SparseConvTensor):
                    f = input.features
                    if fused_bn.is_sync(module) and f is not None and f.is_cuda and f.dtype in (nn_float32, _torch.bfloat16) and f.dim() == 2:
                        relu = i < len(mods) and type(mods[i]) is nn.ReLU
                        input.features = fused_bn.sync_batch_norm_relu(module, f, relu)
                        i += int(relu)
                    elif input.indices.shape[0] != 0:
                        if FUSE_BN_RELU and fused_bn.fusable(module) and f.is_cuda and f.dtype in (nn_float32, _torch.bfloat16) and f.dim() == 2:
                            relu = i < len(mods) and type(mods[i]) is nn.ReLU
                            input.features = fused_bn.batch_norm_relu(module, f, relu)
                            i += int(relu)
                        else:
                            input.features = module(f)
                    elif isinstance(module, nn.SyncBatchNorm) and module.training and f is not None and f.is_cuda:
                        input.features = module(f)
                else:
                    input = module(input)
        return input
```

Baseline: 584.5.

## Write combine-branch BN outputs directly into concat buffer slices

Result: no change. 593.0 (median of 4 runs) (+1.5%).

```diff
diff --git a/btcdet_amd/_lib.py b/btcdet_amd/_lib.py
--- a/btcdet_amd/_lib.py
+++ b/btcdet_amd/_lib.py
@@ -264,6 +264,16 @@
 
 ROI_TARGETS_EXPORTED_SYMBOLS = tuple(_ROI_TARGETS_SIGS.keys())
 
+ll = ctypes.c_longlong
+_STRIDED_SIGS = {
+    "btc_bn_relu_fwd_ld": (ci, [ci, vp, ci, ci, vp, vp, vp, vp, vp, cf, cf, ci, ci, vp, ll, ci, vp, ll, ci, vp, vp, vp, sz, vp]),
+    "btc_bn_relu_bwd_ld": (ci, [ci, vp, vp, ll, ci, vp, ll, ci, ci, ci, vp, vp, vp, ci, ci, vp, vp, vp, vp, sz, vp]),
+    "btc_conv_bn_relu_fwd_ld": (ci, [ci, vp, ll, vp, vp, vp, vp, ci, ci, ci, ci, vp, vp, vp, vp, vp, vp, cf, cf, ci, vp, ll, ci, vp, ll, ci,
+                                     vp, vp, vp, sz, vp, vp]),
+}
+
+STRIDED_EXPORTED_SYMBOLS = tuple(_STRIDED_SIGS.keys())
+
 
 def lib():
     global _lib
@@ -275,7 +285,7 @@
         L = ctypes.CDLL(LIB_PATH)
         for name, (res, args) in (list(_SIGS.items()) + list(_INFER_SIGS.items()) + list(_AUGMENT_SIGS.items()) + list(_BESTMATCH_SIGS.items()) +
                                   list(_FRAMES_SIGS.items()) + list(_GTDB_SIGS.items()) + list(_TEMPLATES_SIGS.items()) + list(_INFOS_SIGS.items()) + list(_HEADS_SIGS.items()) +
-                                  list(_ANCHOR_LOSS_SIGS.items()) + list(_ROI_TARGETS_SIGS.items())):
+                                  list(_ANCHOR_LOSS_SIGS.items()) + list(_ROI_TARGETS_SIGS.items()) + list(_STRIDED_SIGS.items())):
             fn = getattr(L, name)
             fn.restype = res
             fn.argtypes = args
diff --git a/btcdet_amd/backbones_3d.py b/btcdet_amd/backbones_3d.py
--- a/btcdet_amd/backbones_3d.py
+++ b/btcdet_amd/backbones_3d.py
@@ -163,6 +163,7 @@
         return x
 
 
+INPLACE_COMBINE = True
 DET_GEOMETRY_WALK = True
 FAST_STAGES = True
 
@@ -250,13 +251,29 @@
             return plan, plan.finish(handle, coords, indice_dict, have)
         return None
 
-    def _stage(self, stage, x, ready):
+    def _stage(self, stage, x, ready, y_into=None, keep_dense=False):
         sl = ready[0].stage_slices.get(id(stage)) if ready is not None else None
         if sl is not None:
             chain = stage._chain_plan(x, ready[1][sl[0]:sl[1]])
             if chain is not None:
-                return stage._run_chain(x, *chain)
-        return stage(x)
+                if y_into is None:
+                    return stage._run_chain(x, *chain)
+                bn = chain[0][-1][1]
+                if torch.is_grad_enabled() and (bn.training or not bn.track_running_stats) and y_into.shape[0] == chain[0][-1][3].n_out \
+                        and y_into.dtype == x.features.dtype:
+                    return stage._run_chain(x, *chain, y_into=y_into, keep_dense=keep_dense), True
+                return stage._run_chain(x, *chain), False
+        return stage(x) if y_into is None else (stage(x), False)
+
+    def _combine_slices(self, x, ready):
+        if getattr(self, "down3", None) is None or ready is None or not torch.is_grad_enabled() or not INPLACE_COMBINE:
+            return None
+        buf = torch.empty((x.features.shape[0], sum(self._cat_cols)), dtype=x.features.dtype, device=x.features.device)
+        out, c0 = [buf], 0
+        for w in self._cat_cols:
+            out.append(buf[:, c0:c0 + w])
+            c0 += w
+        return out
 
     def _stages(self, stages, x, ready):
         for stage in stages:
@@ -280,6 +297,7 @@
                            (c[1], c[2], 3, dict(padding=(0, 1, 1), indice_key='spconv4', **sp))], norm_fn)
         self.down3 = _seq([(c[2], c[2], 3, dict(padding=(0, 1, 1), indice_key='spconv4', **sp))], norm_fn)
         cat = c[2] * 2 + c[3]
+        self._cat_cols = (c[2], c[2], c[3]) + ((c[3],) if comb_type == "big_bev_combine" else ())
         if comb_type == "big_combine":
             self.down_combine = _seq([(cat, c[3] * 2, 3, dict(padding=1, indice_key='subm4')),
                                       (c[3] * 2, c[3] * 2, 3, dict(padding=1, indice_key='subm4'))], norm_fn)
@@ -328,16 +346,24 @@
         N, C, D, H, W = d.shape
         return d.view(N, C * D, H, W)
 
-    def res_combine(self, x2, x3, x4, bev, out_feat_type="combine", ready=None):
+    def res_combine(self, x2, x3, x4, bev, out_feat_type="combine", ready=None, slices=None):
         if getattr(self, "down3", None) is None:
             return None
-        x2, x3 = self._stage(self.down2, x2, ready), self._stage(self.down3, x3, ready)
+        if slices is not None and x2.features.shape[0] > 0 and x3.features.shape[0] > 0:
+            (x2, w2), (x3, w3) = self._stage(self.down2, x2, ready, y_into=slices[1]), self._stage(self.down3, x3, ready, y_into=slices[2])
+            if not (w2 and w3):
+                slices = None
+        else:
+            x2, x3, slices = self._stage(self.down2, x2, ready), self._stage(self.down3, x3, ready), None
+        parts = [x2.features, x3.features, x4.features]
         if out_feat_type == "big_bev_combine":
             bev2d = self.compress_height(self._stage(self.squeezeBev, bev, ready))
-            x4.features = torch.cat((x2.features, x3.features, x4.features,
-                                     _BevGather.apply(bev2d, x4.indices, tuple(x4.spatial_shape), x4.batch_size).to(x4.features.dtype)), dim=1)
-        else:
-            x4.features = torch.cat((x2.features, x3.features, x4.features), dim=1)
+            into = slices[4] if slices is not None and bev2d.dtype == slices[4].dtype else None
+            rows = _BevGather.apply(bev2d, x4.indices, tuple(x4.spatial_shape), x4.batch_size, into)
+            if slices is not None and into is None:
+                slices = None
+            parts.append(rows.to(x4.features.dtype))
+        x4.features = _InPlaceCat.apply(slices[0], *parts) if slices is not None else torch.cat(parts, dim=1)
         return self._stage(self.down_combine, x4, ready)
 
     @staticmethod
@@ -395,8 +421,19 @@
                 ready = None
         levels = [x1]
         cur = x1
+        slices = None
         for lvl in (1, 2, 3):
             if not (n_occ > lvl):
+                if lvl == 3:
+                    cur = self._stage(self.conv4, cur, ready)
+                    slices = self._combine_slices(cur, ready) if cur.features.shape[0] > 0 else None
+                    if slices is not None:
+                        cur, wrote = self._stage(self.conv4_combine, cur, ready, y_into=slices[3], keep_dense=True)
+                        slices = slices if wrote else None
+                    else:
+                        cur = self._stage(self.conv4_combine, cur, ready)
+                    levels.append(cur)
+                    continue
                 cur = self._stages([getattr(self, 'conv%d' % (lvl + 1)), getattr(self, 'conv%d_combine' % (lvl + 1))], cur, ready)
                 levels.append(cur)
                 continue
@@ -420,7 +457,7 @@
             'x_conv2': self.suqeeze(x2, 2, self.out_feat_type[1]),
             'x_conv3': self.suqeeze(x3, 3, self.out_feat_type[2]),
             'x_conv4': self.suqeeze(x4, 4, self.out_feat_type[3]),
-            'x_combine': self.res_combine(x2, x3, x4, out, out_feat_type=self.out_feat_type[4], ready=ready),
+            'x_combine': self.res_combine(x2, x3, x4, out, out_feat_type=self.out_feat_type[4], ready=ready, slices=slices),
         }})
         return batch_dict
 
@@ -428,10 +465,12 @@
 class _BevGather(torch.autograd.Function):
 
     @staticmethod
-    def forward(ctx, bev2d, indices, spatial_shape, batch_size):
+    def forward(ctx, bev2d, indices, spatial_shape, batch_size, into=None):
         inds = indices.long()
         ctx.save_for_backward(indices)
         ctx.meta = (spatial_shape, batch_size, bev2d.dtype)
+        if into is not None:
+            return torch.ops.aten.index.Tensor_out(bev2d, [inds[:, 0], None, inds[:, 2], inds[:, 3]], out=into.detach())
         return bev2d[inds[:, 0], :, inds[:, 2], inds[:, 3]]
 
     @staticmethod
@@ -439,7 +478,23 @@
         (indices,) = ctx.saved_tensors
         spatial_shape, batch_size, dtype = ctx.meta
         vol = spconv.SparseConvTensor(grad.contiguous(), indices, list(spatial_shape), batch_size).dense()
-        return vol.sum(2).to(dtype), None, None, None
+        return vol.sum(2).to(dtype), None, None, None, None
+
+
+class _InPlaceCat(torch.autograd.Function):
+
+    @staticmethod
+    def forward(ctx, buf, *parts):
+        ctx.widths = [int(p.shape[1]) for p in parts]
+        return buf.detach()
+
+    @staticmethod
+    def backward(ctx, grad):
+        out, c0 = [None], 0
+        for w in ctx.widths:
+            out.append(grad[:, c0:c0 + w])
+            c0 += w
+        return tuple(out)
 
 
 class SparseBasicBlock(spconv.SparseModule):
diff --git a/btcdet_amd/csrc/binding.cpp b/btcdet_amd/csrc/binding.cpp
--- a/btcdet_amd/csrc/binding.cpp
+++ b/btcdet_amd/csrc/binding.cpp
@@ -18,6 +18,7 @@
 
 #include "../../include/btcdet_hip.h"
 #include "../../include/btcdet_hip_infer.h"
+#include "../../include/btcdet_hip_strided.h"
 
 namespace {
 
@@ -176,10 +177,46 @@
   return f.out;
 }
 
+struct SliceOut {
+  Tensor y;
+  void *p = nullptr, *p2 = nullptr;
+  long long ld = 0, ld2 = 0;
+};
+
+bool is_row_slice(const Tensor& t) { return t.dim() == 2 && (t.size(1) == 1 || t.stride(1) == 1) && t.stride(0) >= t.size(1); }
+
+SliceOut slice_out(const Tensor& like, const OptTensor& into, bool keep_dense) {
+  SliceOut o;
+  const Tensor& t = *into;
+  need(is_row_slice(t) && t.sizes() == like.sizes() && t.scalar_type() == like.scalar_type() && t.get_device() == like.get_device() && !t.requires_grad(),
+       "y_into: an (N, C) slice of the activation type with unit column stride expected");
+  if (keep_dense) {
+    o.y = at::empty_like(like);
+    o.p = o.y.data_ptr(); o.ld = like.size(1);
+    o.p2 = t.data_ptr(); o.ld2 = t.stride(0);
+  } else {
+    o.y = at::empty({0}, like.options()).set_(t.storage(), t.storage_offset(), t.sizes(), t.strides());
+    o.p = t.data_ptr(); o.ld = t.stride(0);
+  }
+  return o;
+}
+
+inline bool has(const OptTensor& t) { return t.has_value() && t->defined(); }
+
 std::tuple<Tensor, Tensor> bn_fwd(const Tensor& x, const OptTensor& gamma, const OptTensor& beta, const OptTensor& rm, const OptTensor& rv,
                                   const OptTensor& nbt, bool use_batch, double momentum, double eps, bool relu, const Tensor& ws, int64_t ws_bytes,
-                                  int64_t stream) {
+                                  int64_t stream, const OptTensor& y_into = c10::nullopt, bool keep_dense = false) {
   const int64_t N = x.size(0), C = x.size(1);
+  if (has(y_into)) {
+    SliceOut o = slice_out(x, y_into, keep_dense);
+    Tensor stats = at::empty({2, C}, x.options().dtype(at::kFloat));
+    float* mean = (float*)stats.data_ptr();
+    long long* nb = has(nbt) ? (long long*)nbt->data_ptr() : nullptr;
+    chk(btc_bn_relu_fwd_ld((int)(x.scalar_type() == at::kBFloat16), x.data_ptr(), (int)N, (int)C, fptr(gamma), fptr(beta), (float*)vptr(rm), (float*)vptr(rv), nb,
+                           (float)momentum, (float)eps, (int)use_batch, (int)relu, o.p, o.ld, 0, o.p2, o.ld2, 0, mean, mean + C, ws.data_ptr(), (size_t)ws_bytes,
+                           st(stream)), "btc_bn_relu_fwd_ld");
+    return std::make_tuple(o.y, stats);
+  }
   Tensor y = at::empty_like(x);
   Tensor stats = at::empty({2, C}, x.options().dtype(at::kFloat));
   float* mean = (float*)stats.data_ptr();
@@ -211,7 +248,21 @@
 std::tuple<Tensor, Tensor, Tensor> conv_bn_fwd(const Tensor& features, const Tensor& w, const OptTensor& bias, const Tensor& map_fwd,
                                                const OptTensor& order_fwd, const OptTensor& gamma, const OptTensor& beta, const OptTensor& rm, const OptTensor& rv,
                                                const OptTensor& nbt, bool use_batch, double momentum, double eps, bool relu, const Tensor& ws,
-                                               int64_t ws_bytes, int64_t stream) {
+                                               int64_t ws_bytes, int64_t stream, const OptTensor& y_into = c10::nullopt, bool keep_dense = false) {
+  if (use_batch && map_fwd.size(0) >= 1 && has(y_into)) {
+    FwdSite f = fwd_site("conv_bn_fwd", features, w, map_fwd, order_fwd);
+    SliceOut o = slice_out(f.out, y_into, keep_dense);
+    Tensor stats = at::empty({2, f.cout}, features.options().dtype(at::kFloat));
+    Tensor fw = fuse_ws_of(features, stream);
+    float* mean = (float*)stats.data_ptr();
+    long long* nb = has(nbt) ? (long long*)nbt->data_ptr() : nullptr;
+    const Operands op = operands_of(features, w, f.K, f.cin, f.cout, f.n_res, BTC_PASS_FWD, stream);
+    chk(btc_conv_bn_relu_fwd_ld(op.operands, features.data_ptr(), (long long)features.size(0), op.w, fptr(bias), (const int32_t*)map_fwd.data_ptr(), f.order,
+                                (int)f.n_res, (int)f.K, (int)f.cin, (int)f.cout, f.out.data_ptr(), fptr(gamma), fptr(beta), (float*)vptr(rm), (float*)vptr(rv), nb,
+                                (float)momentum, (float)eps, (int)relu, o.p, o.ld, 0, o.p2, o.ld2, 0, mean, mean + f.cout, ws.data_ptr(), (size_t)ws_bytes,
+                                fw.data_ptr(), st(stream)), "btc_conv_bn_relu_fwd_ld");
+    return std::make_tuple(f.out, o.y, stats);
+  }
   if (use_batch && map_fwd.size(0) >= 1) {
     FwdSite f = fwd_site("conv_bn_fwd", features, w, map_fwd, order_fwd);
     Tensor y = at::empty_like(f.out);
@@ -227,7 +278,7 @@
     return std::make_tuple(f.out, y, stats);
   }
   Tensor x = conv_fwd(features, w, bias, map_fwd, order_fwd, stream);
-  auto ys = bn_fwd(x, gamma, beta, rm, rv, nbt, use_batch, momentum, eps, relu, ws, ws_bytes, stream);
+  auto ys = bn_fwd(x, gamma, beta, rm, rv, nbt, use_batch, momentum, eps, relu, ws, ws_bytes, stream, y_into, keep_dense);
   return std::make_tuple(x, std::get<0>(ys), std::get<1>(ys));
 }
 
@@ -259,12 +310,18 @@
 std::tuple<Tensor, Tensor> bn_bwd(const Tensor& x, const Tensor& y, const Tensor& dy, const OptTensor& gamma, const Tensor& stats, bool use_batch,
                                   bool relu, const Tensor& ws, int64_t ws_bytes, int64_t stream) {
   const int64_t N = x.size(0), C = x.size(1);
-  need(dy.is_contiguous() && dy.scalar_type() == x.scalar_type(), "bn_bwd: dy must be contiguous and of the activation type");
+  const bool sliced = !dy.is_contiguous() || !y.is_contiguous();
+  need((sliced ? is_row_slice(dy) && is_row_slice(y) && dy.sizes() == x.sizes() : dy.is_contiguous()) && dy.scalar_type() == x.scalar_type(),
+       "bn_bwd: dy must be contiguous, or rows of a wider matrix with unit column stride, and of the activation type");
   Tensor dx = at::empty_like(x);
   Tensor dparam = at::empty({2, C}, x.options().dtype(at::kFloat));
   const float* mean = (const float*)stats.data_ptr();
   float* dgamma = (float*)dparam.data_ptr();
-  if (x.scalar_type() == at::kBFloat16)
+  if (sliced)
+    chk(btc_bn_relu_bwd_ld((int)(x.scalar_type() == at::kBFloat16), x.data_ptr(), y.data_ptr(), (long long)y.stride(0), 0, dy.data_ptr(), (long long)dy.stride(0), 0,
+                           (int)N, (int)C, fptr(gamma), mean, mean + C, (int)use_batch, (int)relu, dx.data_ptr(), dgamma, dgamma + C, ws.data_ptr(), (size_t)ws_bytes,
+                           st(stream)), "btc_bn_relu_bwd_ld");
+  else if (x.scalar_type() == at::kBFloat16)
     chk(btc_bn_relu_bwd_bf16(x.data_ptr(), y.data_ptr(), dy.data_ptr(), (int)N, (int)C, fptr(gamma), mean, mean + C, (int)use_batch, (int)relu,
                              dx.data_ptr(), dgamma, dgamma + C, ws.data_ptr(), (size_t)ws_bytes, st(stream)), "btc_bn_relu_bwd_bf16");
   else
@@ -528,9 +585,10 @@
                         const Tensor& map_fwd, const Tensor& map_bwd, const OptTensor& order_fwd, const OptTensor& order_bwd,
                         const OptTensor& gamma, const OptTensor& beta, const OptTensor& rm, const OptTensor& rv, const OptTensor& nbt,
                         bool use_batch, double momentum, double eps, bool relu, const Tensor& ws, int64_t ws_bytes, bool overlap,
-                        bool allow_defer) {
+                        bool allow_defer, const OptTensor& y_into, bool keep_dense) {
     const int64_t stream = current_stream();
-    auto r = conv_bn_fwd(features, weight, bias, map_fwd, order_fwd, gamma, beta, rm, rv, nbt, use_batch, momentum, eps, relu, ws, ws_bytes, stream);
+    auto r = conv_bn_fwd(features, weight, bias, map_fwd, order_fwd, gamma, beta, rm, rv, nbt, use_batch, momentum, eps, relu, ws, ws_bytes, stream, y_into,
+                         keep_dense);
     const Tensor g = (gamma.has_value() && gamma->defined()) ? *gamma : Tensor();
     const Tensor ob = (order_bwd.has_value() && order_bwd->defined()) ? *order_bwd : Tensor();
     ctx->save_for_backward({features, weight, map_fwd, map_bwd, std::get<0>(r), std::get<1>(r), g, std::get<2>(r), ws, ob});
@@ -551,7 +609,10 @@
     const int64_t ws_bytes = ctx->saved_data["ws_bytes"].toInt(), stream = current_stream();
     Tensor dy = grads[0];
     if (dy.scalar_type() != x.scalar_type()) dy = dy.to(x.scalar_type());
-    dy = dy.contiguous();
+    const int64_t vec = x.scalar_type() == at::kBFloat16 ? 8 : 16;
+    const bool in_place = is_row_slice(dy) && dy.sizes() == x.sizes() &&
+                          ((x.size(1) & 3) != 0 || ((dy.stride(0) & 3) == 0 && (reinterpret_cast<uintptr_t>(dy.data_ptr()) % vec) == 0));
+    if (!in_place) dy = dy.contiguous();
     OptTensor og;
     if (gamma.defined()) og = gamma;
     auto b = bn_bwd(x, y, dy, og, stats, use_batch, relu, ws, ws_bytes, stream);
@@ -579,7 +640,7 @@
       dbeta = dparam[1];
     }
     return {din, dw, db, Tensor(), Tensor(), Tensor(), Tensor(), dgamma, dbeta, Tensor(), Tensor(), Tensor(), Tensor(), Tensor(), Tensor(), Tensor(), Tensor(), Tensor(),
-            Tensor(), Tensor()};
+            Tensor(), Tensor(), Tensor(), Tensor()};
   }
 };
 
@@ -589,7 +650,7 @@
   if (eval_fold_wanted(features, weight, bias, map_fwd, gamma, beta, rm, rv, use_batch))
     return conv_bn_eval_fold(features, weight, bias, map_fwd, order_fwd, gamma, beta, *rm, *rv, eps, relu, current_stream());
   return ConvBNReLUNode::apply(features, weight, bias, map_fwd, map_bwd, order_fwd, order_bwd, gamma, beta, rm, rv, nbt, use_batch, momentum, eps, relu, ws, ws_bytes,
-                               overlap, allow_defer);
+                               overlap, allow_defer, c10::nullopt, false);
 }
 
 struct WalkSide {
@@ -833,7 +894,7 @@
                           const std::vector<OptTensor>& betas, const std::vector<OptTensor>& rms, const std::vector<OptTensor>& rvs,
                           const std::vector<OptTensor>& nbts, const std::vector<bool>& use_batch, const std::vector<double>& momenta,
                           const std::vector<double>& epss, const std::vector<bool>& relus, const Tensor& ws, const std::vector<int64_t>& ws_bytes,
-                          const std::vector<bool>& overlaps, const std::vector<bool>& allow_defers) {
+                          const std::vector<bool>& overlaps, const std::vector<bool>& allow_defers, const OptTensor& y_into, bool keep_dense) {
   const size_t L = weights.size();
   need(L >= 1 && biases.size() == L && map_fwd.size() == L && map_bwd.size() == L && order_fwd.size() == L && order_bwd.size() == L && gammas.size() == L && betas.size() == L && rms.size() == L &&
            rvs.size() == L && nbts.size() == L && use_batch.size() == L && momenta.size() == L && epss.size() == L && relus.size() == L &&
@@ -841,12 +902,14 @@
        "conv_bn_relu_chain: per-layer argument lists differ in length");
   Tensor x = features;
   for (size_t i = 0; i < L; ++i) {
+    const bool last = i + 1 == L;
     if (eval_fold_wanted(x, weights[i], biases[i], map_fwd[i], gammas[i], betas[i], rms[i], rvs[i], use_batch[i])) {
+      need(!(last && has(y_into)), "conv_bn_relu_chain: y_into needs the last layer in training mode");
       x = conv_bn_eval_fold(x, weights[i], biases[i], map_fwd[i], order_fwd[i], gammas[i], betas[i], *rms[i], *rvs[i], epss[i], relus[i], current_stream());
       continue;
     }
     x = ConvBNReLUNode::apply(x, weights[i], biases[i], map_fwd[i], map_bwd[i], order_fwd[i], order_bwd[i], gammas[i], betas[i], rms[i], rvs[i], nbts[i], use_batch[i],
-                              momenta[i], epss[i], relus[i], ws, ws_bytes[i], overlaps[i], allow_defers[i]);
+                              momenta[i], epss[i], relus[i], ws, ws_bytes[i], overlaps[i], allow_defers[i], last ? y_into : OptTensor(), last && keep_dense);
   }
   return x;
 }
@@ -931,8 +994,15 @@
   m.def("split_weights", &split_weights, py::call_guard<py::gil_scoped_release>());
   m.def("bf16_weights", &bf16_weights, py::call_guard<py::gil_scoped_release>());
   m.def("conv_fwd", &conv_fwd, py::call_guard<py::gil_scoped_release>());
-  m.def("bn_fwd", &bn_fwd, py::call_guard<py::gil_scoped_release>());
-  m.def("conv_bn_fwd", &conv_bn_fwd, py::call_guard<py::gil_scoped_release>());
+  m.def("bn_fwd", [](const Tensor& x, const OptTensor& gamma, const OptTensor& beta, const OptTensor& rm, const OptTensor& rv, const OptTensor& nbt, bool use_batch,
+                     double momentum, double eps, bool relu, const Tensor& ws, int64_t ws_bytes, int64_t stream) {
+    return bn_fwd(x, gamma, beta, rm, rv, nbt, use_batch, momentum, eps, relu, ws, ws_bytes, stream);
+  }, py::call_guard<py::gil_scoped_release>());
+  m.def("conv_bn_fwd", [](const Tensor& features, const Tensor& w, const OptTensor& bias, const Tensor& map_fwd, const OptTensor& order_fwd, const OptTensor& gamma,
+                          const OptTensor& beta, const OptTensor& rm, const OptTensor& rv, const OptTensor& nbt, bool use_batch, double momentum, double eps, bool relu,
+                          const Tensor& ws, int64_t ws_bytes, int64_t stream) {
+    return conv_bn_fwd(features, w, bias, map_fwd, order_fwd, gamma, beta, rm, rv, nbt, use_batch, momentum, eps, relu, ws, ws_bytes, stream);
+  }, py::call_guard<py::gil_scoped_release>());
   m.def("conv_bn_eval_fold", &conv_bn_eval_fold, py::call_guard<py::gil_scoped_release>());
   m.def("eval_fold_calls", &eval_fold_calls);
   m.def("bn_bwd", &bn_bwd, py::call_guard<py::gil_scoped_release>());
@@ -943,7 +1013,10 @@
   py::class_<PendingWalk, std::shared_ptr<PendingWalk>>(m, "PendingWalk");
   m.def("geometry_walk_start", &geometry_walk_start, py::call_guard<py::gil_scoped_release>());
   m.def("geometry_walk_finish", &geometry_walk_finish, py::call_guard<py::gil_scoped_release>());
-  m.def("conv_bn_relu_chain", &conv_bn_relu_chain, py::call_guard<py::gil_scoped_release>());
+  m.def("conv_bn_relu_chain", &conv_bn_relu_chain, py::arg("features"), py::arg("weights"), py::arg("biases"), py::arg("map_fwd"), py::arg("map_bwd"),
+        py::arg("order_fwd"), py::arg("order_bwd"), py::arg("gammas"), py::arg("betas"), py::arg("rms"), py::arg("rvs"), py::arg("nbts"), py::arg("use_batch"),
+        py::arg("momenta"), py::arg("epss"), py::arg("relus"), py::arg("ws"), py::arg("ws_bytes"), py::arg("overlaps"), py::arg("allow_defers"),
+        py::arg("y_into") = py::none(), py::arg("keep_dense") = false, py::call_guard<py::gil_scoped_release>());
   m.def("pack_grads", &pack_grads, py::call_guard<py::gil_scoped_release>());
   m.def("adam_group_step", &adam_group_step, py::call_guard<py::gil_scoped_release>());
   py::class_<ParamList, std::shared_ptr<ParamList>>(m, "ParamList");
diff --git a/btcdet_amd/csrc/bn.hip b/btcdet_amd/csrc/bn.hip
--- a/btcdet_amd/csrc/bn.hip
+++ b/btcdet_amd/csrc/bn.hip
@@ -1,6 +1,7 @@
 #include "btc_common.h"
 #include "bn_fuse.h"
 #include "../../include/btcdet_hip_infer.h"
+#include "../../include/btcdet_hip_strided.h"
 
 #include <type_traits>
 
@@ -153,10 +154,16 @@
   rstd_out[c] = bn_rstd_eval(running_var[c], eps);
 }
 
-template <bool VEC, bool BF>
+template <bool LD>
+__device__ __forceinline__ long long bn_at(long long i, int c, int C, long long ld) {
+  if constexpr (LD) return (i / C) * ld + c;
+  return i;
+}
+
+template <bool VEC, bool BF, bool LD>
 __global__ __launch_bounds__(BN_T) void bn_apply(const float* __restrict__ x, const float* __restrict__ mean, const float* __restrict__ rstd,
                                                  const float* __restrict__ gamma, const float* __restrict__ beta, long long total, int C,
-                                                 int relu, float* __restrict__ y) {
+                                                 int relu, float* __restrict__ y, long long ld_y, float* __restrict__ y2, long long ld_y2) {
   long long i = ((long long)blockIdx.x * blockDim.x + threadIdx.x) * (VEC ? 4 : 1);
   if (i >= total) return;
   if (VEC) {
@@ -168,19 +175,22 @@
       float g = gamma ? gamma[c + j] : 1.f, b = beta ? beta[c + j] : 0.f;
       o[j] = bn_affine(o[j], mean[c + j], rstd[c + j], g, b, relu);
     }
-    btc_st4<BF>(y, i, o[0], o[1], o[2], o[3]);
+    btc_st4<BF>(y, bn_at<LD>(i, c, C, ld_y), o[0], o[1], o[2], o[3]);
+    if (LD && y2) btc_st4<BF>(y2, bn_at<LD>(i, c, C, ld_y2), o[0], o[1], o[2], o[3]);
   } else {
     int c = (int)(i % C);
     float g = gamma ? gamma[c] : 1.f, b = beta ? beta[c] : 0.f;
-    btc_st1<BF>(y, i, bn_affine(btc_ld1<BF>(x, i), mean[c], rstd[c], g, b, relu));
+    const float o = bn_affine(btc_ld1<BF>(x, i), mean[c], rstd[c], g, b, relu);
+    btc_st1<BF>(y, bn_at<LD>(i, c, C, ld_y), o);
+    if (LD && y2) btc_st1<BF>(y2, bn_at<LD>(i, c, C, ld_y2), o);
   }
 }
 
-template <bool BF, bool VEC>
+template <bool BF, bool VEC, bool LD>
 __global__ __launch_bounds__(BN_T) void bn_bwd_stats(const float* __restrict__ x, const float* __restrict__ y, const float* __restrict__ dy,
                                                      const float* __restrict__ mean, const float* __restrict__ rstd, BnShape S, BnShape SW, int relu,
                                                      double* __restrict__ partial, int32_t* __restrict__ counter,
-                                                     float* __restrict__ dgamma, float* __restrict__ dbeta) {
+                                                     float* __restrict__ dgamma, float* __restrict__ dbeta, long long ld_y, long long ld_dy) {
   constexpr int W = VEC ? 4 : 1, U = VEC ? 2 : 4;
   bn_reduce<W, 2, 8>(
       S, SW, partial, counter,
@@ -190,12 +200,18 @@
         for (int j = 0; j < W; ++j) { m[j] = mean[cw * W + j]; rs[j] = rstd[cw * W + j]; }
         const long long step = stride * S.C;
         long long i = r * S.C + cw * W;
-        for (; r + (U - 1) * stride < S.N; r += U * stride, i += U * step) {
+        const long long sy = LD ? stride * ld_y : 0, sg = LD ? stride * ld_dy : 0;
+        long long jy = LD ? r * ld_y + cw * W : 0, jg = LD ? r * ld_dy + cw * W : 0;
+#define BN_IY (LD ? jy : i)
+#define BN_IG (LD ? jg : i)
+#define BN_SY (LD ? sy : step)
+#define BN_SG (LD ? sg : step)
+        for (; r + (U - 1) * stride < S.N; r += U * stride, i += U * step, jy += U * sy, jg += U * sg) {
           float gv[U][W], yv[U][W], xv[U][W];
 #pragma unroll
           for (int u = 0; u < U; ++u) {
-            bn_ld<BF>(dy, i + u * step, gv[u]);
-            bn_ld<BF>(y, i + u * step, yv[u]);
+            bn_ld<BF>(dy, BN_IG + u * BN_SG, gv[u]);
+            bn_ld<BF>(y, BN_IY + u * BN_SY, yv[u]);
             bn_ld<BF>(x, i + u * step, xv[u]);
           }
 #pragma unroll
@@ -207,10 +223,10 @@
               acc[1][j] += (double)g * ((xv[u][j] - m[j]) * rs[j]);
             }
         }
-        for (; r < S.N; r += stride, i += step) {
+        for (; r < S.N; r += stride, i += step, jy += sy, jg += sg) {
           float gv[W], yv[W], xv[W];
-          bn_ld<BF>(dy, i, gv);
-          bn_ld<BF>(y, i, yv);
+          bn_ld<BF>(dy, BN_IG, gv);
+          bn_ld<BF>(y, BN_IY, yv);
           bn_ld<BF>(x, i, xv);
 #pragma unroll
           for (int j = 0; j < W; ++j) {
@@ -224,28 +240,33 @@
         dbeta[c] = (float)t[0];
         dgamma[c] = (float)t[1];
       });
-}
-
-template <bool VEC, bool BF>
+#undef BN_IY
+#undef BN_IG
+#undef BN_SY
+#undef BN_SG
+}
+
+template <bool VEC, bool BF, bool LD>
 __global__ __launch_bounds__(BN_T) void bn_bwd_apply(const float* __restrict__ x, const float* __restrict__ y, const float* __restrict__ dy,
                                                      const float* __restrict__ mean, const float* __restrict__ rstd,
                                                      const float* __restrict__ gamma, const float* __restrict__ dgamma,
                                                      const float* __restrict__ dbeta, long long total, int C, int N, int relu, int training,
-                                                     float* __restrict__ dx) {
+                                                     float* __restrict__ dx, long long ld_y, long long ld_dy) {
   long long i = ((long long)blockIdx.x * blockDim.x + threadIdx.x) * (VEC ? 4 : 1);
   if (i >= total) return;
   const float invn = 1.0f / (float)N;
   constexpr int W = VEC ? 4 : 1;
   float xv[W], yv[W], gv[W];
+  const int c = (int)(i % C);
+  const long long iy = bn_at<LD>(i, c, C, ld_y), ig = bn_at<LD>(i, c, C, ld_dy);
   if (VEC) {
-    float4 a = btc_ld4<BF>(x, i), b = btc_ld4<BF>(y, i), c4 = btc_ld4<BF>(dy, i);
+    float4 a = btc_ld4<BF>(x, i), b = btc_ld4<BF>(y, iy), c4 = btc_ld4<BF>(dy, ig);
     xv[0] = a.x; xv[W > 1 ? 1 : 0] = a.y; xv[W > 2 ? 2 : 0] = a.z; xv[W > 3 ? 3 : 0] = a.w;
     yv[0] = b.x; yv[W > 1 ? 1 : 0] = b.y; yv[W > 2 ? 2 : 0] = b.z; yv[W > 3 ? 3 : 0] = b.w;
     gv[0] = c4.x; gv[W > 1 ? 1 : 0] = c4.y; gv[W > 2 ? 2 : 0] = c4.z; gv[W > 3 ? 3 : 0] = c4.w;
   } else {
-    xv[0] = btc_ld1<BF>(x, i); yv[0] = btc_ld1<BF>(y, i); gv[0] = btc_ld1<BF>(dy, i);
+    xv[0] = btc_ld1<BF>(x, i); yv[0] = btc_ld1<BF>(y, iy); gv[0] = btc_ld1<BF>(dy, ig);
   }
-  const int c = (int)(i % C);
   float o[W];
 #pragma unroll
   for (int j = 0; j < W; ++j) {
@@ -327,10 +348,24 @@
 
 extern "C" size_t btc_bn_ws_bytes(int C) { return 256 + btc_align((size_t)512 * 2 * C * sizeof(double)); }
 
+struct BnLd {
+  long long ld_y = 0, ld_y2 = 0, ld_dy = 0;
+  float* y2 = nullptr;
+};
+
+template <bool BF>
+static bool bn_ld_ok(int C, const void* p, long long ld, int col) {
+  if (!p) return true;
+  if (ld < (long long)col + C || col < 0) return false;
+  if (C & 3) return true;
+  return (ld & 3) == 0 && (col & 3) == 0 && ((uintptr_t)p % (BF ? 8 : 16)) == 0;
+}
+
 template <bool BF>
 static int bn_fwd_impl(const float* x, int N, int C, const float* gamma, const float* beta, float* running_mean,
                                float* running_var, long long* num_batches_tracked, float momentum, float eps, int training, int relu,
-                               float* y, float* save_mean, float* save_rstd, void* ws_, size_t ws_bytes, void* stream_, bool have_stats = false) {
+                               float* y, float* save_mean, float* save_rstd, void* ws_, size_t ws_bytes, void* stream_, bool have_stats = false,
+                               const BnLd* ld = nullptr) {
   hipStream_t stream = (hipStream_t)stream_;
   BTC_CHECK_ARG(N >= 1 && C >= 1, "btc_bn_relu_fwd: empty input");
   BTC_CHECK_ARG(ws_bytes >= btc_bn_ws_bytes(C), "btc_bn_relu_fwd: workspace too small");
@@ -348,7 +383,11 @@
       bn_eval_stats<<<btc_cdiv(C, BN_T), BN_T, 0, stream>>>(running_mean, running_var, C, eps, save_mean, save_rstd);
     }
     BTC_LAUNCH_CHECK();
-    bn_apply<W == 4, BF><<<btc_cdiv(total / W, BN_T), BN_T, 0, stream>>>(x, save_mean, save_rstd, gamma, beta, total, C, relu, y);
+    if (ld)
+      bn_apply<W == 4, BF, true><<<btc_cdiv(total / W, BN_T), BN_T, 0, stream>>>(x, save_mean, save_rstd, gamma, beta, total, C, relu, y, ld->ld_y,
+                                                                                 ld->y2, ld->ld_y2);
+    else
+      bn_apply<W == 4, BF, false><<<btc_cdiv(total / W, BN_T), BN_T, 0, stream>>>(x, save_mean, save_rstd, gamma, beta, total, C, relu, y, 0, nullptr, 0);
     BTC_LAUNCH_CHECK();
     return BTC_OK;
   });
@@ -357,7 +396,7 @@
 template <bool BF>
 static int bn_bwd_impl(const float* x, const float* y, const float* dy, int N, int C, const float* gamma, const float* save_mean,
                                const float* save_rstd, int training, int relu, float* dx, float* dgamma, float* dbeta, void* ws_,
-                               size_t ws_bytes, void* stream_) {
+                               size_t ws_bytes, void* stream_, const BnLd* ld = nullptr) {
   hipStream_t stream = (hipStream_t)stream_;
   BTC_CHECK_ARG(N >= 1 && C >= 1, "btc_bn_relu_bwd: empty input");
   BTC_CHECK_ARG(ws_bytes >= btc_bn_ws_bytes(C), "btc_bn_relu_bwd: workspace too small");
@@ -367,10 +406,18 @@
   return bn_by_width(N, C, [&](auto w, const BnShape& SW) {
     constexpr int W = decltype(w)::value;
     const int g = W == 4 ? bn_grid_bytes(total * (BF ? 6 : 12), BTC_TUNE_BN_BWD_KB, 128) : bn_grid_bwd(N, S);
-    bn_bwd_stats<BF, W == 4><<<g, BN_T, 0, stream>>>(x, y, dy, save_mean, save_rstd, S, SW, relu, ws.partial, ws.counter, dgamma, dbeta);
+    if (ld)
+      bn_bwd_stats<BF, W == 4, true><<<g, BN_T, 0, stream>>>(x, y, dy, save_mean, save_rstd, S, SW, relu, ws.partial, ws.counter, dgamma, dbeta,
+                                                             ld->ld_y, ld->ld_dy);
+    else
+      bn_bwd_stats<BF, W == 4, false><<<g, BN_T, 0, stream>>>(x, y, dy, save_mean, save_rstd, S, SW, relu, ws.partial, ws.counter, dgamma, dbeta, 0, 0);
     BTC_LAUNCH_CHECK();
-    bn_bwd_apply<W == 4, BF><<<btc_cdiv(total / W, BN_T), BN_T, 0, stream>>>(x, y, dy, save_mean, save_rstd, gamma, dgamma, dbeta, total, C, N,
-                                                                             relu, training, dx);
+    if (ld)
+      bn_bwd_apply<W == 4, BF, true><<<btc_cdiv(total / W, BN_T), BN_T, 0, stream>>>(x, y, dy, save_mean, save_rstd, gamma, dgamma, dbeta, total, C,
+                                                                                     N, relu, training, dx, ld->ld_y, ld->ld_dy);
+    else
+      bn_bwd_apply<W == 4, BF, false><<<btc_cdiv(total / W, BN_T), BN_T, 0, stream>>>(x, y, dy, save_mean, save_rstd, gamma, dgamma, dbeta, total, C,
+                                                                                      N, relu, training, dx, 0, 0);
     BTC_LAUNCH_CHECK();
     return BTC_OK;
   });
@@ -423,6 +470,49 @@
                            dgamma, dbeta, ws, ws_bytes, stream);
 }
 
+template <bool BF>
+static float* bn_col(const void* p, int col) { return p ? (float*)((char*)p + (size_t)col * (BF ? 2 : 4)) : nullptr; }
+
+template <bool BF>
+static int bn_fwd_ld(const char* who, BnLd& ld, float*& yp, int C, void* y, long long ld_y, int col_y, void* y2, long long ld_y2, int col_y2) {
+  BTC_CHECK_ARG(y && bn_ld_ok<BF>(C, y, ld_y, col_y) && bn_ld_ok<BF>(C, y2, ld_y2, col_y2),
+                "%s: y / y2 need ld >= col + C, and for C %% 4 == 0 ld, col multiples of 4 and a 16-byte (bf16: 8) aligned base", who);
+  ld.ld_y = ld_y; ld.ld_y2 = ld_y2; ld.y2 = bn_col<BF>(y2, col_y2);
+  yp = bn_col<BF>(y, col_y);
+  return BTC_OK;
+}
+
+extern "C" int btc_bn_relu_fwd_ld(int bf16, const void* x, int N, int C, const float* gamma, const float* beta, float* running_mean,
+                                  float* running_var, long long* num_batches_tracked, float momentum, float eps, int training, int relu,
+                                  void* y, long long ld_y, int col_y, void* y2, long long ld_y2, int col_y2, float* save_mean,
+                                  float* save_rstd, void* ws, size_t ws_bytes, void* stream) {
+  BnLd ld;
+  float* yp = nullptr;
+  const int rc = bf16 ? bn_fwd_ld<true>("btc_bn_relu_fwd_ld", ld, yp, C, y, ld_y, col_y, y2, ld_y2, col_y2)
+                      : bn_fwd_ld<false>("btc_bn_relu_fwd_ld", ld, yp, C, y, ld_y, col_y, y2, ld_y2, col_y2);
+  if (rc) return rc;
+  if (bf16)
+    return bn_fwd_impl<true>((const float*)x, N, C, gamma, beta, running_mean, running_var, num_batches_tracked, momentum, eps, training, relu, yp,
+                             save_mean, save_rstd, ws, ws_bytes, stream, false, &ld);
+  return bn_fwd_impl<false>((const float*)x, N, C, gamma, beta, running_mean, running_var, num_batches_tracked, momentum, eps, training, relu, yp,
+                            save_mean, save_rstd, ws, ws_bytes, stream, false, &ld);
+}
+
+extern "C" int btc_bn_relu_bwd_ld(int bf16, const void* x, const void* y, long long ld_y, int col_y, const void* dy, long long ld_dy, int col_dy,
+                                  int N, int C, const float* gamma, const float* save_mean, const float* save_rstd, int training, int relu,
+                                  void* dx, float* dgamma, float* dbeta, void* ws, size_t ws_bytes, void* stream) {
+  const bool ok = y && dy && (bf16 ? bn_ld_ok<true>(C, y, ld_y, col_y) && bn_ld_ok<true>(C, dy, ld_dy, col_dy)
+                                   : bn_ld_ok<false>(C, y, ld_y, col_y) && bn_ld_ok<false>(C, dy, ld_dy, col_dy));
+  BTC_CHECK_ARG(ok, "btc_bn_relu_bwd_ld: y / dy need ld >= col + C, and for C %% 4 == 0 ld, col multiples of 4 and a 16-byte (bf16: 8) aligned base");
+  BnLd ld;
+  ld.ld_y = ld_y; ld.ld_dy = ld_dy;
+  if (bf16)
+    return bn_bwd_impl<true>((const float*)x, bn_col<true>(y, col_y), bn_col<true>(dy, col_dy), N, C, gamma, save_mean, save_rstd, training, relu,
+                             (float*)dx, dgamma, dbeta, ws, ws_bytes, stream, &ld);
+  return bn_bwd_impl<false>((const float*)x, bn_col<false>(y, col_y), bn_col<false>(dy, col_dy), N, C, gamma, save_mean, save_rstd, training, relu,
+                            (float*)dx, dgamma, dbeta, ws, ws_bytes, stream, &ld);
+}
+
 extern "C" size_t btc_bn_fuse_ws_bytes(void) { return btc_bn_fuse_bytes(); }
 
 extern "C" int btc_conv_bn_relu_fwd(int operands, const void* src, const void* W, const float* bias, const int32_t* nbr, const int32_t* order,
@@ -433,10 +523,10 @@
                                   num_batches_tracked, momentum, eps, relu, y, save_mean, save_rstd, ws, ws_bytes, fuse_ws, stream);
 }
 
-extern "C" int btc_conv_bn_relu_fwd_src(int operands, const void* src, long long src_rows, const void* W, const float* bias, const int32_t* nbr,
-                                        const int32_t* order, int n_rows, int K, int Cin, int Cout, void* x, const float* gamma, const float* beta,
-                                        float* running_mean, float* running_var, long long* num_batches_tracked, float momentum, float eps, int relu,
-                                        void* y, float* save_mean, float* save_rstd, void* ws, size_t ws_bytes, void* fuse_ws, void* stream) {
+static int conv_bn_relu_fwd(int operands, const void* src, long long src_rows, const void* W, const float* bias, const int32_t* nbr,
+                            const int32_t* order, int n_rows, int K, int Cin, int Cout, void* x, const float* gamma, const float* beta,
+                            float* running_mean, float* running_var, long long* num_batches_tracked, float momentum, float eps, int relu,
+                            void* y, float* save_mean, float* save_rstd, void* ws, size_t ws_bytes, void* fuse_ws, void* stream, const BnLd* ld) {
   BTC_CHECK_ARG(n_rows >= 1, "btc_conv_bn_relu_fwd: empty input");
   BTC_CHECK_ARG(operands >= BTC_OPERANDS_F32 && operands <= BTC_OPERANDS_F32_SPLIT, "btc_conv_bn_relu_fwd: operands=%d", operands);
   const bool bf = operands == BTC_OPERANDS_BF16_ACT || operands == BTC_OPERANDS_BF16;
@@ -454,9 +544,32 @@
   if (rc) return rc;
   if (bf)
     return bn_fwd_impl<true>((const float*)x, n_rows, Cout, gamma, beta, running_mean, running_var, num_batches_tracked, momentum, eps, 1, relu,
-                             (float*)y, save_mean, save_rstd, ws, ws_bytes, stream, fused);
+                             (float*)y, save_mean, save_rstd, ws, ws_bytes, stream, fused, ld);
   return bn_fwd_impl<false>((const float*)x, n_rows, Cout, gamma, beta, running_mean, running_var, num_batches_tracked, momentum, eps, 1, relu,
-                            (float*)y, save_mean, save_rstd, ws, ws_bytes, stream, fused);
+                            (float*)y, save_mean, save_rstd, ws, ws_bytes, stream, fused, ld);
+}
+
+extern "C" int btc_conv_bn_relu_fwd_src(int operands, const void* src, long long src_rows, const void* W, const float* bias, const int32_t* nbr,
+                                        const int32_t* order, int n_rows, int K, int Cin, int Cout, void* x, const float* gamma, const float* beta,
+                                        float* running_mean, float* running_var, long long* num_batches_tracked, float momentum, float eps, int relu,
+                                        void* y, float* save_mean, float* save_rstd, void* ws, size_t ws_bytes, void* fuse_ws, void* stream) {
+  return conv_bn_relu_fwd(operands, src, src_rows, W, bias, nbr, order, n_rows, K, Cin, Cout, x, gamma, beta, running_mean, running_var,
+                          num_batches_tracked, momentum, eps, relu, y, save_mean, save_rstd, ws, ws_bytes, fuse_ws, stream, nullptr);
+}
+
+extern "C" int btc_conv_bn_relu_fwd_ld(int operands, const void* src, long long src_rows, const void* W, const float* bias, const int32_t* nbr,
+                                       const int32_t* order, int n_rows, int K, int Cin, int Cout, void* x, const float* gamma, const float* beta,
+                                       float* running_mean, float* running_var, long long* num_batches_tracked, float momentum, float eps, int relu,
+                                       void* y, long long ld_y, int col_y, void* y2, long long ld_y2, int col_y2, float* save_mean,
+                                       float* save_rstd, void* ws, size_t ws_bytes, void* fuse_ws, void* stream) {
+  const bool bf = operands == BTC_OPERANDS_BF16_ACT || operands == BTC_OPERANDS_BF16;
+  BnLd ld;
+  float* yp = nullptr;
+  const int rc = bf ? bn_fwd_ld<true>("btc_conv_bn_relu_fwd_ld", ld, yp, Cout, y, ld_y, col_y, y2, ld_y2, col_y2)
+                    : bn_fwd_ld<false>("btc_conv_bn_relu_fwd_ld", ld, yp, Cout, y, ld_y, col_y, y2, ld_y2, col_y2);
+  if (rc) return rc;
+  return conv_bn_relu_fwd(operands, src, src_rows, W, bias, nbr, order, n_rows, K, Cin, Cout, x, gamma, beta, running_mean, running_var,
+                          num_batches_tracked, momentum, eps, relu, yp, save_mean, save_rstd, ws, ws_bytes, fuse_ws, stream, &ld);
 }
 
 extern "C" int btc_conv_bn_eval_fwd(int operands, const void* src, long long src_rows, const void* W, const float* bias, const int32_t* nbr,
diff --git a/btcdet_amd/spconv/modules.py b/btcdet_amd/spconv/modules.py
--- a/btcdet_amd/spconv/modules.py
+++ b/btcdet_amd/spconv/modules.py
@@ -133,7 +133,7 @@
             plan.append((conv, bn, relu, rb, conv.inverse))
         return plan, indices, shape
 
-    def _run_chain(self, input, plan, indices, shape):
+    def _run_chain(self, input, plan, indices, shape, y_into=None, keep_dense=False):
         from . import fused_bn, ops
         F = ops.fast()
         key = tuple((bn.training, bn.track_running_stats, id(conv.weight), id(conv.bias), id(bn.weight), id(bn.bias), id(bn.running_mean),
@@ -159,7 +159,11 @@
                 mf.append(rb.nbr_out); mb.append(rb.map_bwd); of.append(rb.order_out); ob.append(rb.order_in)
             ov.append(bool(ops._overlap_ok(mf[-1].shape[0])))
         ws = fused_bn._ws(input.features.device, max(wt.shape[-1] for wt in w))[0]
-        out = F.conv_bn_relu_chain(ops._actc(input.features), w, b, mf, mb, of, ob, ga, be, rms, rvs, nbts, ub, mom, eps, relus, ws, need, ov, dfr)
+        if y_into is None:
+            out = F.conv_bn_relu_chain(ops._actc(input.features), w, b, mf, mb, of, ob, ga, be, rms, rvs, nbts, ub, mom, eps, relus, ws, need, ov, dfr)
+        else:
+            out = F.conv_bn_relu_chain(ops._actc(input.features), w, b, mf, mb, of, ob, ga, be, rms, rvs, nbts, ub, mom, eps, relus, ws, need, ov, dfr,
+                                       y_into=y_into, keep_dense=keep_dense)
         out_tensor = SparseConvTensor(out, indices, shape, input.batch_size)
         out_tensor.indice_dict = input.indice_dict
         out_tensor.grid = input.grid
diff --git a/include/btcdet_hip_strided.h b/include/btcdet_hip_strided.h
--- /dev/null
+++ b/include/btcdet_hip_strided.h
@@ -0,0 +1,31 @@
+#ifndef BTCDET_HIP_STRIDED_H
+#define BTCDET_HIP_STRIDED_H
+
+#include <stddef.h>
+#include <stdint.h>
+
+#include "btcdet_hip.h"
+
+#ifdef __cplusplus
+extern "C" {
+#endif
+
+int btc_bn_relu_fwd_ld(int bf16, const void* x, int N, int C, const float* gamma, const float* beta, float* running_mean,
+                       float* running_var, long long* num_batches_tracked, float momentum, float eps, int training, int relu,
+                       void* y, long long ld_y, int col_y, void* y2, long long ld_y2, int col_y2, float* save_mean,
+                       float* save_rstd, void* ws, size_t ws_bytes, void* stream);
+
+int btc_bn_relu_bwd_ld(int bf16, const void* x, const void* y, long long ld_y, int col_y, const void* dy, long long ld_dy, int col_dy,
+                       int N, int C, const float* gamma, const float* save_mean, const float* save_rstd, int training, int relu,
+                       void* dx, float* dgamma, float* dbeta, void* ws, size_t ws_bytes, void* stream);
+
+int btc_conv_bn_relu_fwd_ld(int operands, const void* src, long long src_rows, const void* W, const float* bias, const int32_t* nbr,
+                            const int32_t* order, int n_rows, int K, int Cin, int Cout, void* x, const float* gamma, const float* beta,
+                            float* running_mean, float* running_var, long long* num_batches_tracked, float momentum, float eps, int relu,
+                            void* y, long long ld_y, int col_y, void* y2, long long ld_y2, int col_y2, float* save_mean,
+                            float* save_rstd, void* ws, size_t ws_bytes, void* fuse_ws, void* stream);
+
+#ifdef __cplusplus
+}
+#endif
+#endif
```
